# L-Scofano/SEEME

Hardware: AMD Instinct MI355X
Metric: sampled seqs/sec (T=196, 50 DDIM steps) (higher is better)
Workload: dtype f32 accumulate (fp16 denoiser weights, fp16 VAE MFMA operands); 1 GPU; config_mld_egobody interactee-only: VAE encode -> 50-step DDIM -> VAE decode, B=32/GPU, T=196, nfeats=132, random-init recipe weights; batch_per_gpu=32, seq_len=196, ddim_steps=50, parallelism=dp1 (independent shards, no collective on the data path)

## Files before the change

include/seeme_hip.h:

```cpp
#ifndef SEEME_HIP_H
#define SEEME_HIP_H

#include <stddef.h>
#include <stdint.h>

#ifdef __cplusplus
extern "C" {
#endif

#define SEEME_D 256
#define SEEME_NLAYERS 5

enum { SEEME_ACT_NONE = 0, SEEME_ACT_RELU = 1, SEEME_ACT_GELU = 2, SEEME_ACT_SILU = 3 };
enum { SEEME_SCHED_NONE = 0, SEEME_SCHED_DDIM = 1, SEEME_SCHED_DDPM = 2 };

int seeme_version(void);
const char* seeme_last_error(void);

#define SEEME_LINEAR_MAX_K 1008
typedef struct {
    const float* A;  int lda;
    const float* A2; int lda2;
    int K1;
    const float* W;  int ldw;
    const float* bias;
    const float* res; int ldr;
    const float* ln_w; const float* ln_b;
    const float* pre_ln_w; const float* pre_ln_b;
    float* Y; int ldy;
    int M, N, K;
    int pre_act;
    int act;
    float eps;
} SeemeLinearArgs;
int seeme_linear(const SeemeLinearArgs* args, void* stream);

typedef struct {
    const float *in_w, *in_b;
    const float *out_w, *out_b;
    const float *l1_w, *l1_b;
    const float *l2_w, *l2_b;
    const float *n1_w, *n1_b, *n2_w, *n2_b;
    const float *ca_in_w, *ca_in_b;
    const float *ca_out_w, *ca_out_b;
    const float *n3_w, *n3_b;
} SeemeXfLayer;

typedef struct {
    SeemeXfLayer layer[SEEME_NLAYERS];
    const float *skip_w[2], *skip_b[2];
    const float *norm_w, *norm_b;
} SeemeSkipStack;

typedef struct { const uint16_t *in_w, *out_w, *l1_w, *l2_w; } SeemeXfLayerH;
typedef struct {
    SeemeXfLayerH enc[SEEME_NLAYERS], dec[SEEME_NLAYERS];
    const uint16_t *enc_skip[2], *dec_skip[2];
    const uint16_t *emb_w, *fin_w, *ca_fold_w;
    const void* dec_pro; int dec_pro_T;
} SeemeVaeWeightsH;

typedef struct {
    int nfeats;
    int ff;
    const float* token;
    const float* pe_enc;
    const float* pe_dec;
    const float* emb_w; int emb_ldw;
    const float* emb_b;
    const float* fin_w;
    const float* fin_b;
    SeemeSkipStack enc, dec;
    const float* ca_fold_w;
    const float* ca_fold_b;
    const SeemeVaeWeightsH* h16;
} SeemeVaeWeights;

size_t seeme_vae_workspace_bytes(int B, int T);

int seeme_vae_encode(const SeemeVaeWeights* w, const float* features, const int32_t* lengths,
                     int B, int T, float* mu, float* logvar, void* workspace, size_t ws_bytes, void* stream);

int seeme_vae_decode(const SeemeVaeWeights* w, const float* z, const int32_t* lengths,
                     int B, int T, float* feats, void* workspace, size_t ws_bytes, void* stream);

size_t seeme_vae_dec_prologue_bytes(int T);
int seeme_vae_dec_prologue_h16(const SeemeVaeWeights* w, int T, void* buf, size_t bytes, void* stream);

typedef struct {
    const void*  wg;   int wdtype;
    const float* vp;
    const int64_t* layout;
    int nhead;
    int ff_sa;
    int ff;
    const float* kv_cat_w; const float* kv_cat_b;
    const float* style_cat_w; const float* style_cat_b;
    const float* time_w1; const float* time_b1; const float* time_w2; const float* time_b2;
    const float* ca_kv_w[SEEME_NLAYERS]; const float* ca_kv_b[SEEME_NLAYERS];
    const float* ca_tn_w[SEEME_NLAYERS]; const float* ca_tn_b[SEEME_NLAYERS];
    const float* ca_fold_w; const float* ca_fold_b;
    const float* ln_ones; const float* ln_zeros;
    int sa_fold;
    const float* ca_pn_w; const float* ca_pn_b;
    const float* ca_po_w; const float* ca_po_b;
} SeemeDenoiserWeights;

#define SEEME_TROW 7680
#define SEEME_CROW 5120

size_t seeme_denoiser_workspace_bytes(int n_rows, int B, int N);

int seeme_denoiser_time_tables(const SeemeDenoiserWeights* w, const float* tfeat, int n_rows,
                               float* ttab, void* workspace, size_t ws_bytes, void* stream);

int seeme_denoiser_cond_tables(const SeemeDenoiserWeights* w, const float* cond, int Bc, int N,
                               float* ctab, void* workspace, size_t ws_bytes, void* stream);

int seeme_denoiser_ca_tables(const SeemeDenoiserWeights* w, const float* ctab, const float* ttab, const int32_t* trow,
                             int trow_per_sample, int n_trow, int Bc, float* catab,
                             void* workspace, size_t ws_bytes, void* stream);

typedef struct {
    int B;
    int N;
    int steps;
    int sched;
    int cfg;
    float guidance_scale;
    const float* latents;
    const float* ctab;
    const float* ttab;
    const int32_t* trow;
    int trow_per_sample;
    const float* coef;
    const float* noise;
    float* out;
    const float* catab;
    float* save;
    int force_query;
    const unsigned char* drop;
    float drop_scale;
    int xcds;
} SeemeSampleArgs;
#define SEEME_DEN_DROP_BYTES 10960

int seeme_denoiser_sample(const SeemeDenoiserWeights* w, const SeemeSampleArgs* a, void* stream);

typedef struct {
    const void*  wgc;  int wdtype;
    const float* vpc;
    int C;
    int placement;
    int flags;
    void* xchg; size_t xchg_bytes;
    int query;
    int samples;
} SeemeDenCluster;
size_t seeme_den_cluster_xchg_bytes(int B, int C);
size_t seeme_den_cluster_ms_xchg_bytes(int B, int C, int samples);
int seeme_den_cluster_layout(int C, int wdtype, int query, int64_t* out, int cap);
int seeme_denoiser_sample_cluster(const SeemeDenoiserWeights* w, const SeemeDenCluster* cl, const SeemeSampleArgs* a, void* stream);

int seeme_den_train_layout(int64_t* out, int cap);
int seeme_den_train_pack(const float* const* mats, float* img_f, float* img_b, const float* const* vec_src,
                         const int* vec_n, const int64_t* vec_dst, int n_vec, float* vp, void* stream);
int seeme_denoiser_backward(const SeemeDenoiserWeights* w, const void* img_bwd, int B, int N, const float* save,
                            const float* ctab, const float* ttab, const int32_t* trow, const float* dout,
                            float* gout, float* dctab, float* dttab, void* stream);
int seeme_denoiser_backward_drop(const SeemeDenoiserWeights* w, const void* img_bwd, int B, int N, const float* save,
                                 const float* ctab, const float* ttab, const int32_t* trow, const float* dout,
                                 float* gout, float* dctab, float* dttab, const unsigned char* drop, float drop_scale, int xcds, void* stream);

int seeme_den_layout(int ff_sa, int ff, int64_t* out, int cap);

typedef struct {
    int V;
    const float* v_template;
    const float* blend_w;
    const float* lbs_weights;
    const float* J_template;
    const float* J_shapedirs;
    const int32_t* parents;
    const float* ex_template;
    const float* ex_shapedirs;
    const float* ex_posedirs;
    const float* ex_weights;
} SeemeSmplModel;

size_t seeme_smpl_workspace_bytes(int M);

int seeme_smpl_lbs(const SeemeSmplModel* m, const float* betas, const float* pose, int pose_is_rotmat,
                   const float* transl, int M, float* joints, float* vertices,
                   void* workspace, size_t ws_bytes, void* stream);

int seeme_smpl_joints_backward(const SeemeSmplModel* m, const float* betas, const float* pose, const float* djoints, int dj_stride,
                               float* dpose, float* dtransl, int M, void* stream);

int seeme_smpl_joints_rot6d(const SeemeSmplModel* m, const float* betas, const float* r6, int order, const float* transl, int M,
                            float* joints, void* stream);
int seeme_smpl_joints_rot6d_backward(const SeemeSmplModel* m, const float* betas, const float* r6, int order, const float* djoints,
                                     int dj_stride, float* dr6, float* dtransl, int M, void* stream);

enum { SEEME_GEO_AA_TO_QUAT = 0, SEEME_GEO_AA_TO_ROTMAT = 1, SEEME_GEO_QUAT_TO_ROTMAT = 2,
       SEEME_GEO_ROT6D_PROHMR = 3, SEEME_GEO_ROT6D_DIFFUSION = 4 };
int seeme_geometry(int op, const float* in, float* out, int M, void* stream);
int seeme_renorm(const float* x, const float* mean, const float* stdv, float* y, long rows, int F, void* stream);

typedef struct {
    int out_dim;
    const float* pos_w; const float* pos_b;
    const float* fc0_w[4]; const float* fc0_b[4];
    const float* fc1_w[4]; const float* fc1_b[4];
    const float* sc_w[4];
    const float* fcc_w; const float* fcc_b;
} SeemePointnetWeights;
size_t seeme_pointnet_workspace_bytes(int B, int P);
int seeme_pointnet_encode(const SeemePointnetWeights* w, const float* points, int B, int P, float* out,
                          void* workspace, size_t ws_bytes, void* stream);

typedef struct {
    const uint16_t* posf;
    const uint16_t* stream[4];
    const uint16_t* sc3f;
} SeemePointnetBf16;
size_t seeme_pointnet_bf16_workspace_bytes(int B, int P);
int seeme_pointnet_encode_bf16(const SeemePointnetWeights* w, const SeemePointnetBf16* wb, const float* points,
                               int B, int P, float* out, void* workspace, size_t ws_bytes, void* stream);

int seeme_den_wgrad(const float* gout, int ldg, int B, const void* tiles, int n_tiles, float* out, void* stream);
int seeme_den_vecgrad(const float* gout, int ldg, int B, const int64_t* idx, int n, float* out, int dx0_col, float* dpe_row0,
                      void* stream);

int seeme_adamw_step(const void* chunks, int n_chunks, void* const* params, const void* const* grads, void* const* exp_avg,
                     void* const* exp_avg_sq, double lr, double beta1, double beta2, double eps, double weight_decay,
                     double step, void* stream);

int seeme_adamw_step_dev(const void* chunks, int n_chunks, void* const* params, const void* const* grads, void* const* exp_avg,
                         void* const* exp_avg_sq, const float* step_lr, double beta1, double beta2, double eps,
                         double weight_decay, void* stream);

typedef struct {
    const void* chunks;
    int n_chunks;
    void* const* params;
    const void* const* grads;
    void* const* exp_avg;
    void* const* exp_avg_sq;
    void* const* ema;
    const float* step_lr;
    double lr, step;
    double beta1, beta2, eps, weight_decay;
    double ema_decay;
    int ema_warmup;
    const float* grad_scale;
} SeemeAdamWEx;
int seeme_adamw_step_ex(const SeemeAdamWEx* a, void* stream);
int seeme_adamw_ex_bytes(void);

size_t seeme_grad_norm_workspace_bytes(int n_chunks);
int seeme_grad_norm(const void* chunks, int n_chunks, const void* const* grads, double max_norm, float* out ,
                    void* ws, size_t ws_bytes, void* stream);

typedef struct {
    int B, N;
    const float* dist;
    int dist_rows;
    const float* eps_z;
    const float* eps_c;
    int slot_c;
    float* cond;
    const float* noise;
    const int64_t* timesteps;
    const float* acp;
// ... 184 lines not shown
```

seeme_amd/_lib.py:

```python
from __future__ import annotations

import ctypes as C
import os
from typing import Optional

_HERE = os.path.dirname(os.path.abspath(__file__))
LIB_PATH = os.environ.get("SEEME_HIP_LIB") or os.path.join(_HERE, "libseeme_hip.so")

NLAYERS = 5
TROW = 7680
CROW = 5120
ACT_NONE, ACT_RELU, ACT_GELU, ACT_SILU = 0, 1, 2, 3
SCHED_NONE, SCHED_DDIM, SCHED_DDPM = 0, 1, 2

fp = C.c_void_p


class SeemeError(RuntimeError):
    pass


class LinearArgs(C.Structure):
    _fields_ = [("A", fp), ("lda", C.c_int), ("A2", fp), ("lda2", C.c_int), ("K1", C.c_int),
                ("W", fp), ("ldw", C.c_int), ("bias", fp), ("res", fp), ("ldr", C.c_int),
# ... 15 lines not shown

class XfLayerH(C.Structure):
    _fields_ = [(n, fp) for n in ("in_w", "out_w", "l1_w", "l2_w")]


class VaeWeightsH(C.Structure):
    _fields_ = [("enc", XfLayerH * NLAYERS), ("dec", XfLayerH * NLAYERS), ("enc_skip", fp * 2), ("dec_skip", fp * 2),
                ("emb_w", fp), ("fin_w", fp), ("ca_fold_w", fp), ("dec_pro", fp), ("dec_pro_T", C.c_int)]


def pack_mfma16(W, dtype):
    import torch
    N, K = W.shape
    Np, Kp = (N + 15) // 16 * 16, (K + 31) // 32 * 32
    Wz = torch.zeros(Np, Kp, device=W.device, dtype=dtype)
    Wz[:N, :K] = W.detach().to(dtype)
    return Wz.view(Np // 16, 16, Kp // 32, 4, 8).permute(0, 2, 3, 1, 4).contiguous()


class VaeWeights(C.Structure):
    _fields_ = [("nfeats", C.c_int), ("ff", C.c_int), ("token", fp), ("pe_enc", fp), ("pe_dec", fp),
                ("emb_w", fp), ("emb_ldw", C.c_int), ("emb_b", fp), ("fin_w", fp), ("fin_b", fp),
                ("enc", SkipStack), ("dec", SkipStack), ("ca_fold_w", fp), ("ca_fold_b", fp), ("h16", fp)]


class DenoiserWeights(C.Structure):
    _fields_ = [("wg", fp), ("wdtype", C.c_int), ("vp", fp), ("layout", fp), ("nhead", C.c_int), ("ff_sa", C.c_int),
                ("ff", C.c_int), ("kv_cat_w", fp), ("kv_cat_b", fp), ("style_cat_w", fp), ("style_cat_b", fp),
                ("time_w1", fp), ("time_b1", fp), ("time_w2", fp), ("time_b2", fp),
                ("ca_kv_w", fp * NLAYERS), ("ca_kv_b", fp * NLAYERS),
                ("ca_tn_w", fp * NLAYERS), ("ca_tn_b", fp * NLAYERS),
                ("ca_fold_w", fp), ("ca_fold_b", fp), ("ln_ones", fp), ("ln_zeros", fp), ("sa_fold", C.c_int),
                ("ca_pn_w", fp), ("ca_pn_b", fp), ("ca_po_w", fp), ("ca_po_b", fp)]


class SampleArgs(C.Structure):
    _fields_ = [("B", C.c_int), ("N", C.c_int), ("steps", C.c_int), ("sched", C.c_int), ("cfg", C.c_int),
                ("guidance_scale", C.c_float), ("latents", fp), ("ctab", fp), ("ttab", fp), ("trow", fp),
                ("trow_per_sample", C.c_int), ("coef", fp), ("noise", fp), ("out", fp), ("catab", fp), ("save", fp), ("force_query", C.c_int), ("drop", fp), ("drop_scale", C.c_float), ("xcds", C.c_int)]


class DenCluster(C.Structure):
    _fields_ = [("wgc", fp), ("wdtype", C.c_int), ("vpc", fp), ("C", C.c_int), ("placement", C.c_int), ("flags", C.c_int),
                ("xchg", fp), ("xchg_bytes", C.c_size_t), ("query", C.c_int), ("samples", C.c_int)]


class SmplModel(C.Structure):
    _fields_ = [("V", C.c_int), ("v_template", fp), ("blend_w", fp), ("lbs_weights", fp), ("J_template", fp),
                ("J_shapedirs", fp), ("parents", fp), ("ex_template", fp), ("ex_shapedirs", fp),
                ("ex_posedirs", fp), ("ex_weights", fp)]


class PointnetWeights(C.Structure):
    _fields_ = [("out_dim", C.c_int), ("pos_w", fp), ("pos_b", fp), ("fc0_w", fp * 4), ("fc0_b", fp * 4),
                ("fc1_w", fp * 4), ("fc1_b", fp * 4), ("sc_w", fp * 4), ("fcc_w", fp), ("fcc_b", fp)]


class PointnetBf16(C.Structure):
    _fields_ = [("posf", fp), ("stream", fp * 4), ("sc3f", fp)]


class GlueRows(C.Structure):
    _fields_ = [("B", C.c_int), ("N", C.c_int), ("dist", fp), ("dist_rows", C.c_int), ("eps_z", fp), ("eps_c", fp),
                ("slot_c", C.c_int), ("cond", fp), ("noise", fp), ("timesteps", fp), ("acp", fp), ("freq", fp),
                ("flip_sin_to_cos", C.c_int), ("latents", fp), ("noisy", fp), ("tfeat", fp)]


class GemmProblem(C.Structure):
    _fields_ = [("a", fp * 10), ("b", fp * 10), ("seg_len", C.c_int * 10), ("a_ks", C.c_long * 10),
                ("b_ks", C.c_long * 10), ("nseg", C.c_int), ("a_rs", C.c_long), ("b_cs", C.c_long), ("c", fp), ("ldc", C.c_long),
                ("M", C.c_int), ("N", C.c_int), ("a_pro", C.c_int), ("a_p0", fp), ("a_p1", fp), ("b_pro", C.c_int),
                ("b_p0", fp), ("b_p1", fp), ("bias", fp), ("epi", C.c_int), ("e0", fp), ("e_ld", C.c_long),
                ("accumulate", C.c_int), ("colsum", fp), ("tile0", C.c_int), ("tiles_n", C.c_int), ("nbatch", C.c_int),
                ("a_bstride", C.c_long), ("b_bstride", C.c_long), ("c_bstride", C.c_long), ("alpha", C.c_float), ("addend", fp),
                ("add_ld", C.c_long)]


class VtLn(C.Structure):
    _fields_ = [("sub", fp), ("res", fp), ("gamma", fp), ("beta", fp), ("y", fp), ("xhat", fp), ("rstd", fp), ("M", C.c_long),
                ("sub_seq_rows", C.c_int), ("eps", C.c_float)]


class VtLnBwd(C.Structure):
    _fields_ = [("dy", fp), ("xhat", fp), ("rstd", fp), ("gamma", fp), ("dpre", fp), ("dgamma", fp), ("dbeta", fp), ("M", C.c_long),
                ("accumulate", C.c_int), ("dy2", fp)]


class GlueMid(C.Structure):
    _fields_ = [("M", C.c_int), ("B", C.c_int), ("dxl", fp), ("dcs", fp), ("xhat", fp), ("rstd", fp), ("tn_w", fp * 5),
                ("g_tn_w", fp * 5), ("g_tn_b", fp * 5), ("dcond", fp), ("dea", fp), ("deb", fp), ("emb", fp), ("demb", fp)]


class AdamWEx(C.Structure):
    _fields_ = [("chunks", fp), ("n_chunks", C.c_int), ("params", fp), ("grads", fp), ("exp_avg", fp), ("exp_avg_sq", fp),
                ("ema", fp), ("step_lr", fp), ("lr", C.c_double), ("step", C.c_double), ("beta1", C.c_double), ("beta2", C.c_double),
                ("eps", C.c_double), ("weight_decay", C.c_double), ("ema_decay", C.c_double), ("ema_warmup", C.c_int),
                ("grad_scale", fp)]


RESNET_FP32, RESNET_BF16 = 0, 1
IMG_F32_NCHW, IMG_U8_NHWC = 0, 1
RESNET50_NCONV = 53


class Conv(C.Structure):
    _fields_ = [("weight", fp), ("weight_bf16", fp), ("bias", fp), ("cin", C.c_int), ("cout", C.c_int), ("k", C.c_int),
                ("stride", C.c_int)]


class Resnet50(C.Structure):
    _fields_ = [("precision", C.c_int), ("conv", Conv * RESNET50_NCONV), ("tap", fp * 5)]


class RenderScene(C.Structure):
    _fields_ = [("verts", fp), ("faces", fp), ("points", fp), ("cams", fp)] + \
               [(n, C.c_int) for n in ("F", "NV", "NF", "P", "FC", "H", "W", "point_size")] + \
               [(n, C.c_float) for n in ("fx", "fy", "cx", "cy", "znear")]


GEO_AA_TO_QUAT, GEO_AA_TO_ROTMAT, GEO_QUAT_TO_ROTMAT, GEO_ROT6D_PROHMR, GEO_ROT6D_DIFFUSION = range(5)

_SIGNATURES = {
    "seeme_smpl_joints_backward": (C.c_int, [C.POINTER(SmplModel), fp, fp, fp, C.c_int, fp, fp, C.c_int, fp]),
    "seeme_smpl_joints_rot6d": (C.c_int, [C.POINTER(SmplModel), fp, fp, C.c_int, fp, C.c_int, fp, fp]),
    "seeme_smpl_joints_rot6d_backward": (C.c_int, [C.POINTER(SmplModel), fp, fp, C.c_int, fp, C.c_int, fp, fp, C.c_int, fp]),
    "seeme_vt_add_ln": (C.c_int, [C.POINTER(VtLn), fp]),
    "seeme_vt_ln_bwd": (C.c_int, [C.POINTER(VtLnBwd), fp]),
    "seeme_vt_softmax_fwd": (C.c_int, [fp, fp, C.c_int, C.c_int, C.c_int, C.c_float, fp]),
    "seeme_vt_softmax_bwd": (C.c_int, [fp, fp, C.c_long, C.c_int, C.c_float, fp]),
    "seeme_vt_gelu": (C.c_int, [fp, fp, fp, C.c_long, fp]),
    "seeme_vt_seq_sum": (C.c_int, [fp, fp, C.c_int, C.c_int, C.c_int, fp, C.c_float, fp]),
    "seeme_vt_dropout": (C.c_int, [fp, fp, C.c_float, fp, C.c_long, fp]),
    "seeme_vt_cross_rows": (C.c_int, [fp, fp, fp, fp, C.c_float, C.c_int, C.c_int, fp, fp]),
    "seeme_den_vecgrad": (C.c_int, [fp, C.c_int, C.c_int, fp, C.c_int, fp, C.c_int, fp, fp]),
    "seeme_glue_rows": (C.c_int, [C.POINTER(GlueRows), fp]),
    "seeme_glue_ln": (C.c_int, [fp, fp, fp, C.c_int, fp]),
    "seeme_glue_mid": (C.c_int, [C.POINTER(GlueMid), fp]),
    "seeme_grouped_gemm": (C.c_int, [fp, C.c_int, C.c_int, fp]),
    "seeme_gemm_problem_bytes": (C.c_int, []),
    "seeme_wgrad128": (C.c_int, [fp, C.c_long, fp, C.c_long, C.c_int, C.c_int, C.c_int, fp, C.c_long, fp, fp]),
    "seeme_gemm128": (C.c_int, [fp, C.c_long, fp, C.c_long, C.c_int, fp, C.c_long, C.c_int, C.c_int, C.c_int, fp, fp, C.c_long, fp]),
    "seeme_version": (C.c_int, []),
    "seeme_last_error": (C.c_char_p, []),
    "seeme_linear": (C.c_int, [C.POINTER(LinearArgs), fp]),
    "seeme_vae_workspace_bytes": (C.c_size_t, [C.c_int, C.c_int]),
    "seeme_vae_encode": (C.c_int, [C.POINTER(VaeWeights), fp, fp, C.c_int, C.c_int, fp, fp, fp, C.c_size_t, fp]),
    "seeme_vae_decode": (C.c_int, [C.POINTER(VaeWeights), fp, fp, C.c_int, C.c_int, fp, fp, C.c_size_t, fp]),
    "seeme_vae_dec_prologue_bytes": (C.c_size_t, [C.c_int]),
    "seeme_vae_dec_prologue_h16": (C.c_int, [C.POINTER(VaeWeights), C.c_int, fp, C.c_size_t, fp]),
    "seeme_denoiser_workspace_bytes": (C.c_size_t, [C.c_int, C.c_int, C.c_int]),
    "seeme_denoiser_time_tables": (C.c_int, [C.POINTER(DenoiserWeights), fp, C.c_int, fp, fp, C.c_size_t, fp]),
    "seeme_denoiser_cond_tables": (C.c_int, [C.POINTER(DenoiserWeights), fp, C.c_int, C.c_int, fp, fp, C.c_size_t, fp]),
    "seeme_denoiser_ca_tables": (C.c_int, [C.POINTER(DenoiserWeights), fp, fp, fp, C.c_int, C.c_int, C.c_int, fp, fp, C.c_size_t, fp]),
    "seeme_denoiser_sample": (C.c_int, [C.POINTER(DenoiserWeights), C.POINTER(SampleArgs), fp]),
    "seeme_denoiser_sample_cluster": (C.c_int, [C.POINTER(DenoiserWeights), C.POINTER(DenCluster), C.POINTER(SampleArgs), fp]),
    "seeme_den_cluster_xchg_bytes": (C.c_size_t, [C.c_int, C.c_int]),
    "seeme_den_cluster_ms_xchg_bytes": (C.c_size_t, [C.c_int, C.c_int, C.c_int]),
    "seeme_den_cluster_layout": (C.c_int, [C.c_int, C.c_int, C.c_int, C.POINTER(C.c_int64), C.c_int]),
    "seeme_den_train_layout": (C.c_int, [C.POINTER(C.c_int64), C.c_int]),
    "seeme_den_train_pack": (C.c_int, [fp, fp, fp, fp, C.POINTER(C.c_int), C.POINTER(C.c_int64), C.c_int, fp, fp]),
    "seeme_denoiser_backward": (C.c_int, [C.POINTER(DenoiserWeights), fp, C.c_int, C.c_int, fp, fp, fp, fp, fp, fp, fp, fp, fp]),
    "seeme_denoiser_backward_drop": (C.c_int, [C.POINTER(DenoiserWeights), fp, C.c_int, C.c_int, fp, fp, fp, fp, fp, fp, fp, fp, fp, C.c_float, C.c_int, fp]),
    "seeme_den_layout": (C.c_int, [C.c_int, C.c_int, C.POINTER(C.c_int64), C.c_int]),
    "seeme_den_wgrad": (C.c_int, [fp, C.c_int, C.c_int, fp, C.c_int, fp, fp]),
    "seeme_adamw_step": (C.c_int, [fp, C.c_int, fp, fp, fp, fp, C.c_double, C.c_double, C.c_double, C.c_double, C.c_double,
                                   C.c_double, fp]),
    "seeme_adamw_step_dev": (C.c_int, [fp, C.c_int, fp, fp, fp, fp, fp, C.c_double, C.c_double, C.c_double, C.c_double, fp]),
    "seeme_adamw_step_ex": (C.c_int, [C.POINTER(AdamWEx), fp]),
    "seeme_adamw_ex_bytes": (C.c_int, []),
    "seeme_grad_norm_workspace_bytes": (C.c_size_t, [C.c_int]),
    "seeme_grad_norm": (C.c_int, [fp, C.c_int, fp, C.c_double, fp, fp, C.c_size_t, fp]),
    "seeme_geometry": (C.c_int, [C.c_int, fp, fp, C.c_int, fp]),
    "seeme_renorm": (C.c_int, [fp, fp, fp, fp, C.c_long, C.c_int, fp]),
    "seeme_pointnet_workspace_bytes": (C.c_size_t, [C.c_int, C.c_int]),
    "seeme_pointnet_encode": (C.c_int, [C.POINTER(PointnetWeights), fp, C.c_int, C.c_int, fp, fp, C.c_size_t, fp]),
    "seeme_pointnet_bf16_workspace_bytes": (C.c_size_t, [C.c_int, C.c_int]),
    "seeme_pointnet_encode_bf16": (C.c_int, [C.POINTER(PointnetWeights), C.POINTER(PointnetBf16), fp, C.c_int, C.c_int, fp, fp,
                                             C.c_size_t, fp]),
    "seeme_smpl_workspace_bytes": (C.c_size_t, [C.c_int]),
    "seeme_smpl_lbs": (C.c_int, [C.POINTER(SmplModel), fp, fp, C.c_int, fp, C.c_int, fp, fp, fp, C.c_size_t, fp]),
    "seeme_hyp_metrics_workspace_bytes": (C.c_size_t, [C.c_int, C.c_int, C.c_int]),
    "seeme_hyp_metrics": (C.c_int, [fp, fp, fp, C.c_int, C.c_int, C.c_int, fp, fp, fp, C.c_size_t, fp]),
    "seeme_hyp_pairdist_workspace_bytes": (C.c_size_t, [C.c_int, C.c_int, C.c_int]),
    "seeme_hyp_pairdist": (C.c_int, [fp, fp, C.c_int, C.c_int, C.c_int, fp, fp, fp, C.c_size_t, fp]),
    "seeme_social_metrics_workspace_bytes": (C.c_size_t, [C.c_int, C.c_int, C.c_int]),
    "seeme_social_metrics": (C.c_int, [fp, fp, fp, fp, fp, fp, fp, C.c_int, C.c_int, C.c_int, fp, fp, fp, C.c_size_t, fp]),
    "seeme_overlap_cost_workspace_bytes": (C.c_size_t, [C.c_int, C.c_int, C.c_int, C.c_int]),
    "seeme_overlap_cost": (C.c_int, [fp, C.c_int, C.c_int, C.c_int, C.c_int, fp, fp, C.c_size_t, fp]),
    "seeme_path_select_workspace_bytes": (C.c_size_t, [C.c_int, C.c_int]),
    "seeme_path_select": (C.c_int, [fp, fp, C.c_int, C.c_int, fp, fp, fp, fp, C.c_size_t, fp]),
    "seeme_stitch_windows": (C.c_int, [fp, C.c_int, C.c_int, C.c_int, C.c_int, C.c_int, C.c_int, fp, fp]),
    "seeme_scene_views_workspace_bytes": (C.c_size_t, [C.c_int, C.c_int, C.c_int]),
    "seeme_scene_views": (C.c_int, [fp, fp, C.c_int, C.c_int, C.c_int, fp, fp, fp, fp, C.c_size_t, fp]),
    "seeme_crop_patches": (C.c_int, [fp, C.c_int, C.c_int, C.c_int, fp, fp, C.c_int, C.c_int, fp, fp]),
    "seeme_render_workspace_bytes": (C.c_size_t, [C.c_int, C.c_int, C.c_int, C.c_int]),
    "seeme_render": (C.c_int, [C.POINTER(RenderScene), fp, fp, fp, fp, C.c_size_t, fp]),
    "seeme_render_shade": (C.c_int, [C.POINTER(RenderScene), fp, fp, fp, C.c_int, fp, C.c_uint32, fp, fp]),
    "seeme_pa_mpjpe_frames": (C.c_int, [fp, fp, fp, C.c_int, fp, fp]),
    "seeme_mesh_v2v_frames": (C.c_int, [fp, fp, fp, fp, fp, C.c_int, C.c_int, fp, fp]),
    "seeme_scene_min_dist2_workspace_bytes": (C.c_size_t, [C.c_int, C.c_int, C.c_int, C.c_int]),
    "seeme_scene_min_dist2": (C.c_int, [fp, fp, fp, C.c_int, C.c_int, C.c_int, C.c_int, fp, fp, C.c_size_t, fp]),
    "seeme_scene_inside_count_workspace_bytes": (C.c_size_t, [C.c_int, C.c_int, C.c_int, C.c_int]),
    "seeme_scene_inside_count": (C.c_int, [fp, fp, C.c_int, fp, fp, C.c_int, C.c_int, C.c_int, C.c_int, fp, fp, C.c_size_t, fp]),
    "seeme_mesh_winding": (C.c_int, [fp, fp, C.c_int, fp, fp, C.c_int, C.c_int, C.c_int, C.c_int, fp, fp]),
    "seeme_resnet50_workspace_bytes": (C.c_size_t, [C.c_int, C.c_int]),
    "seeme_resnet50_encode": (C.c_int, [C.POINTER(Resnet50), fp, C.c_int, C.c_int, fp, fp, C.c_size_t, fp]),
    "seeme_resnet_conv": (C.c_int, [C.POINTER(Conv), C.c_int, fp, C.c_int, C.c_int, C.c_int, fp, C.c_int, fp, fp]),
    "seeme_resnet_stem_pack": (C.c_int, [fp, C.c_int, C.c_int, C.c_int, C.c_int, C.c_int, fp, fp]),
    "seeme_resnet_maxpool": (C.c_int, [C.c_int, fp, C.c_int, C.c_int, C.c_int, C.c_int, fp, fp]),
}

_lib: Optional[C.CDLL] = None


def lib() -> C.CDLL:
    global _lib
    if _lib is None:
        if not os.path.exists(LIB_PATH):
            raise SeemeError(
                f"{LIB_PATH} is missing: build it with `python -c 'import __graft_entry__ as g; g.build()'` "
                "or seeme_amd/csrc/build.sh.  There is no CPU / PyTorch fallback for this path.")
        try:
            l = C.CDLL(LIB_PATH)
        except OSError as e:
            raise SeemeError(f"cannot load {LIB_PATH}: {e}") from e
        for name, (res, args) in _SIGNATURES.items():
            f = getattr(l, name)
            f.restype = res
            f.argtypes = args
        _lib = l
    return _lib


def exported_symbols():
    return sorted(_SIGNATURES)


def check(rc: int, what: str = ""):
    if rc != 0:
        msg = lib().seeme_last_error().decode("utf-8", "replace")
        raise SeemeError(f"{what or 'seeme_hip'} failed (rc={rc}): {msg}")


def call(name: str, *args):
    check(getattr(lib(), name)(*args), name)


class Workspace:

    def __init__(self, per_stream: bool):
        self.per_stream = per_stream
        self._held = {}

    def get(self, need: int, device):
        import torch
        device = torch.device(device)
        if device.type == "cuda" and device.index is None:
            device = torch.device("cuda", torch.cuda.current_device())
        key = device
        if self.per_stream and device.type == "cuda":
            key = (device, torch.cuda.current_stream(device).cuda_stream)
        ws = self._held.get(key)
        if ws is None or ws.numel() < max(need, 16):
            ws = None
            self._held.pop(key, None)
            ws = self._held[key] = torch.empty(max(int(need), 16), dtype=torch.uint8, device=device)
        return ws

    def cached(self) -> list:
        return list(self._held.values())

    def fill_(self, byte: int):
        for ws in self._held.values():
            ws.fill_(byte)


def default_xcds(chains: int, want="auto") -> int:
    e = os.environ.get("SEEME_DEN_XCDS")
    if e is not None:
        want = int(e)
    if want == "auto":
        want = (chains + 15) // 16
    return min(8, max(1, int(want)))


def ptr(t) -> int:
    return 0 if t is None else t.data_ptr()


def current_stream() -> int:
    import torch
    return torch.cuda.current_stream().cuda_stream


def require_cuda(t, name: str):
    import torch
    if not isinstance(t, torch.Tensor) or not t.is_cuda:
        raise SeemeError(f"{name} must be a tensor on the ROCm device (cuda:N); this path has no CPU fallback")
    if t.dtype != torch.float32:
        raise SeemeError(f"{name} must be float32, got {t.dtype}")
```

seeme_amd/csrc/den_kernels.hip:

```cpp
#include <atomic>
#include "common.hpp"
#include "api_util.hpp"
#include "den_layout.h"
#include "lds_ring.hpp"
#include "den_train.h"
#include <utility>

#define DEN_THREADS 512
#define SEEME_DEN_PAIR_ABOVE 256
#define DEN_MAXTOK 6
#define DEN_R 4
#define DEN_CH 8

struct WF32 { typedef float T; static constexpr int KV = 4; static constexpr bool HALF = false, MFMA = false; static constexpr int PARTS = 1; };
struct WBF16 { typedef uint16_t T; static constexpr int KV = 8; static constexpr bool HALF = false, MFMA = true; static constexpr int PARTS = 3; };
struct WF16 { typedef uint16_t T; static constexpr int KV = 8; static constexpr bool HALF = true, MFMA = true; static constexpr int PARTS = 2; };
#define DEN_F16_LO_SCALE 2048.f

typedef float f2 __attribute__((ext_vector_type(2)));
typedef unsigned int u32x4 __attribute__((ext_vector_type(4)));
typedef float f32x4 __attribute__((ext_vector_type(4)));
typedef _Float16 h16x8 __attribute__((ext_vector_type(8)));
typedef __bf16 bf16x8 __attribute__((ext_vector_type(8)));

struct Ring { u32x4 r[DEN_R][DEN_CH]; };

#define FF_SA 1024
#define FF_D 128
#define XB_LD 1024

enum { G_SKIP = 0, G_INP, G_OUTP, G_L1, G_L2, G_CAQ, G_CAO, G_F1, G_F2, G_FO, G_NUM,
       GB_FO = G_NUM, GB_F2, GB_F1, GB_CAO, GB_CAQ, GB_L2, GB_L1, GB_OUTP, GB_INP, GB_SKIP, G_ALL };
constexpr int den_gK(int g) {
    constexpr int k[G_ALL] = {512, 256, 256, 256, FF_SA, 256, 256, 256, FF_D, 256,
                              256, 256, FF_D, 256, 256, 256, FF_SA, 256, 768, 256};
    return k[g];
}
constexpr int den_gN(int g) {
    constexpr int n[G_ALL] = {256, 768, 256, FF_SA, 256, 256, 256, FF_D, 256, 256,
                              256, FF_D, 256, 256, 256, FF_SA, 256, 256, 256, 512};
    return n[g];
}

constexpr int den_gcd(int a, int b) { return b == 0 ? a : den_gcd(b, a % b); }
template <typename WT, int G>
struct GS {
    static constexpr int K = den_gK(G), N = den_gN(G);
    static constexpr int G0 = N / 2;
    static constexpr int KS = DEN_THREADS / den_gcd(G0, DEN_THREADS);
    static constexpr int IT = G0 / den_gcd(G0, DEN_THREADS);
    static constexpr int NQ = K / WT::KV / KS;
    static constexpr int CPI = NQ / 4;
    static constexpr int TOT = IT * CPI;
    static_assert(G0 * KS == DEN_THREADS * IT && NQ * KS * WT::KV == K && NQ % 4 == 0 && TOT >= 1, "unsupported GEMV shape");
    static constexpr int TW = N / 16 / (DEN_THREADS / 64), KB = K / 32;
    static constexpr int TG = (TW % 4 == 0) ? 4 : ((TW % 3 == 0) ? 3 : ((TW % 2 == 0) ? 2 : 1));
    static constexpr int GL = TG * KB;
    static_assert(!WT::MFMA || (TW * 16 * (DEN_THREADS / 64) == N && KB * 32 == K && TW * KB == TOT * DEN_CH && GL % DEN_CH == 0),
                  "unsupported MFMA GEMV shape");
    __device__ static __forceinline__ void item(int tid, int it, int& ks, int& n0) {
        const int idx = tid + it * DEN_THREADS;
        ks = idx / G0; n0 = idx - ks * G0;
    }
};

#define V_CAQ 1
#define V_FOLD 2
template <typename WT, int V>
struct Prog {
    static constexpr bool CAQ = (V & V_CAQ) != 0, FOLD = (V & V_FOLD) != 0;
    static constexpr int NG = 6 + (CAQ ? 2 : 0) + (FOLD ? 0 : 1);
    static constexpr int gid(int i) {
        constexpr int all[9] = {G_INP, G_OUTP, G_L1, G_L2, G_CAQ, G_CAO, G_F1, G_F2, G_FO};
        int k = 0;
        for (int j = 0; j < 9; ++j) {
            const int g = all[j];
            if ((g == G_OUTP && FOLD) || ((g == G_CAQ || g == G_CAO) && !CAQ)) continue;
            if (k == i) return g;
            ++k;
        }
        return G_FO;
    }
    static constexpr int tot(int g) {
        switch (g) {
            case G_SKIP: return GS<WT, G_SKIP>::TOT; case G_INP: return GS<WT, G_INP>::TOT; case G_OUTP: return GS<WT, G_OUTP>::TOT;
            case G_L1: return GS<WT, G_L1>::TOT; case G_L2: return GS<WT, G_L2>::TOT; case G_CAQ: return GS<WT, G_CAQ>::TOT;
            case G_CAO: return GS<WT, G_CAO>::TOT; case G_F1: return GS<WT, G_F1>::TOT; case G_F2: return GS<WT, G_F2>::TOT;
            default: return GS<WT, G_FO>::TOT;
        }
    }
    static constexpr int sum_real() { int s = 0; for (int j = 0; j < NG; ++j) s += tot(gid(j)); return s; }
    static constexpr int T = (sum_real() + DEN_R - 1) / DEN_R * DEN_R;
    static constexpr int PAD = T - sum_real();
    static constexpr int PAD0 = tot(G_INP);
    static constexpr bool is_pad(int t) { return t >= PAD0 && t < PAD0 + PAD; }
    static constexpr int start(int i) { int s = (i >= 1 ? PAD : 0); for (int j = 0; j < i; ++j) s += tot(gid(j)); return s; }
    static constexpr int TS = tot(G_SKIP);
    static constexpr int find(int t) { int i = 0; while (i + 1 < NG && start(i + 1) <= t) ++i; return i; }
    static constexpr int pos(int g) { int i = 0; while (gid(i) != g) ++i; return i; }
    static_assert(gid(0) == G_INP, "in_proj opens the layer program");
    static_assert(TS % DEN_R == 0 && TS >= DEN_R, "skip linear must fill whole ring turns");
    static_assert(tot(G_INP) >= DEN_R, "the first GEMV of a layer must cover the cross-layer prefetch");
};

#ifdef DEN_DBG_TIMES
__device__ unsigned long long den_dbg_times[512];
__device__ __forceinline__ void den_dbg(int mode) {
    __shared__ unsigned long long buf[512];
    __shared__ int cnt, armed;
    if (blockIdx.x != 0 || threadIdx.x != 0) return;
    if (mode == 1) { cnt = 0; armed = 1; }
    else if (mode == 2) { armed = 0; }
    else if (mode == 0) { if (armed && cnt < 511) { buf[cnt] = __builtin_readcyclecounter(); cnt = cnt + 1; } }
    else {
        const int n = (armed == 0 && cnt >= 0 && cnt <= 511) ? cnt : 0;
        for (int i = 0; i < n; ++i) den_dbg_times[i + 1] = buf[i];
        den_dbg_times[0] = (unsigned long long)n;
    }
}
#define DEN_DBG(m) den_dbg(m)
#else
#define DEN_DBG(m) do {} while (0)
#endif

template <typename WT, int G, int C>
__device__ __forceinline__ void issue_mat(u32x4 (&slot)[DEN_CH], int tid, __amdgpu_buffer_rsrc_t rsrc, unsigned mat_bytes) {
    typedef GS<WT, G> S;
    if constexpr (WT::MFMA) {
        const unsigned voff = (unsigned)(tid >> 6) * (unsigned)(S::TW * S::KB * 1024) + (unsigned)(tid & 63) * 16u;
        const unsigned soff = mat_bytes + (unsigned)(C * DEN_CH) * 1024u;
#pragma unroll
        for (int i = 0; i < DEN_CH; ++i) slot[i] = __builtin_amdgcn_raw_buffer_load_b128(rsrc, voff, soff + (unsigned)(i * 1024), 0);
        return;
    }
    constexpr int it = C / S::CPI, cc = C % S::CPI;
    int ks, n0;
    S::item(tid, it, ks, n0);
    const unsigned voff = (unsigned)(ks * S::NQ * S::N + n0) * 16u;
    const unsigned soff = mat_bytes + (unsigned)(cc * 4) * S::N * 16u;
#pragma unroll
    for (int i = 0; i < DEN_CH; ++i)
        slot[i] = __builtin_amdgcn_raw_buffer_load_b128(rsrc, voff, soff + (unsigned)(((i >> 1) * S::N + (i & 1) * S::G0) * 16), 0);
}
struct MatOffs { unsigned m[G_NUM]; unsigned next; };
template <typename WT>
__device__ __forceinline__ MatOffs load_mat_offs(const DenLayerOff* __restrict__ L, const DenLayerOff* __restrict__ Ln, bool nskip) {
    MatOffs o;
#pragma unroll
    for (int g = 0; g < G_NUM; ++g) o.m[g] = (unsigned)(reinterpret_cast<const int64_t*>(L)[g] * (long long)sizeof(typename WT::T));
    o.next = (unsigned)((nskip ? Ln->skip : Ln->inp) * (long long)sizeof(typename WT::T));
    return o;
}

template <typename WT, int V, int T>
__device__ __forceinline__ void issue_p0(Ring& ring, int tid, __amdgpu_buffer_rsrc_t rsrc, const MatOffs& mo) {
// ... 659 lines not shown
                    xr = f4_add(nl, ld4(CONSTV + 4 * lane));
                    put_x<WT, MS>(XB, es, 0, lane, xr);
                }
                __syncthreads(); DEN_DBG(0);
            }
            cur ^= 1;
        }
        row = row_next;
    }
    DEN_DBG(3);
    if (epi && (es == 0 || (!A.cfg && MS * b + es < A.B))) st4(A.out + (size_t)bl * 256 + 4 * lane, ld4(keep));
#pragma unroll
    for (int s = 0; s < DEN_R; ++s) asm volatile("" ::"v"(ring.r[s][0].x));
}

static size_t den_lds_bytes(int MS, int N, bool mfma) {
    return (size_t)(768 + MS * 768 + 2 * (VP_LAYER + STG_TT + MS * N * 1024 + (N > 1 ? 0 : MS * 256)) + XB_FLOATS(mfma, MS) + (mfma ? MS * 1024 : 4 * MS * 768)) * sizeof(float);
}

static int den_xcd_grid(int chains, int want, int* xcds) {
    int k = (want >= 1 && want <= 7) ? want : 8;
    if (chains > 32 * k) k = 8;
    *xcds = k;
    return k < 8 ? (chains + k - 1) / k * 8 : chains;
}
template <typename WT, int MS, int V>
static int launch_den(const DenKArgs& ka, hipStream_t st) {
    const int chains = (MS == 2 && !ka.s.cfg) ? (ka.s.B + 1) / 2 : ka.s.B;
    const size_t lds = den_lds_bytes(MS, ka.s.N, WT::MFMA);
    if (lds > 160 * 1024) return seeme_fail("denoiser_sample: LDS budget exceeded");
    SEEME_HIP(hipFuncSetAttribute((const void*)k_den_sample<WT, MS, V>, hipFuncAttributeMaxDynamicSharedMemorySize, (int)lds));
    DenKArgs k2 = ka;
    k2.chains = chains;
    const int grid = den_xcd_grid(chains, ka.s.xcds, &k2.xcds);
    hipLaunchKernelGGL((k_den_sample<WT, MS, V>), dim3(grid), dim3(DEN_THREADS), lds, st, k2);
    return seeme_check_launch("k_den_sample");
}
template <typename WT, int MS>
static int launch_den_ms(const DenKArgs& ka, bool fold, hipStream_t st) {
    const bool caq = ka.s.N > 1 || ka.s.force_query;
    if (caq) return fold ? launch_den<WT, MS, V_CAQ | V_FOLD>(ka, st) : launch_den<WT, MS, V_CAQ>(ka, st);
    return fold ? launch_den<WT, MS, V_FOLD>(ka, st) : launch_den<WT, MS, 0>(ka, st);
}
template <typename WT>
static int launch_den_wt(const DenKArgs& ka, bool fold, hipStream_t st) {
    const bool pair = ka.s.cfg || (ka.s.B > SEEME_DEN_PAIR_ABOVE && !ka.s.trow_per_sample);
    return pair ? launch_den_ms<WT, 2>(ka, fold, st) : launch_den_ms<WT, 1>(ka, fold, st);
}

extern "C" int seeme_denoiser_sample(const SeemeDenoiserWeights* w, const SeemeSampleArgs* a, void* stream) {
    if (a->B <= 0) return seeme_fail("denoiser_sample: B must be > 0");
    if (a->N < 1 || a->N > DEN_MAXTOK - 2) return seeme_fail("denoiser_sample: 1 <= N <= 4 condition tokens");
    if (w->nhead != 1 && w->nhead != 2 && w->nhead != 4) return seeme_fail("denoiser_sample: nhead must be 1, 2 or 4");
    if (w->ff_sa != FF_SA || w->ff != FF_D) return seeme_fail("denoiser_sample: built for sa ff 1024 / ffn_dim 128 (all reference configs)");
    if (w->layout == nullptr) return seeme_fail("denoiser_sample: layout table missing");
    if (a->sched == SEEME_SCHED_NONE && a->steps != 1) return seeme_fail("denoiser_sample: SCHED_NONE needs steps == 1");
    if (a->steps < 1) return seeme_fail("denoiser_sample: steps must be >= 1");
    if (a->save != nullptr && (a->steps != 1 || a->cfg || w->sa_fold || w->wdtype != 0 || !(a->N > 1 || a->force_query) || !a->trow_per_sample))
        return seeme_fail("denoiser_sample: save needs one step, no CFG, the unfolded fp32 image, the query GEMV and per-sample rows");
    DenKArgs ka;
    ka.wg = w->wg; ka.vp = w->vp; ka.lay = seeme_make_den_layout(FF_SA, FF_D);
    ka.wg_bytes = (int)(ka.lay.wg_total * (w->wdtype == 0 ? 4 : 2));
    ka.nhead = w->nhead; ka.s = *a;
    hipStream_t st = (hipStream_t)stream;
    const bool fold = w->sa_fold != 0;
    if (fold && w->nhead != 1) return seeme_fail("denoiser_sample: sa_fold needs nhead == 1");
    if (a->N == 1 && a->catab == nullptr && !a->force_query) return seeme_fail("denoiser_sample: N == 1 needs the ca table (seeme_denoiser_ca_tables)");
    if (w->wdtype == 0) return launch_den_wt<WF32>(ka, fold, st);
    if (w->wdtype == 1) return launch_den_wt<WBF16>(ka, fold, st);
    if (w->wdtype == 2) return launch_den_wt<WF16>(ka, fold, st);
    return seeme_fail("denoiser_sample: wdtype must be 0 (fp32), 1 (bf16) or 2 (fp16)");
}

extern "C" int seeme_den_layout(int ff_sa, int ff, int64_t* out, int cap) {
    if (cap < SEEME_DEN_LAYOUT_FIELDS) return seeme_fail("seeme_den_layout: output too small");
    const DenLayout lay = seeme_make_den_layout(ff_sa, ff);
    int k = 0;
    for (int l = 0; l < SEEME_DEN_NL; ++l) {
        const int64_t* f = reinterpret_cast<const int64_t*>(&lay.L[l]);
        for (int i = 0; i < SEEME_DEN_LAYER_FIELDS; ++i) out[k++] = f[i];
    }
    out[k++] = lay.pe0; out[k++] = lay.fnw; out[k++] = lay.fnb; out[k++] = lay.wg_total; out[k++] = lay.vp_total;
    return 0;
}

extern "C" size_t seeme_denoiser_workspace_bytes(int n_rows, int B, int N) {
    (void)B; (void)N;
    return (size_t)n_rows * 256 * 2 * sizeof(float) + 256;
}

extern "C" int seeme_denoiser_time_tables(const SeemeDenoiserWeights* w, const float* tfeat, int n_rows,
                                          float* ttab, void* workspace, size_t ws_bytes, void* stream) {
    hipStream_t st = (hipStream_t)stream;
    if (ws_bytes < seeme_denoiser_workspace_bytes(n_rows, 0, 0)) return seeme_fail("time_tables: workspace too small");
    float* t1 = (float*)workspace;
    float* temb = t1 + (size_t)n_rows * 256;
    int rc;
    if ((rc = seeme_linear_simple(st, tfeat, 256, w->time_w1, 256, w->time_b1, t1, 256, n_rows, 256, 256, SEEME_ACT_SILU, 0, nullptr, nullptr))) return rc;
    if ((rc = seeme_linear_simple(st, t1, 256, w->time_w2, 256, w->time_b2, temb, 256, n_rows, 256, 256, 0, 0, nullptr, nullptr))) return rc;
    if ((rc = seeme_linear_simple(st, temb, 256, w->kv_cat_w, 256, w->kv_cat_b, ttab, SEEME_TROW, n_rows, 2560, 256, 0, 0, nullptr, nullptr))) return rc;
    return seeme_linear_simple(st, temb, 256, w->style_cat_w, 256, w->style_cat_b, ttab + 2560, SEEME_TROW, n_rows, 5120, 256, 0, SEEME_ACT_SILU, nullptr, nullptr);
}

extern "C" int seeme_denoiser_cond_tables(const SeemeDenoiserWeights* w, const float* cond, int Bc, int N,
                                          float* ctab, void* workspace, size_t ws_bytes, void* stream) {
    (void)workspace; (void)ws_bytes;
    hipStream_t st = (hipStream_t)stream;
    const int M = Bc * N;
    if (w->ca_fold_w == nullptr) return seeme_fail("cond_tables: folded key/value weights missing");
    LinearKArgs ka{};
    ka.a.A = cond; ka.a.lda = 256; ka.a.K1 = 256; ka.a.K = 256; ka.a.W = w->kv_cat_w; ka.a.ldw = 256; ka.a.bias = w->kv_cat_b;
    ka.a.Y = ctab; ka.a.ldy = SEEME_CROW; ka.a.M = M; ka.a.N = 2560; ka.a.eps = 1e-5f;
    ka.a.pre_ln_w = w->ln_ones; ka.a.pre_ln_b = w->ln_zeros;
    ka.nz = 2; ka.zs_a = 0; ka.zs_w = (long)(w->ca_fold_w - w->kv_cat_w); ka.zs_b = (long)(w->ca_fold_b - w->kv_cat_b); ka.zs_y = 2560;
    ka.zs_ln = 0; ka.pre_ln_zmin = 1;
    return seeme_launch_linear(ka, st);
}

__global__ __launch_bounds__(256) void k_ca_rows(const float* __restrict__ ctab, const float* __restrict__ ttab,
                                                 const int32_t* __restrict__ trow, int per_sample, int n_trow, int R, int rows,
                                                 const float* __restrict__ nw, const float* __restrict__ nb, float* __restrict__ H) {
    const int lane = threadIdx.x & 63, l = blockIdx.y;
    const int r0 = blockIdx.x * 4 + (threadIdx.x >> 6);
    if (r0 >= rows) return;
    const int bc = r0 / R, r = r0 - bc * R;
    const int row = per_sample ? trow[bc % n_trow] : trow[r];
    const float4 v = ld4(ctab + (size_t)bc * SEEME_CROW + 2560 + l * 512 + 256 + 4 * lane);
    const float4 hn = wave_ln(v, nw + l * 256, nb + l * 256, lane);
    const float* tt = ttab + (size_t)row * SEEME_TROW + 2560 + l * 1024;
    st4(H + ((size_t)l * rows + r0) * 256 + 4 * lane, f4_silu(f4_adaln(hn, ld4(tt + 4 * lane), ld4(tt + 256 + 4 * lane))));
}

extern "C" int seeme_denoiser_ca_tables(const SeemeDenoiserWeights* w, const float* ctab, const float* ttab, const int32_t* trow,
                                        int trow_per_sample, int n_trow, int Bc, float* catab,
                                        void* workspace, size_t ws_bytes, void* stream) {
    hipStream_t st = (hipStream_t)stream;
    if (Bc <= 0 || n_trow <= 0) return seeme_fail("ca_tables: empty batch / row list");
    const int R = trow_per_sample ? 1 : n_trow;
    const int rows = Bc * R;
    if (ws_bytes < (size_t)SEEME_DEN_NL * rows * 256 * sizeof(float)) return seeme_fail("ca_tables: workspace too small");
    if (w->ca_pn_w == nullptr || w->ca_po_w == nullptr) return seeme_fail("ca_tables: proj_out weights missing");
    float* H = (float*)workspace;
    hipLaunchKernelGGL(k_ca_rows, dim3((rows + 3) / 4, SEEME_DEN_NL), dim3(256), 0, st, ctab, ttab, trow, trow_per_sample, n_trow, R, rows,
                       w->ca_pn_w, w->ca_pn_b, H);
    int rc = seeme_check_launch("k_ca_rows");
    if (rc) return rc;
    LinearKArgs ka{};
    ka.a.A = H; ka.a.lda = 256; ka.a.K1 = 256; ka.a.W = w->ca_po_w; ka.a.ldw = 256; ka.a.bias = w->ca_po_b;
    ka.a.Y = catab; ka.a.ldy = SEEME_DEN_NL * 256; ka.a.M = rows; ka.a.N = 256; ka.a.K = 256; ka.a.eps = 1e-5f;
    ka.nz = SEEME_DEN_NL; ka.zs_a = (long)rows * 256; ka.zs_w = 256 * 256; ka.zs_b = 256; ka.zs_y = 256;
    return seeme_launch_linear(ka, st);
}

#ifdef DEN_DBG_TIMES
extern "C" int seeme_debug_den_times(unsigned long long* host, int n) {
    SEEME_HIP(hipMemcpyFromSymbol(host, HIP_SYMBOL(den_dbg_times), sizeof(unsigned long long) * (size_t)(n < 512 ? n : 512)));
    return 0;
}
#endif

#include "den_train.inc.hip"
#include "den_cluster.inc.hip"
#include "den_cluster_ms.inc.hip"
```

seeme_amd/csrc/vae_h16.hip:

```cpp
#include "common.hpp"
#include "api_util.hpp"

typedef _Float16 h16x8 __attribute__((ext_vector_type(8)));
#define HPAD 16

__device__ __forceinline__ unsigned short f2h(float x) { return __builtin_bit_cast(unsigned short, (_Float16)x); }
__device__ __forceinline__ float h_exp(float x) { return __builtin_amdgcn_exp2f(x * 1.44269504088896340736f); }
__device__ __forceinline__ float h_gelu(float x) {
    const float z = fabsf(x) * 0.70710678118654752440f;
    const float t = __builtin_amdgcn_rcpf(fmaf(0.3275911f, z, 1.f));
    const float poly = t * fmaf(t, fmaf(t, fmaf(t, fmaf(t, 1.061405429f, -1.453152027f), 1.421413741f), -0.284496736f), 0.254829592f);
    return 0.5f * x * (1.f + copysignf(1.f - poly * h_exp(-z * z), x));
}
__device__ __forceinline__ float h_act(float v, int act) { return act == SEEME_ACT_GELU ? h_gelu(v) : act_apply(v, act); }

#ifdef H16_DBG_TIMES
__device__ unsigned long long h16_dbg_times[32];
#ifndef H16_DBG_KERNEL
#define H16_DBG_KERNEL 1
#endif
#define H16_DBG(k, i) do { if (H16_DBG_KERNEL == (k) && blockIdx.x == 3 && blockIdx.y == ((k) == 1 ? 5 : 0) && threadIdx.x == 0) h16_dbg_times[i] = __builtin_readcyclecounter(); } while (0)
extern "C" int seeme_debug_h16_times(unsigned long long* host, int n) {
    SEEME_HIP(hipMemcpyFromSymbol(host, HIP_SYMBOL(h16_dbg_times), sizeof(unsigned long long) * (size_t)(n < 32 ? n : 32)));
    return 0;
}
#else
#define H16_DBG(k, i) do {} while (0)
#endif
#ifndef H16_PF
#define H16_PF 4
#endif
#ifndef H16_ALA
#define H16_ALA 1
#endif
#ifndef FFN_PF
#define FFN_PF H16_PF
#endif
template <int NTL, int PF>
struct BRing { uint4 br[PF][NTL]; };
template <int NTL, int PF, typename LoadB>
__device__ __forceinline__ void ring_prime(BRing<NTL, PF>& ring, int K32, LoadB loadb) {
#pragma unroll
    for (int u = 0; u < PF; ++u)
#pragma unroll
        for (int nt = 0; nt < NTL; ++nt) ring.br[u][nt] = loadb(nt, u < K32 ? u : K32 - 1);
}

template <int MTL, int NTL, int PF, typename LoadB>
__device__ __forceinline__ void tile_gemm_h16(const unsigned short* __restrict__ As, int lda, int K32, LoadB loadb,
                                              f32x4 (&acc)[MTL][NTL], BRing<NTL, PF>& ring) {
    const int lane = threadIdx.x & 63, r = lane & 15, kq = lane >> 4;
    const unsigned short* ap = As + r * lda + 8 * kq;
    uint4 (&br)[PF][NTL] = ring.br;
    constexpr int AS = H16_ALA == 1 ? 2 : 4;
    static_assert(PF % AS == 0, "A-fragment slots follow the ring slot");
    uint4 ab[AS][MTL];
#pragma unroll
    for (int d = 0; d < H16_ALA; ++d)
#pragma unroll
        for (int mt = 0; mt < MTL; ++mt) ab[d][mt] = *reinterpret_cast<const uint4*>(ap + mt * 16 * lda + (d < K32 ? d : K32 - 1) * 32);
    const int K32r = (K32 + PF - 1) / PF * PF;
    int kb0 = 0;
    for (; kb0 + PF < K32r; kb0 += PF) {
#pragma unroll
        for (int u = 0; u < PF; ++u) {
            const int kb = kb0 + u;
            const int ka = kb + H16_ALA < K32 ? kb + H16_ALA : K32 - 1;
#pragma unroll
            for (int mt = 0; mt < MTL; ++mt) ab[(u + H16_ALA) % AS][mt] = *reinterpret_cast<const uint4*>(ap + mt * 16 * lda + ka * 32);
            __builtin_amdgcn_sched_barrier(0);
#pragma unroll
            for (int mt = 0; mt < MTL; ++mt)
#pragma unroll
                for (int nt = 0; nt < NTL; ++nt)
                    acc[mt][nt] = __builtin_amdgcn_mfma_f32_16x16x32_f16(__builtin_bit_cast(h16x8, ab[u % AS][mt]), __builtin_bit_cast(h16x8, br[u][nt]), acc[mt][nt], 0, 0, 0);
            __builtin_amdgcn_sched_barrier(0);
            const int kn = kb + PF < K32 ? kb + PF : K32 - 1;
#pragma unroll
            for (int nt = 0; nt < NTL; ++nt) br[u][nt] = loadb(nt, kn);
        }
    }
#pragma unroll
    for (int u = 0; u < PF; ++u) {
        const int kb = kb0 + u;
        const int ka = (kb + H16_ALA < K32) ? kb + H16_ALA : K32 - 1;
#pragma unroll
        for (int mt = 0; mt < MTL; ++mt) ab[(u + H16_ALA) % AS][mt] = *reinterpret_cast<const uint4*>(ap + mt * 16 * lda + ka * 32);
        __builtin_amdgcn_sched_barrier(0);
        if (kb < K32) {
#pragma unroll
            for (int mt = 0; mt < MTL; ++mt)
#pragma unroll
                for (int nt = 0; nt < NTL; ++nt)
                    acc[mt][nt] = __builtin_amdgcn_mfma_f32_16x16x32_f16(__builtin_bit_cast(h16x8, ab[u % AS][mt]), __builtin_bit_cast(h16x8, br[u][nt]), acc[mt][nt], 0, 0, 0);
        }
        __builtin_amdgcn_sched_barrier(0);
    }
}
struct PackedSrc {
    __amdgpu_buffer_rsrc_t rs; int kstride, ntile0, ntiles; unsigned voff;
    __device__ __forceinline__ PackedSrc(const uint4* __restrict__ Wp, int kstride_, int ntile0_, int ntiles_)
        : rs(__builtin_amdgcn_make_buffer_rsrc(const_cast<uint4*>(Wp), 0, 0x7FFFFFF0, 0x00020000)), kstride(kstride_),
          ntile0(__builtin_amdgcn_readfirstlane(ntile0_)), ntiles(ntiles_), voff((threadIdx.x & 63) * 16u) {}
    __device__ __forceinline__ uint4 operator()(int nt, int kb) const {
        int t = ntile0 + nt; t = t < ntiles ? t : ntiles - 1;
        return __builtin_bit_cast(uint4, __builtin_amdgcn_raw_buffer_load_b128(rs, voff, (unsigned)(t * kstride + kb) * 1024u, 0));
    }
};
template <int MTL, int NTL, int PF = H16_PF>
__device__ __forceinline__ void gemm_packed(const unsigned short* As, int lda, const uint4* __restrict__ Wp, int kstride,
                                            int ntile0, int ntiles, int K32, f32x4 (&acc)[MTL][NTL], BRing<NTL, PF>& ring) {
    tile_gemm_h16<MTL, NTL, PF>(As, lda, K32, PackedSrc(Wp, kstride, ntile0, ntiles), acc, ring);
}
template <int NTL, int PF = H16_PF>
__device__ __forceinline__ void prime_packed(BRing<NTL, PF>& ring, const uint4* __restrict__ Wp, int kstride, int ntile0, int ntiles, int K32) {
    ring_prime(ring, K32, PackedSrc(Wp, kstride, ntile0, ntiles));
}
template <int MTL, int NTL, int PF = H16_PF>
__device__ __forceinline__ void gemm_packed(const unsigned short* As, int lda, const uint4* __restrict__ Wp, int kstride,
                                            int ntile0, int ntiles, int K32, f32x4 (&acc)[MTL][NTL]) {
    BRing<NTL, PF> ring;
    prime_packed(ring, Wp, kstride, ntile0, ntiles, K32);
    gemm_packed<MTL, NTL, PF>(As, lda, Wp, kstride, ntile0, ntiles, K32, acc, ring);
}
template <int MTL, int NTL, int PF = H16_PF>
__device__ __forceinline__ void gemm_rows(const unsigned short* As, int lda, const unsigned short* __restrict__ Bm, int ldb,
                                          int n0, int n_valid, int K32, f32x4 (&acc)[MTL][NTL]) {
    const int lane = threadIdx.x & 63, r = lane & 15, kq = lane >> 4;
    auto loadb = [&](int nt, int kb) {
        int n = n0 + nt * 16 + r; n = n < n_valid ? n : n_valid - 1;
        return *reinterpret_cast<const uint4*>(Bm + (size_t)n * ldb + kb * 32 + 8 * kq);
    };
    BRing<NTL, PF> ring;
    ring_prime(ring, K32, loadb);
    tile_gemm_h16<MTL, NTL, PF>(As, lda, K32, loadb, acc, ring);
}
template <int MTL, int NTL>
__device__ __forceinline__ void acc_store_h16(const f32x4 (&acc)[MTL][NTL], unsigned short* __restrict__ Hs, int ldh, int c0,
                                              const float* __restrict__ bias, int act) {
    const int lane = threadIdx.x & 63, r = lane & 15, kq = lane >> 4;
#pragma unroll
    for (int nt = 0; nt < NTL; ++nt) {
        const int c = c0 + nt * 16 + r;
        const float bv = bias ? bias[c] : 0.f;
#pragma unroll
        for (int mt = 0; mt < MTL; ++mt)
#pragma unroll
            for (int i = 0; i < 4; ++i) Hs[(mt * 16 + 4 * kq + i) * ldh + c] = f2h(h_act(acc[mt][nt][i] + bv, act));
    }
}

template <int MTL, int NTL>
__device__ __forceinline__ void acc_store_h16(const f32x4 (&acc)[MTL][NTL], unsigned short* __restrict__ Hs, int ldh, int c0,
                                              const BiasRegs<NTL>& bias, int act) {
    const int lane = threadIdx.x & 63, r = lane & 15, kq = lane >> 4;
#pragma unroll
    for (int nt = 0; nt < NTL; ++nt) {
        const int c = c0 + nt * 16 + r;
#pragma unroll
        for (int mt = 0; mt < MTL; ++mt)
#pragma unroll
            for (int i = 0; i < 4; ++i) Hs[(mt * 16 + 4 * kq + i) * ldh + c] = f2h(h_act(acc[mt][nt][i] + bias.v[nt], act));
    }
}

struct LinearHArgs {
    LinearKArgs k;
    const uint4* wp; int kstride; int ntiles;
    int qkv_mode;
    unsigned short* qk; unsigned short* vt; int S, spv;
    int fast;
};
__host__ __device__ static inline bool linear_h_fast(const SeemeLinearArgs& a) {
    return (a.pre_ln_w == nullptr) && ((a.K & 3) == 0) && ((a.K1 & 3) == 0) && ((a.lda & 3) == 0) &&
           ((reinterpret_cast<size_t>(a.A) & 15) == 0) &&
           (a.A2 == nullptr || (((a.lda2 & 3) == 0) && ((reinterpret_cast<size_t>(a.A2) & 15) == 0)));
}

__global__ __launch_bounds__(256) void k_linear_h(const LinearHArgs ha) {
    extern __shared__ __attribute__((aligned(16))) float smem[];
    const LinearKArgs& ka = ha.k;
    const SeemeLinearArgs& a = ka.a;
    const int tid = threadIdx.x, wave = tid >> 6, lane = tid & 63;
    const int Kp = (a.K + 31) & ~31;
    const int lda_f = Kp + LDS_PAD, lda_h = Kp + HPAD;
    const bool fast = ha.fast != 0;
    float* Af = smem;
    float* Cs = fast ? smem : Af + TILE_M * lda_f;
    unsigned short* Ah = reinterpret_cast<unsigned short*>(Cs + TILE_M * (CH_N + LDS_PAD));
    const int ldc = CH_N + LDS_PAD;
    const int m0 = blockIdx.x * TILE_M, cn0 = blockIdx.y * CH_N;
    H16_DBG(2, 0);
    const int n0 = cn0 + wave * 64;
    const BiasRegs<4> bias = bias_load<4>(a.bias, n0, a.N);
    BRing<4, H16_PF> ring;
    if (n0 < a.N) prime_packed(ring, ha.wp, ha.kstride, n0 >> 4, ha.ntiles, Kp >> 5);

    if (ha.fast == 1) {
        const int Kp4 = Kp >> 2, K4 = a.K >> 2, total = TILE_M * Kp4;
        for (int base = 0; base < total; base += 256 * 8) {
            float4 v[8];
#pragma unroll
            for (int j = 0; j < 8; ++j) {
                const int idx = base + tid + j * 256, row = idx / Kp4, c4 = idx - row * Kp4, m = m0 + row;
                const bool valid = idx < total && m < a.M && c4 < K4;
                int prow = valid ? m : 0;
                if (ka.seq_in > 0) prow = (prow / ka.seq_in) * ka.in_stride + (prow % ka.seq_in) + ka.in_off;
                const bool first = 4 * c4 < a.K1 || a.A2 == nullptr;
                const float* p = first ? a.A + (size_t)prow * a.lda + 4 * c4 : a.A2 + (size_t)prow * a.lda2 + (4 * c4 - a.K1);
                v[j] = *reinterpret_cast<const float4*>(valid ? p : a.A);
                if (!valid) v[j] = make_float4(0.f, 0.f, 0.f, 0.f);
            }
            __builtin_amdgcn_sched_barrier(0);
#pragma unroll
            for (int j = 0; j < 8; ++j) {
                const int idx = base + tid + j * 256, row = idx / Kp4, c4 = idx - row * Kp4;
                if (idx < total) {
                    float4 w = v[j];
                    if (a.pre_act != SEEME_ACT_NONE)
                        w = make_float4(act_apply(w.x, a.pre_act), act_apply(w.y, a.pre_act), act_apply(w.z, a.pre_act), act_apply(w.w, a.pre_act));
                    if (!(m0 + row < a.M && c4 < K4)) w = make_float4(0.f, 0.f, 0.f, 0.f);
                    const unsigned lo = (unsigned)f2h(w.x) | ((unsigned)f2h(w.y) << 16), hi = (unsigned)f2h(w.z) | ((unsigned)f2h(w.w) << 16);
                    *reinterpret_cast<uint2*>(Ah + row * lda_h + 4 * c4) = make_uint2(lo, hi);
                }
            }
        }
        __syncthreads();
    } else if (ha.fast == 2) {
        const LnParams lp = ln_params256(a.pre_ln_w, a.pre_ln_b);
        float4 xv[8];
#pragma unroll
        for (int rr = 0; rr < 8; ++rr) {
            const int m = m0 + wave * 8 + rr;
            int prow = m < a.M ? m : 0;
            if (ka.seq_in > 0) prow = (prow / ka.seq_in) * ka.in_stride + (prow % ka.seq_in) + ka.in_off;
            xv[rr] = *reinterpret_cast<const float4*>(a.A + (size_t)prow * a.lda + lane * 4);
        }
        __builtin_amdgcn_sched_barrier(0);
#pragma unroll
        for (int rr = 0; rr < 8; ++rr) {
            const int row = wave * 8 + rr;
            float4 v = wave_layernorm256(xv[rr], lp, a.eps);
            if (a.pre_act != SEEME_ACT_NONE)
                v = make_float4(act_apply(v.x, a.pre_act), act_apply(v.y, a.pre_act), act_apply(v.z, a.pre_act), act_apply(v.w, a.pre_act));
            if (m0 + row >= a.M) v = make_float4(0.f, 0.f, 0.f, 0.f);
            const unsigned lo = (unsigned)f2h(v.x) | ((unsigned)f2h(v.y) << 16), hi = (unsigned)f2h(v.z) | ((unsigned)f2h(v.w) << 16);
            *reinterpret_cast<uint2*>(Ah + row * lda_h + lane * 4) = make_uint2(lo, hi);
        }
        __syncthreads();
// ... 386 lines not shown
    const BiasRegs<2> bias1 = bias_load<2>(a.b1, wave * 32, a.FF);
    const BiasRegs<4> bias2 = bias_load<4>(a.b2, wave * 64, 256);
    BRing<2, FFN_PF> ring1;
    BRing<4, H16_PF> ring2;
    prime_packed(ring1, a.w1, 8, wave * 2, a.FF >> 4, 8);
    prime_packed(ring2, a.w2, a.FF >> 5, wave * 4, 16, a.FF >> 5);
    H16_DBG(3, 0);
    {
        float4 xv[8], cv[8];
        const LnParams lc = ln_params256(a.lnc_w, a.lnc_b);
#pragma unroll
        for (int rr = 0; rr < 8; ++rr) {
            const int m = m0 + wave * 8 + rr, mc = m < a.M ? m : 0;
            const int seq = mc / a.seq_rows;
            const size_t prow = (size_t)seq * a.seq_stride + (mc % a.seq_rows);
            xv[rr] = *reinterpret_cast<const float4*>(a.x + prow * 256 + lane * 4);
            cv[rr] = make_float4(0.f, 0.f, 0.f, 0.f);
            if (a.cvec != nullptr) cv[rr] = *reinterpret_cast<const float4*>(a.cvec + (size_t)seq * a.cvec_ld + lane * 4);
        }
        __builtin_amdgcn_sched_barrier(0);
#pragma unroll
        for (int rr = 0; rr < 8; ++rr) {
            const int row = wave * 8 + rr, m = m0 + row;
            float4 v = xv[rr];
            if (a.cvec != nullptr) {
                v = make_float4(v.x + cv[rr].x, v.y + cv[rr].y, v.z + cv[rr].z, v.w + cv[rr].w);
                v = wave_layernorm256(v, lc, a.eps);
            }
            if (m >= a.M) v = make_float4(0.f, 0.f, 0.f, 0.f);
            *reinterpret_cast<float4*>(Xs + row * ld + lane * 4) = v;
            const unsigned lo = (unsigned)f2h(v.x) | ((unsigned)f2h(v.y) << 16), hi = (unsigned)f2h(v.z) | ((unsigned)f2h(v.w) << 16);
            *reinterpret_cast<uint2*>(Xh + row * ldh + lane * 4) = make_uint2(lo, hi);
        }
    }
    __syncthreads();
    H16_DBG(3, 1);
    const int ldhh = a.FF + HPAD;
    {
        f32x4 acc1[2][2];
        acc_zero(acc1);
        gemm_packed<2, 2, FFN_PF>(Xh, ldh, a.w1, 8, wave * 2, a.FF >> 4, 8, acc1, ring1);
        acc_store_h16<2, 2>(acc1, Hh, ldhh, wave * 32, bias1, a.act);
    }
    __syncthreads();
    H16_DBG(3, 2);
    {
        f32x4 acc2[2][4];
        acc_zero(acc2);
        gemm_packed<2, 4>(Hh, ldhh, a.w2, a.FF >> 5, wave * 4, 16, a.FF >> 5, acc2, ring2);
        acc_store_lds<2, 4>(acc2, Cs, ld, wave * 64, bias2, SEEME_ACT_NONE);
    }
    __syncthreads();
    H16_DBG(3, 3);
    const LnParams lp = ln_params256(a.ln_w, a.ln_b), lf = ln_params256(a.fin_w, a.fin_b);
#pragma unroll 2
    for (int rr = 0; rr < 8; ++rr) {
        const int row = wave * 8 + rr, m = m0 + row;
        if (m >= a.M) continue;
        float4 v = *reinterpret_cast<const float4*>(Cs + row * ld + lane * 4);
        const float4 x = *reinterpret_cast<const float4*>(Xs + row * ld + lane * 4);
        v = make_float4(v.x + x.x, v.y + x.y, v.z + x.z, v.w + x.w);
        v = wave_layernorm256(v, lp, a.eps);
        if (a.fin_w != nullptr) v = wave_layernorm256(v, lf, a.eps);
        const int seq = m / a.seq_rows, sr = m % a.seq_rows;
        size_t orow = (size_t)seq * a.seq_stride + sr;
        if (a.out_mode == 1) orow = (size_t)sr * (a.M / a.seq_rows) + seq;
        *reinterpret_cast<float4*>(a.out + orow * 256 + lane * 4) = v;
    }
    H16_DBG(3, 4);
}

static int launch_ffn_h(const FfnHArgs& a, hipStream_t st) {
    if (a.FF != 128) return seeme_fail("ffn_h: FF must be 128 (hard-coded in the reference VAE, mld_vae.py:53)");
    const size_t lds = (size_t)2 * TILE_M * (256 + LDS_PAD) * 4 + (size_t)TILE_M * (a.FF + HPAD) * 2;
    dim3 grid((a.M + TILE_M - 1) / TILE_M);
    SEEME_HIP(hipFuncSetAttribute((const void*)k_ffn_block_h, hipFuncAttributeMaxDynamicSharedMemorySize, (int)lds));
    hipLaunchKernelGGL(k_ffn_block_h, grid, dim3(256), lds, st, a);
    return seeme_check_launch("k_ffn_block_h");
}

#ifndef LAYER_KV_PF
#define LAYER_KV_PF 4
#endif
#ifndef LAYER_W8_PF
#define LAYER_W8_PF 4
#endif
#ifndef LAYER_WPE
#define LAYER_WPE 2
#endif
struct LayerHArgs {
    const unsigned short* q; const uint4* kp; const uint4* vp; const float* res;
    const uint4* wo; const float* bo; const float* n1_w; const float* n1_b;
    const int32_t* lengths;
    int S, n_prefix, q_rows, Sp, spv; float scale, eps;
    const float* cvec; int cvec_ld; const float* lnc_w; const float* lnc_b;
    const uint4* w1; const float* b1; const uint4* w2; const float* b2; const float* n2_w; const float* n2_b;
    const float* fin_w; const float* fin_b;
    float* out; int out_mode, B;
    int in_shared;
    const uint4* skip_w; const float* skip_b; const float* skip_src; float* xnext;
    const uint4* qkv_w; const float* qkv_b; unsigned short* q_out; uint4* kp_out; uint4* vp_out;
    const uint4* proj_w; const float* proj_b; float* feats; int F;
    const float* z; const uint4* cf_w; const float* cf_b; int layer;
};
template <int WAVES, int RW>
__host__ __device__ constexpr bool layer_cvec_in() { return WAVES == 8 && RW == 4; }

__device__ __forceinline__ void rows_to_h16(unsigned short* Xh, int ldh, int row, int lane, float4 v) {
    const unsigned lo = (unsigned)f2h(v.x) | ((unsigned)f2h(v.y) << 16), hi = (unsigned)f2h(v.z) | ((unsigned)f2h(v.w) << 16);
    *reinterpret_cast<uint2*>(Xh + row * ldh + lane * 4) = make_uint2(lo, hi);
}

template <int WAVES, int RW>
__device__ __forceinline__ void tail_store_q(const unsigned short* Oh, int ld, unsigned short* __restrict__ q_out, size_t base, int q0, int S) {
    constexpr int NT = 64 * WAVES;
    const int tid = threadIdx.x;
#pragma unroll
    for (int it = 0; it < RW / 2; ++it) {
        const int idx = tid + it * NT, row = idx >> 5, c8 = (idx & 31) * 8, s = q0 + row;
        if (s < S) *reinterpret_cast<uint4*>(q_out + (base + s) * 256 + c8) = *reinterpret_cast<const uint4*>(Oh + row * ld + c8);
    }
}
template <int WAVES, int RW>
__device__ __forceinline__ void tail_store_k(const unsigned short* Oh, int ld, uint4* __restrict__ kp_out, int b, int q0, int S, int NT16) {
    constexpr int NT = 64 * WAVES;
    const int tid = threadIdx.x;
    uint4* kb_out = kp_out + ((size_t)b * NT16 + (q0 >> 4)) * 512;
#pragma unroll
    for (int it = 0; it < RW / 2; ++it) {
        const int idx = tid + it * NT, r = idx & 15, kq = (idx >> 4) & 3, kb = (idx >> 6) & 7, half = idx >> 9, row = half * 16 + r;
        if (q0 + row < S) kb_out[(half * 8 + kb) * 64 + kq * 16 + r] = *reinterpret_cast<const uint4*>(Oh + row * ld + kb * 32 + kq * 8);
    }
}
template <int WAVES, int RW>
__device__ __forceinline__ void tail_store_v(const unsigned short* Oh, int ld, uint4* __restrict__ vp_out, int b, int q0, int S, int KB) {
    constexpr int NT = 64 * WAVES;
    const int tid = threadIdx.x;
    uint4* vb_out = vp_out + (size_t)b * 16 * KB * 64;
#pragma unroll
    for (int it = 0; it < RW / 2; ++it) {
        const int idx = tid + it * NT, r = idx & 15, g = (idx >> 4) & 3, nt = (idx >> 6) & 15, kh = idx >> 10;
        const int row0 = 32 * kh + 8 * g, kb = (q0 >> 5) + kh;
        const unsigned short* src = Oh + row0 * ld + nt * 16 + r;
        unsigned w[4];
#pragma unroll
        for (int j = 0; j < 4; ++j) {
            const int s0 = q0 + row0 + 2 * j;
            const unsigned lo = s0 < S ? src[(2 * j) * ld] : 0u, hi = s0 + 1 < S ? src[(2 * j + 1) * ld] : 0u;
            w[j] = lo | (hi << 16);
        }
        if (kb < KB) vb_out[((size_t)nt * KB + kb) * 64 + g * 16 + r] = make_uint4(w[0], w[1], w[2], w[3]);
    }
}
template <int WAVES, int RW, int PF>
__device__ __forceinline__ void tail_qkv_rows(const unsigned short* Xh, unsigned short* Oh, const uint4* __restrict__ qkv_w,
                                              const float* __restrict__ qkv_b, unsigned short* __restrict__ q_out,
                                              uint4* __restrict__ kp_out, uint4* __restrict__ vp_out, int b, int q0, int S, int spv,
                                              BRing<16 / WAVES, PF>& ring_t) {
    constexpr int ROWS = RW * WAVES, MTL = ROWS / 16, NTL = 16 / WAVES, CW = 256 / WAVES;
    const int tid = threadIdx.x, wave = tid >> 6;
    const int ldq = 256 + HPAD;
    const size_t base = (size_t)b * S;
    const int NT16 = (S + 15) >> 4, KB = spv >> 5;
    constexpr int ldk = 256;
    unsigned short* const OhK = Oh + ROWS * ldq;
    {
        f32x4 acc[MTL][NTL];
        acc_zero(acc);
        const BiasRegs<NTL> bias = bias_load<NTL>(qkv_b, 0 * 256 + wave * CW, 768);
        gemm_packed<MTL, NTL, PF>(Xh, ldq, qkv_w, 8, 0 * 16 + wave * NTL, 48, 8, acc, ring_t);
        prime_packed(ring_t, qkv_w, 8, 1 * 16 + wave * NTL, 48, 8);
        __syncthreads();
        acc_store_h16<MTL, NTL>(acc, Oh, ldq, wave * CW, bias, SEEME_ACT_NONE);
    }
    {
        f32x4 acc[MTL][NTL];
        acc_zero(acc);
        const BiasRegs<NTL> bias = bias_load<NTL>(qkv_b, 1 * 256 + wave * CW, 768);
        gemm_packed<MTL, NTL, PF>(Xh, ldq, qkv_w, 8, 1 * 16 + wave * NTL, 48, 8, acc, ring_t);
        prime_packed(ring_t, qkv_w, 8, 2 * 16 + wave * NTL, 48, 8);
        acc_store_h16<MTL, NTL>(acc, OhK, ldk, wave * CW, bias, SEEME_ACT_NONE);
    }
    {
        f32x4 acc[MTL][NTL];
        acc_zero(acc);
        const BiasRegs<NTL> bias = bias_load<NTL>(qkv_b, 2 * 256 + wave * CW, 768);
        gemm_packed<MTL, NTL, PF>(Xh, ldq, qkv_w, 8, 2 * 16 + wave * NTL, 48, 8, acc, ring_t);
        __syncthreads();
        tail_store_q<WAVES, RW>(Oh, ldq, q_out, base, q0, S);
        tail_store_k<WAVES, RW>(OhK, ldk, kp_out, b, q0, S, NT16);
        __syncthreads();
        acc_store_h16<MTL, NTL>(acc, Oh, ldq, wave * CW, bias, SEEME_ACT_NONE);
        __syncthreads();
        tail_store_v<WAVES, RW>(Oh, ldq, vp_out, b, q0, S, KB);
    }
}

#define LAYER_DBG(i) do { if (a.qkv_w != nullptr) H16_DBG(5, i); } while (0)
template <int WAVES, int RW>
__global__ __launch_bounds__(64 * WAVES, WAVES == 4 ? LAYER_WPE : 1) void k_layer_h(const LayerHArgs a) {
    constexpr int ROWS = RW * WAVES, MTL = ROWS / 16, NTL = 16 / WAVES, CW = 256 / WAVES, N1 = 8 / WAVES, NT = 64 * WAVES;
    constexpr int PFW = (WAVES == 8 && RW == 4) ? LAYER_W8_PF : H16_PF, PFA = (WAVES == 8 && RW == 4) ? LAYER_W8_PF : ATT_PF,
                  PFK = (WAVES == 8 && RW == 4) ? LAYER_W8_PF : LAYER_KV_PF, PFF = (WAVES == 8 && RW == 4) ? LAYER_W8_PF : FFN_PF;
    extern __shared__ __attribute__((aligned(16))) float smem[];
    const int tid = threadIdx.x, wave = tid >> 6, lane = tid & 63, r = lane & 15, kq = lane >> 4;
    const int ldp = a.Sp + LDS_PAD, ldq = 256 + HPAD, ldph = 2 * ldp, ldc = 256 + LDS_PAD;
    float* R0 = smem;
    unsigned short* R1 = reinterpret_cast<unsigned short*>(R0 + ROWS * ldp);
    float* Ps = R0;
    unsigned short* Ph = reinterpret_cast<unsigned short*>(R0);
    unsigned short* Qh = R1;
    int b = blockIdx.y, qt = blockIdx.x;
    if ((gridDim.y & 7) == 0) {
        const int L = blockIdx.x + gridDim.x * blockIdx.y, rr = L & 7, q = L >> 3;
        b = rr + 8 * (q / (int)gridDim.x);
        qt = q % (int)gridDim.x;
    }
    const int q0 = qt * ROWS;
    const size_t base = (size_t)b * a.S;
    const size_t bin = a.in_shared ? 0 : (size_t)b, base_in = bin * a.S;
    const int n_valid_keys = min(a.S, a.n_prefix + a.lengths[b]);
    const BiasRegs<NTL> bias_o = bias_load<NTL>(a.bo, wave * CW, 256);
    BRing<NTL, PFA> ring_o;
    prime_packed(ring_o, a.wo, 8, wave * NTL, 16, 8);
    const bool cv_in = layer_cvec_in<WAVES, RW>() && a.z != nullptr;
    unsigned short* Zh = R1 + ROWS * ldq;
    float* CVs = reinterpret_cast<float*>(Zh + 16 * ldq);
    const int cv_t0 = 16 * a.layer + wave * NTL;
    BRing<NTL, 8> ring_c;
    BiasRegs<NTL> bias_c;
    if (cv_in) {
        bias_c = bias_load<NTL>(a.cf_b + 256 * a.layer, wave * CW, 256);
        for (int i = tid; i < 15 * ldq / 8; i += NT) reinterpret_cast<uint4*>(Zh + ldq)[i] = make_uint4(0u, 0u, 0u, 0u);
        if (wave == 0) rows_to_h16(Zh, ldq, 0, lane, *reinterpret_cast<const float4*>(a.z + (size_t)b * 256 + lane * 4));
    }
    LAYER_DBG(0);
    {
        uint4 qv[4];
#pragma unroll
        for (int it = 0; it < RW / 2; ++it) {
            const int idx = tid + it * NT, row = idx >> 5, c8 = (idx & 31) * 8, s = q0 + row;
            qv[it] = *reinterpret_cast<const uint4*>(a.q + (base_in + (s < a.q_rows ? s : 0)) * 256 + c8);
            if (s >= a.q_rows) qv[it] = make_uint4(0u, 0u, 0u, 0u);
        }
#pragma unroll
        for (int it = 0; it < RW / 2; ++it) {
            const int idx = tid + it * NT, row = idx >> 5, c8 = (idx & 31) * 8;
            *reinterpret_cast<uint4*>(Qh + row * ldq + c8) = qv[it];
        }
    }
    __syncthreads();
    LAYER_DBG(1);
    const int NT16 = (a.S + 15) >> 4;
    const uint4* Kp = a.kp + bin * NT16 * 512;
    for (int c0 = 0; c0 < a.Sp; c0 += CH_N) {
        const int n0 = c0 + wave * CW;
        f32x4 acc[MTL][NTL];
        acc_zero(acc);
        if (n0 < a.S) gemm_packed<MTL, NTL, PFK>(Qh, ldq, Kp, 8, n0 >> 4, NT16, 8, acc);
#pragma unroll
        for (int nt = 0; nt < NTL; ++nt) {
            const int c = n0 + nt * 16 + r;
            const bool ok = c < n_valid_keys;
#pragma unroll
            for (int mt = 0; mt < MTL; ++mt)
#pragma unroll
                for (int i = 0; i < 4; ++i) Ps[(mt * 16 + 4 * kq + i) * ldp + c] = ok ? acc[mt][nt][i] * a.scale : -INFINITY;
        }
    }
    __syncthreads();
    LAYER_DBG(2);
    if (cv_in) prime_packed(ring_c, a.cf_w, 8, cv_t0, 16 * SEEME_NLAYERS, 8);
    LAYER_DBG(21);
    if (a.Sp == 256) attn_softmax_rows<4, RW>(Ps, ldp, Ph, ldph, wave, lane);
    else attn_softmax_rows<8, RW>(Ps, ldp, Ph, ldph, wave, lane);
    __syncthreads();
    LAYER_DBG(3);
    if (cv_in) {
        f32x4 acc_c[1][NTL];
        acc_zero(acc_c);
        gemm_packed<1, NTL, 8>(Zh, ldq, a.cf_w, 8, cv_t0, 16 * SEEME_NLAYERS, 8, acc_c, ring_c);
        if (kq == 0) {
#pragma unroll
            for (int nt = 0; nt < NTL; ++nt) CVs[wave * CW + nt * 16 + r] = acc_c[0][nt][0] + bias_c.v[nt];
        }
    }
    LAYER_DBG(22);
    {
        f32x4 acc[MTL][NTL];
        acc_zero(acc);
        const int K32 = (n_valid_keys + 31) >> 5;
        gemm_packed<MTL, NTL, PFK>(Ph, ldph, a.vp + bin * 16 * (a.spv >> 5) * 64, a.spv >> 5, wave * NTL, 16, K32, acc);
        acc_store_h16<MTL, NTL>(acc, Qh, ldq, wave * CW, nullptr, SEEME_ACT_NONE);
    }
    __syncthreads();
    LAYER_DBG(4);
    float* Cs = R0;
    {
        f32x4 acc[MTL][NTL];
        acc_zero(acc);
        gemm_packed<MTL, NTL, PFA>(Qh, ldq, a.wo, 8, wave * NTL, 16, 8, acc, ring_o);
#ifdef H16_DBG_TIMES
        asm volatile("" : "+v"(acc[0][0][0]), "+v"(acc[MTL - 1][NTL - 1][3]));
        LAYER_DBG(23);
#endif
        acc_store_lds<MTL, NTL>(acc, Cs, ldc, wave * CW, bias_o, SEEME_ACT_NONE);
    }
    LAYER_DBG(24);
    const BiasRegs<N1> bias1 = bias_load<N1>(a.b1, wave * (128 / WAVES), 128);
    const BiasRegs<NTL> bias2 = bias_load<NTL>(a.b2, wave * CW, 256);
    BRing<N1, PFF> ring1;
    BRing<NTL, PFW> ring2;
    prime_packed(ring1, a.w1, 8, wave * N1, 8, 8);
    prime_packed(ring2, a.w2, 4, wave * NTL, 16, 4);
    LAYER_DBG(25);
    __syncthreads();
    LAYER_DBG(5);
    unsigned short* Xh = R1;
    float4 x1[RW];
    {
        const LnParams lp = ln_params256_opt(a.n1_w, a.n1_b, a.n1_w), lc = ln_params256_opt(a.lnc_w, a.lnc_b, a.n1_w);
        float4 xr[RW];
        const bool has_cv = cv_in || a.cvec != nullptr;
        const float4 cv = cv_in ? *reinterpret_cast<const float4*>(CVs + lane * 4)
                                : *reinterpret_cast<const float4*>((a.cvec != nullptr ? a.cvec + (size_t)b * a.cvec_ld : a.n1_w) + lane * 4);
#pragma unroll
        for (int rr = 0; rr < RW; ++rr) {
            const int s = q0 + wave * RW + rr;
            xr[rr] = *reinterpret_cast<const float4*>(a.res + (base_in + (s < a.q_rows ? s : 0)) * 256 + lane * 4);
        }
        __builtin_amdgcn_sched_barrier(0);
        LAYER_DBG(16);
#pragma unroll
        for (int rr = 0; rr < RW; ++rr) {
            const float4 v = *reinterpret_cast<const float4*>(Cs + (wave * RW + rr) * ldc + lane * 4);
            x1[rr] = make_float4(v.x + xr[rr].x, v.y + xr[rr].y, v.z + xr[rr].z, v.w + xr[rr].w);
        }
        LAYER_DBG(17);
        wave_layernorm256_rows<RW>(x1, lp, a.eps);
        LAYER_DBG(18);
        if (has_cv) {
#pragma unroll
            for (int rr = 0; rr < RW; ++rr) x1[rr] = make_float4(x1[rr].x + cv.x, x1[rr].y + cv.y, x1[rr].z + cv.z, x1[rr].w + cv.w);
            wave_layernorm256_rows<RW>(x1, lc, a.eps);
        }
        LAYER_DBG(19);
#pragma unroll
        for (int rr = 0; rr < RW; ++rr) {
            const int row = wave * RW + rr;
            if (q0 + row >= a.q_rows) x1[rr] = make_float4(0.f, 0.f, 0.f, 0.f);
            rows_to_h16(Xh, ldq, row, lane, x1[rr]);
        }
        LAYER_DBG(20);
    }
    __syncthreads();
    LAYER_DBG(6);
    unsigned short* Hh = R1;
    const int ldhh = 128 + HPAD;
    {
        f32x4 acc1[MTL][N1];
        acc_zero(acc1);
        gemm_packed<MTL, N1, PFF>(Xh, ldq, a.w1, 8, wave * N1, 8, 8, acc1, ring1);
        __syncthreads();
        acc_store_h16<MTL, N1>(acc1, Hh, ldhh, wave * (128 / WAVES), bias1, SEEME_ACT_GELU);
    }
    __syncthreads();
    LAYER_DBG(7);
    {
        f32x4 acc2[MTL][NTL];
        acc_zero(acc2);
        gemm_packed<MTL, NTL, PFW>(Hh, ldhh, a.w2, 4, wave * NTL, 16, 4, acc2, ring2);
        acc_store_lds<MTL, NTL>(acc2, Cs, ldc, wave * CW, bias2, SEEME_ACT_NONE);
    }
    const bool has_tail = a.skip_w != nullptr || a.qkv_w != nullptr || a.proj_w != nullptr;
    BRing<NTL, PFW> ring_t;
    if (a.skip_w != nullptr) prime_packed(ring_t, a.skip_w, 16, wave * NTL, 16, 8);
    else if (a.qkv_w != nullptr) prime_packed(ring_t, a.qkv_w, 8, wave * NTL, 48, 8);
    else if (a.proj_w != nullptr) prime_packed(ring_t, a.proj_w, 8, wave * NTL, (a.F + 15) >> 4, 8);
    __syncthreads();
    LAYER_DBG(8);
    {
        const LnParams lp = ln_params256_opt(a.n2_w, a.n2_b, a.n2_w), lf = ln_params256_opt(a.fin_w, a.fin_b, a.n2_w);
        float4 v[RW];
#pragma unroll
        for (int rr = 0; rr < RW; ++rr) {
            const float4 c = *reinterpret_cast<const float4*>(Cs + (wave * RW + rr) * ldc + lane * 4);
            v[rr] = make_float4(c.x + x1[rr].x, c.y + x1[rr].y, c.z + x1[rr].z, c.w + x1[rr].w);
        }
        wave_layernorm256_rows<RW>(v, lp, a.eps);
        if (a.fin_w != nullptr) wave_layernorm256_rows<RW>(v, lf, a.eps);
#pragma unroll
        for (int rr = 0; rr < RW; ++rr) {
            const int row = wave * RW + rr, s = q0 + row;
            if (s >= a.q_rows) v[rr] = make_float4(0.f, 0.f, 0.f, 0.f);
            if (a.out != nullptr && s < a.q_rows) {
                const size_t orow = a.out_mode == 1 ? (size_t)s * a.B + b : base + s;
                *reinterpret_cast<float4*>(a.out + orow * 256 + lane * 4) = v[rr];
            }
            if (has_tail) rows_to_h16(Xh, ldq, row, lane, v[rr]);
        }
    }
    LAYER_DBG(9);
    if (!has_tail) return;
    __syncthreads();
    if (a.skip_w != nullptr) {
        unsigned short* Sh = reinterpret_cast<unsigned short*>(R0);
        {
            float4 sv[RW];
#pragma unroll
            for (int rr = 0; rr < RW; ++rr) {
                const int s = q0 + wave * RW + rr;
                sv[rr] = *reinterpret_cast<const float4*>(a.skip_src + (base + (s < a.S ? s : 0)) * 256 + lane * 4);
                if (s >= a.S) sv[rr] = make_float4(0.f, 0.f, 0.f, 0.f);
            }
#pragma unroll
            for (int rr = 0; rr < RW; ++rr) rows_to_h16(Sh, ldq, wave * RW + rr, lane, sv[rr]);
        }
        const BiasRegs<NTL> bias_s = bias_load<NTL>(a.skip_b, wave * CW, 256);
        __syncthreads();
        f32x4 acc[MTL][NTL];
        acc_zero(acc);
        gemm_packed<MTL, NTL, PFW>(Xh, ldq, a.skip_w, 16, wave * NTL, 16, 8, acc, ring_t);
        gemm_packed<MTL, NTL, PFW>(Sh, ldq, a.skip_w + 8 * 64, 16, wave * NTL, 16, 8, acc);
        if (a.qkv_w != nullptr) prime_packed(ring_t, a.qkv_w, 8, wave * NTL, 48, 8);
        __syncthreads();
        acc_store_lds<MTL, NTL>(acc, Cs, ldc, wave * CW, bias_s, SEEME_ACT_NONE);
        __syncthreads();
#pragma unroll
        for (int rr = 0; rr < RW; ++rr) {
            const int row = wave * RW + rr, s = q0 + row;
            float4 v = *reinterpret_cast<const float4*>(Cs + row * ldc + lane * 4);
            if (s >= a.S) v = make_float4(0.f, 0.f, 0.f, 0.f);
            if (s < a.S) *reinterpret_cast<float4*>(a.xnext + (base + s) * 256 + lane * 4) = v;
            rows_to_h16(Xh, ldq, row, lane, v);
        }
        __syncthreads();
    }
    LAYER_DBG(10);
    if (a.qkv_w != nullptr) {
        tail_qkv_rows<WAVES, RW, PFW>(Xh, reinterpret_cast<unsigned short*>(R0), a.qkv_w, a.qkv_b, a.q_out, a.kp_out, a.vp_out, b, q0, a.S, a.spv, ring_t);
        LAYER_DBG(11);
        return;
    }
    if (a.proj_w != nullptr) {
        const int ntiles = (a.F + 15) >> 4;
        const BiasRegs<NTL> bias = bias_load<NTL>(a.proj_b, wave * CW, a.F);
        f32x4 acc[MTL][NTL];
        acc_zero(acc);
        if (wave * NTL < ntiles) gemm_packed<MTL, NTL, PFW>(Xh, ldq, a.proj_w, 8, wave * NTL, ntiles, 8, acc, ring_t);
        acc_store_lds<MTL, NTL>(acc, Cs, ldc, wave * CW, bias, SEEME_ACT_NONE);
        __syncthreads();
        for (int idx = tid; idx < ROWS * 256; idx += NT) {
            const int row = idx >> 8, c = idx & 255, s = q0 + row;
            if (s < a.S && c < a.F) a.feats[(base + s) * a.F + c] = Cs[row * ldc + c];
        }
    }
}

template <int WAVES, int RW>
static int launch_layer_w(const LayerHArgs& a, hipStream_t st) {
    constexpr int ROWS = RW * WAVES;
    if (a.z != nullptr && !layer_cvec_in<WAVES, RW>()) return seeme_fail("layer_h: this instantiation does not form the cross-attention vector");
    const size_t lds = (size_t)ROWS * (a.Sp + LDS_PAD) * 4 + (size_t)ROWS * (256 + HPAD) * 2 +
                       (layer_cvec_in<WAVES, RW>() ? (size_t)16 * (256 + HPAD) * 2 + 256 * 4 : 0);
    dim3 grid((a.q_rows + ROWS - 1) / ROWS, a.B);
    SEEME_HIP(hipFuncSetAttribute((const void*)k_layer_h<WAVES, RW>, hipFuncAttributeMaxDynamicSharedMemorySize, (int)lds));
    hipLaunchKernelGGL((k_layer_h<WAVES, RW>), grid, dim3(64 * WAVES), lds, st, a);
    return seeme_check_launch("k_layer_h");
}
static int layer_form(int B, int q_rows, int S) {
    static int rows = -1, w8_max = -1;
    if (rows < 0) { const char* e = getenv("SEEME_LAYER_ROWS"); rows = e ? atoi(e) : 32; }
    if (w8_max < 0) { const char* e = getenv("SEEME_LAYER_W8_MAX"); w8_max = e ? atoi(e) : 256; }
    const int Sp = (S + CH_N - 1) / CH_N * CH_N;
    if (rows == 64 && Sp <= 256 && q_rows > 32) return 2;
    const long wgs = (long)B * ((q_rows + 31) / 32);
    return wgs <= w8_max ? 1 : 0;
}
static bool layer_forms_cvec(int B, int q_rows, int S) { return layer_form(B, q_rows, S) == 1; }
static int launch_layer_h(const LayerHArgs& a_in, hipStream_t st) {
    LayerHArgs a = a_in;
    if (a.S <= 0 || a.S > 512) return seeme_fail("layer_h: S must be in 1..512");
    a.Sp = (a.S + CH_N - 1) / CH_N * CH_N;
    const int form = layer_form(a.B, a.q_rows, a.S);
    if (form == 2) return launch_layer_w<8, 8>(a, st);
    return form == 1 ? launch_layer_w<8, 4>(a, st) : launch_layer_w<4, 8>(a, st);
}


struct ProHArgs {
    int mode, B, S, T, F, spv;
    const float* features; const uint4* emb_w; const float* emb_b; const float* token; const float* pe;
    float* x;
    const uint4* qkv_w; const float* qkv_b; unsigned short* q_out; uint4* kp_out; uint4* vp_out;
};
__global__ __launch_bounds__(256) void k_vae_pro_h(const ProHArgs a) {
    extern __shared__ __attribute__((aligned(16))) float smem[];
    const int tid = threadIdx.x, wave = tid >> 6, lane = tid & 63;
    const int ldq = 256 + HPAD, ldc = 256 + LDS_PAD;
    float* Cs = smem;
    unsigned short* R1 = reinterpret_cast<unsigned short*>(Cs + TILE_M * ldc);
    const int b = blockIdx.y, q0 = blockIdx.x * TILE_M;
    const size_t base = (size_t)b * a.S;
    BRing<4, H16_PF> ring_t;
    if (a.mode == 1) {
        const int Kp = (a.F + 31) & ~31, lda_h = Kp + HPAD;
        const BiasRegs<4> bias = bias_load<4>(a.emb_b, wave * 64, 256);
        for (int idx = tid; idx < TILE_M * Kp; idx += 256) {
            const int row = idx / Kp, c = idx - row * Kp, s = q0 + row;
            const bool ok = s >= 2 && s < a.S && c < a.F;
            float v = a.features[ok ? ((size_t)b * a.T + (s - 2)) * a.F + c : 0];
            R1[row * lda_h + c] = f2h(ok ? v : 0.f);
        }
        __syncthreads();
        f32x4 acc[2][4];
        acc_zero(acc);
        gemm_packed<2, 4>(R1, lda_h, a.emb_w, Kp >> 5, wave * 4, 16, Kp >> 5, acc);
        acc_store_lds<2, 4>(acc, Cs, ldc, wave * 64, bias, SEEME_ACT_NONE);
    }
    prime_packed(ring_t, a.qkv_w, 8, wave * 4, 48, 8);
    __syncthreads();
    unsigned short* Xh = R1;
#pragma unroll
    for (int rr = 0; rr < 8; ++rr) {
        const int row = wave * 8 + rr, s = q0 + row, sc = s < a.S ? s : 0;
        float4 v = *reinterpret_cast<const float4*>(a.pe + (size_t)sc * 256 + lane * 4);
        if (a.mode == 1) {
            const float4 e = s < 2 ? *reinterpret_cast<const float4*>(a.token + (size_t)sc * 256 + lane * 4)
                                   : *reinterpret_cast<const float4*>(Cs + row * ldc + lane * 4);
            v = make_float4(v.x + e.x, v.y + e.y, v.z + e.z, v.w + e.w);
        }
        if (s >= a.S) v = make_float4(0.f, 0.f, 0.f, 0.f);
        else *reinterpret_cast<float4*>(a.x + (base + s) * 256 + lane * 4) = v;
        rows_to_h16(Xh, ldq, row, lane, v);
    }
    __syncthreads();
    tail_qkv_rows<4, 8, H16_PF>(Xh, reinterpret_cast<unsigned short*>(Cs), a.qkv_w, a.qkv_b, a.q_out, a.kp_out, a.vp_out, b, q0, a.S, a.spv, ring_t);
}
static int launch_pro_h(const ProHArgs& a, hipStream_t st) {
    if (a.mode == 1 && a.F > 256) return seeme_fail("vae_pro_h: nfeats > 256");
    const size_t lds = (size_t)TILE_M * (256 + LDS_PAD) * 4 + (size_t)TILE_M * (256 + HPAD) * 2;
    dim3 grid((a.S + TILE_M - 1) / TILE_M, a.B);
    SEEME_HIP(hipFuncSetAttribute((const void*)k_vae_pro_h, hipFuncAttributeMaxDynamicSharedMemorySize, (int)lds));
    hipLaunchKernelGGL(k_vae_pro_h, grid, dim3(256), lds, st, a);
    return seeme_check_launch("k_vae_pro_h");
}

__global__ void k_enc_tokens_h(const float* __restrict__ token, const float* __restrict__ pe, float* __restrict__ x, int B, int S) {
    const int idx = blockIdx.x * blockDim.x + threadIdx.x;
    if (idx >= B * 2 * 256) return;
    const int d = idx & 255, i = (idx >> 8) & 1, b = idx >> 9;
    x[((size_t)b * S + i) * 256 + d] = token[i * 256 + d] + pe[i * 256 + d];
}
__global__ void k_bcast_rows_h(const float* __restrict__ src, float* __restrict__ dst, int B, int rows) {
    const size_t idx = (size_t)blockIdx.x * blockDim.x + threadIdx.x;
    const size_t per = (size_t)rows * 64;
    if (idx >= per * B) return;
    reinterpret_cast<float4*>(dst)[idx] = reinterpret_cast<const float4*>(src)[idx % per];
}

struct WsH { float *x, *y, *sk0, *sk1, *cvec; unsigned short *qk, *vt; int spv; uint4* kp[2]; };
static WsH carve_h(void* ws, int B, int S) {
    const size_t R = (size_t)B * S;
    float* p = (float*)ws;
    WsH w;
    w.x = p; p += R * 256; w.y = p; p += R * 256; w.sk0 = p; p += R * 256; w.sk1 = p; p += R * 256;
    unsigned short* h = (unsigned short*)p;
    w.qk = h; h += R * 512;
    w.spv = (S + 31) & ~31;
    w.vt = h;
    p += R * 768;
    w.cvec = p;
    p += (size_t)B * 256 * (SEEME_NLAYERS + 1) + 64;
    w.kp[0] = reinterpret_cast<uint4*>(p);
    w.kp[1] = reinterpret_cast<uint4*>(reinterpret_cast<unsigned short*>(p) + (size_t)B * ((S + 15) & ~15) * 256);
    return w;
}

static int lin_h(hipStream_t st, const float* A, int lda, const uint16_t* wp, int K, int N, const float* bias, float* Y, int ldy,
                 int M, const float* pre_ln_w = nullptr, const float* pre_ln_b = nullptr) {
    LinearHArgs ha{};
    ha.k.a.A = A; ha.k.a.lda = lda; ha.k.a.K1 = K; ha.k.a.K = K; ha.k.a.bias = bias; ha.k.a.Y = Y; ha.k.a.ldy = ldy;
    ha.k.a.M = M; ha.k.a.N = N; ha.k.a.eps = 1e-5f; ha.k.a.pre_ln_w = pre_ln_w; ha.k.a.pre_ln_b = pre_ln_b;
    ha.wp = (const uint4*)wp; ha.kstride = ((K + 31) & ~31) >> 5; ha.ntiles = (N + 15) >> 4;
    return launch_linear_h(ha, st);
}

static int run_layer_h(hipStream_t st, const SeemeXfLayer& L, const SeemeXfLayerH& H, float* cur, float* mid, float* out, WsH& ws,
                       const int32_t* lengths, int B, int S, int n_prefix, int q_rows, const float* cvec, int cvec_ld,
                       const float* fin_w, const float* fin_b, int out_mode) {
    LinearHArgs q{};
    q.k.a.A = cur; q.k.a.lda = 256; q.k.a.K1 = 256; q.k.a.K = 256; q.k.a.bias = L.in_b; q.k.a.M = B * S; q.k.a.N = 768; q.k.a.eps = 1e-5f;
    q.wp = (const uint4*)H.in_w; q.kstride = 8; q.ntiles = 48; q.qkv_mode = 1; q.qk = ws.qk; q.vt = ws.vt; q.S = S; q.spv = ws.spv;
    int rc = ((reinterpret_cast<size_t>(cur) & 15) == 0) ? launch_qkv_h(q, st) : launch_linear_h(q, st);
    if (rc) return rc;
    AttnHArgs at{};
    at.qk = ws.qk; at.vt = ws.vt; at.res = cur; at.wo = (const uint4*)H.out_w; at.bo = L.out_b; at.ln_w = L.n1_w; at.ln_b = L.n1_b;
    at.out = mid; at.lengths = lengths; at.S = S; at.n_prefix = n_prefix; at.q_rows = q_rows; at.spv = ws.spv;
    at.scale = 1.0f / 16.0f; at.eps = 1e-5f;
    if ((rc = launch_attn_h(at, B, st))) return rc;
    FfnHArgs f{};
    f.x = mid; f.out = out; f.w1 = (const uint4*)H.l1_w; f.b1 = L.l1_b; f.w2 = (const uint4*)H.l2_w; f.b2 = L.l2_b;
    f.M = B * q_rows; f.FF = 128; f.act = SEEME_ACT_GELU; f.seq_rows = q_rows; f.seq_stride = S; f.out_mode = out_mode; f.eps = 1e-5f;
    f.fin_w = fin_w; f.fin_b = fin_b;
    if (cvec != nullptr) { f.cvec = cvec; f.cvec_ld = cvec_ld; f.lnc_w = L.n2_w; f.lnc_b = L.n2_b; f.ln_w = L.n3_w; f.ln_b = L.n3_b; }
    else { f.ln_w = L.n2_w; f.ln_b = L.n2_b; }
    return launch_ffn_h(f, st);
}

static int skip_lin_h(hipStream_t st, const float* a1, const float* a2, const uint16_t* wp, const float* b, float* y, int M) {
    LinearHArgs ha{};
    ha.k.a.A = a1; ha.k.a.lda = 256; ha.k.a.A2 = a2; ha.k.a.lda2 = 256; ha.k.a.K1 = 256; ha.k.a.K = 512; ha.k.a.bias = b;
    ha.k.a.Y = y; ha.k.a.ldy = 256; ha.k.a.M = M; ha.k.a.N = 256; ha.k.a.eps = 1e-5f;
    ha.wp = (const uint4*)wp; ha.kstride = 16; ha.ntiles = 16;
    return launch_linear_h(ha, st);
}

static void place_vt_unfused(WsH& ws, int S_carved) {
    if (ws.spv > 4 * S_carved) ws.vt = reinterpret_cast<unsigned short*>(ws.kp[0]);
}

static int vae_encode_h16_unfused(const SeemeVaeWeights* w, const float* features, const int32_t* lengths, int B, int T, float* mu,
                         void* workspace, hipStream_t st) {
    const SeemeVaeWeightsH* H = w->h16;
    const int S = T + 2, F = w->nfeats;
    WsH ws = carve_h(workspace, B, S);
    place_vt_unfused(ws, S);
    const SeemeSkipStack& E = w->enc;
    SEEME_HIP(hipMemsetAsync(ws.vt, 0, (size_t)B * 256 * ws.spv * 2, st));
    hipLaunchKernelGGL(k_enc_tokens_h, dim3((B * 512 + 255) / 256), dim3(256), 0, st, w->token, w->pe_enc, ws.x, B, S);
    int rc = seeme_check_launch("k_enc_tokens_h");
    if (rc) return rc;
    {
        LinearHArgs ha{};
        ha.k.a.A = features; ha.k.a.lda = F; ha.k.a.K1 = F; ha.k.a.K = F; ha.k.a.bias = w->emb_b; ha.k.a.res = w->pe_enc; ha.k.a.ldr = 256;
        ha.k.a.Y = ws.x; ha.k.a.ldy = 256; ha.k.a.M = B * T; ha.k.a.N = 256; ha.k.a.eps = 1e-5f;
        ha.k.seq_in = T; ha.k.in_stride = T; ha.k.out_stride = S; ha.k.out_off = 2; ha.k.res_mode = 1; ha.k.res_off = 2;
        ha.wp = (const uint4*)H->emb_w; ha.kstride = ((F + 31) & ~31) >> 5; ha.ntiles = 16;
        if ((rc = launch_linear_h(ha, st))) return rc;
    }
    if ((rc = run_layer_h(st, E.layer[0], H->enc[0], ws.x, ws.y, ws.sk0, ws, lengths, B, S, 2, S, nullptr, 0, nullptr, nullptr, 0))) return rc;
    if ((rc = run_layer_h(st, E.layer[1], H->enc[1], ws.sk0, ws.y, ws.sk1, ws, lengths, B, S, 2, S, nullptr, 0, nullptr, nullptr, 0))) return rc;
    if ((rc = run_layer_h(st, E.layer[2], H->enc[2], ws.sk1, ws.y, ws.x, ws, lengths, B, S, 2, S, nullptr, 0, nullptr, nullptr, 0))) return rc;
    if ((rc = skip_lin_h(st, ws.x, ws.sk1, H->enc_skip[0], E.skip_b[0], ws.x, B * S))) return rc;
    if ((rc = run_layer_h(st, E.layer[3], H->enc[3], ws.x, ws.y, ws.x, ws, lengths, B, S, 2, S, nullptr, 0, nullptr, nullptr, 0))) return rc;
    if ((rc = skip_lin_h(st, ws.x, ws.sk0, H->enc_skip[1], E.skip_b[1], ws.x, B * S))) return rc;
    return run_layer_h(st, E.layer[4], H->enc[4], ws.x, ws.y, mu, ws, lengths, B, S, 2, 2, nullptr, 0, E.norm_w, E.norm_b, 1);
}

static int vae_decode_h16_unfused(const SeemeVaeWeights* w, const float* z, const int32_t* lengths, int B, int T, float* feats,
                         void* workspace, hipStream_t st) {
    const SeemeVaeWeightsH* H = w->h16;
    const int S = T, F = w->nfeats;
    WsH ws = carve_h(workspace, B, S + 2);
    ws.spv = (S + 31) & ~31;
    place_vt_unfused(ws, S + 2);
    const SeemeSkipStack& Dk = w->dec;
    int rc;
    SEEME_HIP(hipMemsetAsync(ws.vt, 0, (size_t)B * 256 * ws.spv * 2, st));
    const int CL = SEEME_NLAYERS * 256;
    if ((rc = lin_h(st, z, 256, H->ca_fold_w, 256, CL, w->ca_fold_b, ws.cvec, CL, B))) return rc;
    {
        const size_t n4 = (size_t)B * S * 64;
        hipLaunchKernelGGL(k_bcast_rows_h, dim3((unsigned)((n4 + 255) / 256)), dim3(256), 0, st, w->pe_dec, ws.x, B, S);
        if ((rc = seeme_check_launch("k_bcast_rows_h"))) return rc;
    }
    if ((rc = run_layer_h(st, Dk.layer[0], H->dec[0], ws.x, ws.y, ws.sk0, ws, lengths, B, S, 0, S, ws.cvec + 0 * 256, CL, nullptr, nullptr, 0))) return rc;
    if ((rc = run_layer_h(st, Dk.layer[1], H->dec[1], ws.sk0, ws.y, ws.sk1, ws, lengths, B, S, 0, S, ws.cvec + 1 * 256, CL, nullptr, nullptr, 0))) return rc;
    if ((rc = run_layer_h(st, Dk.layer[2], H->dec[2], ws.sk1, ws.y, ws.x, ws, lengths, B, S, 0, S, ws.cvec + 2 * 256, CL, nullptr, nullptr, 0))) return rc;
    if ((rc = skip_lin_h(st, ws.x, ws.sk1, H->dec_skip[0], Dk.skip_b[0], ws.x, B * S))) return rc;
    if ((rc = run_layer_h(st, Dk.layer[3], H->dec[3], ws.x, ws.y, ws.x, ws, lengths, B, S, 0, S, ws.cvec + 3 * 256, CL, nullptr, nullptr, 0))) return rc;
    if ((rc = skip_lin_h(st, ws.x, ws.sk0, H->dec_skip[1], Dk.skip_b[1], ws.x, B * S))) return rc;
    if ((rc = run_layer_h(st, Dk.layer[4], H->dec[4], ws.x, ws.y, ws.x, ws, lengths, B, S, 0, S, ws.cvec + 4 * 256, CL, nullptr, nullptr, 0))) return rc;
    return lin_h(st, ws.x, 256, H->fin_w, 256, F, w->fin_b, feats, F, B * S, Dk.norm_w, Dk.norm_b);
}

static bool vae_fused_enabled() {
    static int v = -1;
    if (v < 0) { const char* e = getenv("SEEME_VAE_FUSED"); v = (e && e[0] == '0') ? 0 : 1; }
    return v != 0;
}
struct KvSet { unsigned short* q; uint4* kp; uint4* vp; };
static void kv_sets(const WsH& ws, int B, KvSet (&kv)[2]) {
    kv[0] = KvSet{ws.qk, ws.kp[0], reinterpret_cast<uint4*>(ws.vt)};
    kv[1] = KvSet{reinterpret_cast<unsigned short*>(ws.y), ws.kp[1], reinterpret_cast<uint4*>(ws.vt + (size_t)B * 256 * ws.spv)};
}

static LayerHArgs layer_args(const SeemeXfLayer& L, const SeemeXfLayerH& H, const KvSet& in, const float* res, const int32_t* lengths,
                             int B, int S, int spv, int n_prefix, int q_rows, const float* cvec, int cvec_ld) {
    LayerHArgs a{};
    a.q = in.q; a.kp = in.kp; a.vp = in.vp; a.res = res; a.wo = (const uint4*)H.out_w; a.bo = L.out_b; a.n1_w = L.n1_w; a.n1_b = L.n1_b;
    a.lengths = lengths; a.S = S; a.n_prefix = n_prefix; a.q_rows = q_rows; a.spv = spv; a.scale = 1.0f / 16.0f; a.eps = 1e-5f;
    a.w1 = (const uint4*)H.l1_w; a.b1 = L.l1_b; a.w2 = (const uint4*)H.l2_w; a.b2 = L.l2_b; a.B = B;
    if (cvec != nullptr) { a.cvec = cvec; a.cvec_ld = cvec_ld; a.lnc_w = L.n2_w; a.lnc_b = L.n2_b; a.n2_w = L.n3_w; a.n2_b = L.n3_b; }
    else { a.n2_w = L.n2_w; a.n2_b = L.n2_b; }
    return a;
}
static void tail_qkv(LayerHArgs& a, const SeemeXfLayer& Ln, const SeemeXfLayerH& Hn, const KvSet& out) {
// ... 112 lines not shown
```

seeme_amd/csrc/vae_kernels.hip:

```cpp
#include "common.hpp"
#include "api_util.hpp"



__global__ __launch_bounds__(256) void k_linear(const LinearKArgs ka) {
    extern __shared__ __attribute__((aligned(16))) float smem[];
    SeemeLinearArgs a = ka.a;
    if (ka.nz > 1) {
        const long z = blockIdx.z;
        a.A += z * ka.zs_a; a.W += z * ka.zs_w; a.Y += z * ka.zs_y;
        if (a.bias) a.bias += z * ka.zs_b;
        if (a.pre_ln_w) { a.pre_ln_w += z * ka.zs_ln; a.pre_ln_b += z * ka.zs_ln; }
        if (z < ka.pre_ln_zmin) { a.pre_ln_w = nullptr; a.pre_ln_b = nullptr; }
    }
    const int tid = threadIdx.x, wave = tid >> 6, lane = tid & 63;
    const int Kp = (a.K + 15) & ~15;
    const int lda_s = Kp + LDS_PAD;
    float* As = smem;
    float* Cs = smem + TILE_M * lda_s;
    const int ldc = CH_N + LDS_PAD;
    const int m0 = blockIdx.x * TILE_M;
    const int cn0 = blockIdx.y * (ka.narrow ? 64 : CH_N);

    const bool a_vec = (a.A2 == nullptr) && ((a.K & 3) == 0) && ((a.lda & 3) == 0) && ((reinterpret_cast<size_t>(a.A) & 15) == 0);
    if (a_vec) {
        const int K4 = a.K >> 2, Kp4 = Kp >> 2, total = TILE_M * Kp4;
        for (int base = 0; base < total; base += 256 * 8) {
            float4 v[8];
#pragma unroll
            for (int j = 0; j < 8; ++j) {
                const int idx = base + tid + j * 256, row = idx / Kp4, c4 = idx - row * Kp4, m = m0 + row;
                const bool valid = idx < total && m < a.M && c4 < K4;
                int prow = valid ? m : 0;
                if (ka.seq_in > 0) prow = (prow / ka.seq_in) * ka.in_stride + (prow % ka.seq_in) + ka.in_off;
                v[j] = *reinterpret_cast<const float4*>(valid ? a.A + (size_t)prow * a.lda + 4 * c4 : a.A);
                if (!valid) v[j] = make_float4(0.f, 0.f, 0.f, 0.f);
            }
#pragma unroll
            for (int j = 0; j < 8; ++j) {
                const int idx = base + tid + j * 256, row = idx / Kp4, c4 = idx - row * Kp4;
                if (idx < total) *reinterpret_cast<float4*>(As + row * lda_s + 4 * c4) = v[j];
            }
        }
    } else {
        for (int idx = tid; idx < TILE_M * Kp; idx += 256) {
            const int row = idx / Kp, c = idx - row * Kp;
            const int m = m0 + row;
            float v = 0.f;
            if (m < a.M && c < a.K) {
                int prow = m;
                if (ka.seq_in > 0) prow = (m / ka.seq_in) * ka.in_stride + (m % ka.seq_in) + ka.in_off;
                v = (c < a.K1) ? a.A[(size_t)prow * a.lda + c] : a.A2[(size_t)prow * a.lda2 + (c - a.K1)];
            }
            As[row * lda_s + c] = v;
        }
    }
    __syncthreads();
    if (a.pre_ln_w != nullptr) {
        for (int rr = 0; rr < 8; ++rr) {
            const int row = wave * 8 + rr;
            float s = 0.f;
            for (int c = lane; c < a.K; c += 64) s += As[row * lda_s + c];
            const float mean = wave_sum(s) / (float)a.K;
            float q = 0.f;
            for (int c = lane; c < a.K; c += 64) { float d = As[row * lda_s + c] - mean; q += d * d; }
            const float rs = 1.f / sqrtf(wave_sum(q) / (float)a.K + a.eps);
            for (int c = lane; c < a.K; c += 64)
                As[row * lda_s + c] = (As[row * lda_s + c] - mean) * rs * a.pre_ln_w[c] + a.pre_ln_b[c];
        }
        __syncthreads();
    }
    if (a.pre_act != SEEME_ACT_NONE) {
        for (int idx = tid; idx < TILE_M * Kp; idx += 256) {
            const int row = idx / Kp, c = idx - row * Kp;
            if (c < a.K) As[row * lda_s + c] = act_apply(As[row * lda_s + c], a.pre_act);
        }
        __syncthreads();
    }

    if (ka.narrow) {
        f32x4 acc[2][1];
        acc_zero(acc);
        const int n0 = cn0 + wave * 16;
        if (n0 < a.N) tile_gemm_f32<2, 1>(As, lda_s, a.W, a.ldw, n0, a.N, Kp >> 4, acc);
        acc_store_lds<2, 1>(acc, Cs, ldc, wave * 16, a.bias, cn0, a.N, a.act);
    } else {
        f32x4 acc[2][4];
        acc_zero(acc);
        const int n0 = cn0 + wave * 64;
        if (n0 < a.N) tile_gemm_f32<2, 4>(As, lda_s, a.W, a.ldw, n0, a.N, Kp >> 4, acc);
        acc_store_lds<2, 4>(acc, Cs, ldc, wave * 64, a.bias, cn0, a.N, a.act);
    }
    __syncthreads();

    const bool vec_ok = ((a.ldy & 3) == 0) && ((a.N & 3) == 0) && ((reinterpret_cast<size_t>(a.Y) & 15) == 0);
    const bool res_vec = a.res != nullptr && ((a.ldr & 3) == 0) && ((a.N & 3) == 0) && ((reinterpret_cast<size_t>(a.res) & 15) == 0);
    const LnParams lp = ln_params256(a.ln_w, a.ln_b);
    float4 rv[8];
#pragma unroll
    for (int rr = 0; rr < 8; ++rr) {
        rv[rr] = make_float4(0.f, 0.f, 0.f, 0.f);
        if (res_vec) {
            const int m = m0 + wave * 8 + rr, mc = m < a.M ? m : 0, g = (ka.narrow && lane >= 16) ? a.N : cn0 + lane * 4;
            int orow = mc;
            if (ka.seq_in > 0) orow = (mc / ka.seq_in) * ka.out_stride + (mc % ka.seq_in) + ka.out_off;
            const size_t rrow = ka.res_mode == 1 ? (size_t)((mc % ka.seq_in) + ka.res_off)
                              : ka.res_mode == 2 ? (size_t)(mc / ka.seq_in) : (size_t)orow;
            rv[rr] = *reinterpret_cast<const float4*>(a.res + rrow * a.ldr + (g + 3 < a.N ? g : 0));
            if (g + 3 >= a.N) rv[rr] = make_float4(0.f, 0.f, 0.f, 0.f);
        }
    }
#pragma unroll
    for (int rr = 0; rr < 8; ++rr) {
        const int row = wave * 8 + rr;
        const int m = m0 + row;
        if (m >= a.M) continue;
        int orow = m;
        if (ka.seq_in > 0) orow = (m / ka.seq_in) * ka.out_stride + (m % ka.seq_in) + ka.out_off;
        const int c = (ka.narrow && lane >= 16) ? 0 : lane * 4, g = (ka.narrow && lane >= 16) ? a.N : cn0 + c;
        float4 v = *reinterpret_cast<const float4*>(Cs + row * ldc + c);
        if (res_vec) {
            v = make_float4(v.x + rv[rr].x, v.y + rv[rr].y, v.z + rv[rr].z, v.w + rv[rr].w);
        } else if (a.res != nullptr) {
            const size_t rrow = ka.res_mode == 1 ? (size_t)((m % ka.seq_in) + ka.res_off)
                              : ka.res_mode == 2 ? (size_t)(m / ka.seq_in) : (size_t)orow;
            const float* rp = a.res + rrow * a.ldr + g;
            if (g + 0 < a.N) v.x += rp[0];
            if (g + 1 < a.N) v.y += rp[1];
            if (g + 2 < a.N) v.z += rp[2];
            if (g + 3 < a.N) v.w += rp[3];
        }
        if (a.ln_w != nullptr) v = wave_layernorm256(v, lp, a.eps);
        float* yp = a.Y + (size_t)orow * a.ldy + g;
        if (vec_ok && g + 3 < a.N) {
            *reinterpret_cast<float4*>(yp) = v;
        } else {
            if (g + 0 < a.N) yp[0] = v.x;
            if (g + 1 < a.N) yp[1] = v.y;
            if (g + 2 < a.N) yp[2] = v.z;
            if (g + 3 < a.N) yp[3] = v.w;
        }
    }
}

#define SEEME_LDS_PER_WORKGROUP 163840
#ifndef SEEME_NARROW_MIN_N
#define SEEME_NARROW_MIN_N 512
#endif
#ifndef SEEME_NARROW_MAX
#define SEEME_NARROW_MAX 64
#endif
int seeme_launch_linear(const LinearKArgs& ka, hipStream_t st) {
    const SeemeLinearArgs& a = ka.a;
    if (a.M <= 0 || a.N <= 0 || a.K <= 0) return seeme_fail("seeme_linear: empty problem");
    if (a.ln_w && a.N != 256) return seeme_fail("seeme_linear: fused LayerNorm needs N == 256");
    if (a.A2 == nullptr && a.K1 != a.K) return seeme_fail("seeme_linear: K1 must equal K without A2");
    const int Kp = (a.K + 15) & ~15;
    if (a.ldw < Kp) return seeme_fail("seeme_linear: ldw < roundup16(K) (weights must be zero padded)");
    if ((a.ldw & 3) != 0) return seeme_fail("seeme_linear: ldw must be a multiple of 4");
    const size_t lds = (size_t)(TILE_M * ((size_t)Kp + LDS_PAD) + TILE_M * (CH_N + LDS_PAD)) * sizeof(float);
    static_assert(SEEME_LINEAR_MAX_K == (SEEME_LDS_PER_WORKGROUP / (TILE_M * sizeof(float)) - (CH_N + 2 * LDS_PAD)) / 16 * 16, "header's K limit");
    if (lds > SEEME_LDS_PER_WORKGROUP) return seeme_fail("seeme_linear: K > 1008 not supported (A tile + output tile exceed the 163840 B of LDS a workgroup may have)");
    LinearKArgs k2 = ka;
    const long wide = (long)((a.M + TILE_M - 1) / TILE_M) * ((a.N + CH_N - 1) / CH_N) * (ka.nz > 1 ? ka.nz : 1);
    k2.narrow = (a.ln_w == nullptr && a.N >= SEEME_NARROW_MIN_N && wide <= SEEME_NARROW_MAX) ? 1 : 0;
    const int cw = k2.narrow ? 64 : CH_N;
    dim3 grid((a.M + TILE_M - 1) / TILE_M, (a.N + cw - 1) / cw, ka.nz > 1 ? ka.nz : 1);
    SEEME_HIP(hipFuncSetAttribute((const void*)k_linear, hipFuncAttributeMaxDynamicSharedMemorySize, (int)lds));
    hipLaunchKernelGGL(k_linear, grid, dim3(256), lds, st, k2);
    return seeme_check_launch("k_linear");
}

extern "C" int seeme_linear(const SeemeLinearArgs* args, void* stream) {
    LinearKArgs ka{};
    ka.a = *args;
    if (ka.a.A2 == nullptr) ka.a.K1 = ka.a.K;
    return seeme_launch_linear(ka, (hipStream_t)stream);
}

static int linear_simple(hipStream_t st, const float* A, int lda, const float* W, int ldw, const float* bias,
                         float* Y, int ldy, int M, int N, int K, int act = SEEME_ACT_NONE,
                         int pre_act = SEEME_ACT_NONE, const float* pre_ln_w = nullptr,
                         const float* pre_ln_b = nullptr) {
    LinearKArgs ka{};
    ka.a.A = A; ka.a.lda = lda; ka.a.K1 = K; ka.a.W = W; ka.a.ldw = ldw; ka.a.bias = bias;
    ka.a.Y = Y; ka.a.ldy = ldy; ka.a.M = M; ka.a.N = N; ka.a.K = K; ka.a.act = act; ka.a.pre_act = pre_act;
    ka.a.pre_ln_w = pre_ln_w; ka.a.pre_ln_b = pre_ln_b; ka.a.eps = 1e-5f;
    return seeme_launch_linear(ka, st);
}
int seeme_linear_simple(hipStream_t st, const float* A, int lda, const float* W, int ldw, const float* bias,
                        float* Y, int ldy, int M, int N, int K, int act, int pre_act,
                        const float* pre_ln_w, const float* pre_ln_b) {
    return linear_simple(st, A, lda, W, ldw, bias, Y, ldy, M, N, K, act, pre_act, pre_ln_w, pre_ln_b);
}

struct AttnKArgs {
    const float* qkv;
    const float* res;
    const float* wo; const float* bo; const float* ln_w; const float* ln_b;
    float* out;
    const int32_t* lengths;
    int S;
    int n_prefix;
    int q_rows;
    int Sp;
    float scale;
    float eps;
};

template <int NC>
__device__ __forceinline__ void attn_softmax_rows_f32(float* Ps, int ldp, int wave, int lane) {
    float v[8][NC], mx[8], sum[8];
#pragma unroll
    for (int rr = 0; rr < 8; ++rr) {
        const float* prow = Ps + (wave * 8 + rr) * ldp + lane;
        mx[rr] = -INFINITY;
#pragma unroll
        for (int j = 0; j < NC; ++j) { v[rr][j] = prow[64 * j]; mx[rr] = fmaxf(mx[rr], v[rr][j]); }
    }
#pragma unroll
    for (int rr = 0; rr < 8; ++rr) mx[rr] = wave_max(mx[rr]);
#pragma unroll
    for (int rr = 0; rr < 8; ++rr) {
        sum[rr] = 0.f;
#pragma unroll
        for (int j = 0; j < NC; ++j) { v[rr][j] = expf(v[rr][j] - mx[rr]); sum[rr] += v[rr][j]; }
    }
#pragma unroll
    for (int rr = 0; rr < 8; ++rr) sum[rr] = wave_sum(sum[rr]);
#pragma unroll
    for (int rr = 0; rr < 8; ++rr) {
        const float inv = 1.f / sum[rr];
        float* prow = Ps + (wave * 8 + rr) * ldp + lane;
#pragma unroll
        for (int j = 0; j < NC; ++j) prow[64 * j] = v[rr][j] * inv;
    }
}

__global__ __launch_bounds__(256) void k_attn_block(const AttnKArgs a) {
    extern __shared__ __attribute__((aligned(16))) float smem[];
    const int tid = threadIdx.x, wave = tid >> 6, lane = tid & 63, r = lane & 15, kq = lane >> 4;
    const int ldq = 256 + LDS_PAD, ldp = a.Sp + LDS_PAD;
    float* Qs = smem;
    float* Ps = smem + TILE_M * ldq;
    int b = blockIdx.y, qt = blockIdx.x;
    if ((gridDim.y & 7) == 0) {
        const int L = blockIdx.x + gridDim.x * blockIdx.y, r = L & 7, q = L >> 3;
        b = r + 8 * (q / (int)gridDim.x);
        qt = q % (int)gridDim.x;
    }
    const int q0 = qt * TILE_M;
    const size_t base = (size_t)b * a.S;
    const int n_valid_keys = min(a.S, a.n_prefix + a.lengths[b]);

    {
        float4 qv[8];
#pragma unroll
        for (int it = 0; it < 8; ++it) {
            const int idx = tid + it * 256, row = idx >> 6, c4 = (idx & 63) * 4, s = q0 + row;
            qv[it] = *reinterpret_cast<const float4*>(a.qkv + (base + (s < a.q_rows ? s : 0)) * 768 + c4);
            if (s >= a.q_rows) qv[it] = make_float4(0.f, 0.f, 0.f, 0.f);
        }
#pragma unroll
        for (int it = 0; it < 8; ++it) {
            const int idx = tid + it * 256, row = idx >> 6, c4 = (idx & 63) * 4;
            *reinterpret_cast<float4*>(Qs + row * ldq + c4) = qv[it];
        }
    }
    __syncthreads();

    const float* Kmat = a.qkv + base * 768 + 256;
    for (int c0 = 0; c0 < a.Sp; c0 += CH_N) {
        const int n0 = c0 + wave * 64;
        f32x4 acc[2][4];
        acc_zero(acc);
        if (n0 < a.S) tile_gemm_f32<2, 4>(Qs, ldq, Kmat, 768, n0, a.S, 16, acc);
#pragma unroll
        for (int nt = 0; nt < 4; ++nt) {
            const int c = n0 + nt * 16 + r;
            const bool ok = c < n_valid_keys;
#pragma unroll
            for (int mt = 0; mt < 2; ++mt)
#pragma unroll
                for (int i = 0; i < 4; ++i)
                    Ps[(mt * 16 + 4 * kq + i) * ldp + c] = ok ? acc[mt][nt][i] * a.scale : -INFINITY;
        }
    }
    __syncthreads();

    if (a.Sp == 256) attn_softmax_rows_f32<4>(Ps, ldp, wave, lane);
    else attn_softmax_rows_f32<8>(Ps, ldp, wave, lane);
    __syncthreads();

    {
        f32x4 acc[2][4];
// ... 279 lines not shown
```

seeme_amd/mld_denoiser.py:

```python
from __future__ import annotations

import ctypes as C
import math
import os
from typing import Optional

import torch
import torch.nn as nn

from . import _lib as L
from .mld_vae import _PositionEmbeddingLearned1D, _EncoderLayerParams, _SkipStackParams, _param_fingerprint

_LAYER_FIELDS = ["skip", "inp", "outp", "l1", "l2", "caq", "cao", "f1", "f2", "fo",
                 "skip_b", "in_b", "out_b", "n1w", "n1b", "l1b", "l2b", "n2w", "n2b", "cnw", "cnb", "caq_b",
                 "csnw", "csnb", "cao_b", "f1b", "f2b", "fsnw", "fsnb", "fo_b"]


_CUS = {}


def _device_cus(device) -> int:
    idx = torch.device(device).index
    idx = torch.cuda.current_device() if idx is None else idx
    if idx not in _CUS:
        _CUS[idx] = int(torch.cuda.get_device_properties(idx).multi_processor_count)
    return _CUS[idx]


def timestep_features(timesteps: torch.Tensor, dim: int = 256, flip_sin_to_cos: bool = True,
                      freq_shift: float = 0.0, max_period: int = 10000) -> torch.Tensor:
    assert timesteps.dim() == 1
    half = dim // 2
    exponent = -math.log(max_period) * torch.arange(0, half, dtype=torch.float32, device=timesteps.device)
    exponent = exponent / (half - freq_shift)
    emb = timesteps[:, None].float() * torch.exp(exponent)[None, :]
    emb = torch.cat([torch.sin(emb), torch.cos(emb)], dim=-1)
    if flip_sin_to_cos:
        emb = torch.cat([emb[:, half:], emb[:, :half]], dim=-1)
    if dim % 2 == 1:
        emb = torch.nn.functional.pad(emb, (0, 1, 0, 0))
    return emb


def cluster_pack_stage(Wsub: torch.Tensor, TPW: int, KL: int, UL: int) -> torch.Tensor:
    EPL = KL // 4
    NT, K = Wsub.shape[0] // 16, Wsub.shape[1]
    assert NT == 8 * TPW and K % KL == 0 and (K // KL * TPW) % UL == 0
    KB = K // KL
    t = Wsub.reshape(NT, 16, KB, 4, EPL).permute(0, 2, 3, 1, 4).reshape(8, TPW, KB, 64, EPL)
    t = t.permute(0, 2, 1, 3, 4).reshape(8, (KB * TPW) // UL, UL, 64, EPL)
    return t.permute(1, 0, 2, 3, 4)


class _TimestepEmbeddingParams(nn.Module):
    def __init__(self, channel, time_embed_dim):
        super().__init__()
        self.linear_1 = nn.Linear(channel, time_embed_dim)
        self.linear_2 = nn.Linear(time_embed_dim, time_embed_dim)


class _StylizationParams(nn.Module):

    def __init__(self, d, t):
        super().__init__()
        self.emb_layers = nn.Sequential(nn.SiLU(), nn.Linear(t, 2 * d))
        self.norm = nn.LayerNorm(d)
        self.out_layers = nn.Sequential(nn.SiLU(), nn.Dropout(p=0.0), nn.Linear(d, d))


class _CrossAttnParams(nn.Module):
    def __init__(self, d, t):
        super().__init__()
        self.norm = nn.LayerNorm(d)
        self.text_norm = nn.LayerNorm(d)
        self.query = nn.Linear(d, d)
        self.key = nn.Linear(d, d)
        self.value = nn.Linear(d, d)
        self.proj_out = _StylizationParams(d, t)


class _FFNParams(nn.Module):
    def __init__(self, d, ff, t):
        super().__init__()
        self.linear1 = nn.Linear(d, ff)
        self.linear2 = nn.Linear(ff, d)
        self.proj_out = _StylizationParams(d, t)


class _MDLayerParams(nn.Module):

    def __init__(self, d, ff, nhead, dropout):
        super().__init__()
        self.d_model = d
        self.ca_block = _CrossAttnParams(d, d)
        self.ffn = _FFNParams(d, ff, d)
        self.sa_block = _EncoderLayerParams(d, nhead, 1024, dropout)


class MldDenoiser(nn.Module):

    def __init__(self,
                 ablation,
                 nfeats: int = 72,
                 condition: str = "text",
                 latent_dim: list = [1, 256],
                 ff_size: int = 128,
                 num_layers: int = 6,
                 num_heads: int = 4,
                 dropout: float = 0.1,
                 normalize_before: bool = False,
                 activation: str = "gelu",
                 flip_sin_to_cos: bool = True,
                 return_intermediate_dec: bool = False,
                 position_embedding: str = "learned",
                 arch: str = "trans_enc",
                 freq_shift: int = 0,
                 guidance_scale: float = 7.5,
                 guidance_uncondp: float = 0.1,
                 text_encoded_dim: int = 256,
                 nclasses: int = 10,
                 weight_dtype: str = "fp32",
                 cluster="auto",
                 **kwargs) -> None:
        super().__init__()
        self.latent_dim = latent_dim[-1]
        self.text_encoded_dim = text_encoded_dim
        self.condition = condition
        self.arch = arch
        self.pe_type = ablation.DIFF_PE_TYPE
        self.MD_trans = ablation.MD_TRANS
        self.flip_sin_to_cos, self.freq_shift = flip_sin_to_cos, freq_shift
        self.num_heads, self.ff_size, self.num_layers = num_heads, ff_size, num_layers
        if "text" not in self.condition:
            raise TypeError(f"condition type {self.condition} not supported")
        if self.pe_type != "mld":
            if self.pe_type == "actor":
                raise NotImplementedError("DIFF_PE_TYPE 'actor' is outside the accelerated path")
            raise ValueError("Not Support PE type")
        if arch != "trans_enc":
            if arch == "trans_dec":
                raise NotImplementedError("arch 'trans_dec' is outside the accelerated path")
            raise ValueError(f"Not supported architechure{self.arch}!")
        if ablation.VAE_TYPE == "no" or not ablation.SKIP_CONNECT or not self.MD_trans:
            raise NotImplementedError("accelerated path: VAE latent + SKIP_CONNECT + MD_TRANS (all SEE-ME configs)")
        if text_encoded_dim != self.latent_dim or self.latent_dim != 256 or latent_dim[0] != 1 or num_layers != 5:
            raise NotImplementedError("accelerated path: latent_dim [1,256], text_encoded_dim 256, 5 layers")
        if num_heads not in (1, 2, 4):
            raise NotImplementedError("accelerated path: num_heads in {1,2,4}")
        if weight_dtype not in ("fp32", "bf16", "fp16"):
            raise ValueError("weight_dtype must be 'fp32', 'bf16' or 'fp16'")
        self.weight_dtype = weight_dtype
        if cluster not in ("auto", 0, 2, 4, 8):
            raise ValueError("cluster must be 'auto', 0, 2, 4 or 8")
        self.cluster = cluster
        self.cluster_placement = 1
        self.cluster_flags = 0
        self.cluster_ms = True
        self.pack_xcds = "auto"

        d = self.latent_dim
        self.time_embedding = _TimestepEmbeddingParams(text_encoded_dim, d)
        self.query_pos = _PositionEmbeddingLearned1D(d)
        self.mem_pos = _PositionEmbeddingLearned1D(d)
        self.encoder = _SkipStackParams(lambda: _MDLayerParams(d, ff_size, num_heads, dropout), num_layers, d)

        self._wcache = None
        self._ws = L.Workspace(per_stream=False)
        self._table_cache = {}
        self._ccache = {}
        self._xchg = None

    def _layout(self):
        n = 5 * len(_LAYER_FIELDS) + 5
        buf = (C.c_int64 * n)()
        L.call("seeme_den_layout", 1024, self.ff_size, buf, n)
        vals = list(buf)
        layers = [dict(zip(_LAYER_FIELDS, vals[i * 30:(i + 1) * 30])) for i in range(5)]
        pe0, fnw, fnb, wg_total, vp_total = vals[150:155]
        self._layout_vals = vals
        return layers, pe0, fnw, fnb, wg_total, vp_total

    def _weights(self):
        fpnt = (_param_fingerprint(self), self.weight_dtype)
        if self._wcache is not None and self._wcache[0] == fpnt:
            return self._wcache[1]
        for p in self.parameters():
            L.require_cuda(p, "MldDenoiser parameter")
        dev = self.query_pos.pe.device
        layers, pe0, fnw, fnb, wg_total, vp_total = self._layout()
        bf16 = self.weight_dtype != "fp32"
        KV = 8 if bf16 else 4
        wdt = {"fp32": torch.float32, "bf16": torch.bfloat16, "fp16": torch.float16}[self.weight_dtype]
        wg = torch.zeros(wg_total, dtype=wdt, device=dev)
        vp = torch.zeros(vp_total, dtype=torch.float32, device=dev)

        def put_w(off, W):
            N, K = W.shape
            if bf16:
                TW, KB = N // 128, K // 32
                TG = 4 if TW % 4 == 0 else (3 if TW % 3 == 0 else (2 if TW % 2 == 0 else 1))
                g = W.detach().reshape(8, TW // TG, TG, 16, KB, 4, 8).permute(0, 1, 4, 2, 5, 3, 6).reshape(-1)
            else:
                g = W.detach().reshape(N, K // KV, KV).permute(1, 0, 2).reshape(-1)
            wg[off:off + g.numel()] = g.to(wg.dtype)

        def put_v(off, v):
            vp[off:off + v.numel()] = v.detach().reshape(-1)

        blocks = self.encoder.blocks()
        fold = self.num_heads == 1

        def sa_in_proj(sa):
            Wi, bi = sa.self_attn.in_proj_weight.detach(), sa.self_attn.in_proj_bias.detach()
            if not fold:
                return Wi, bi
            Wo, bo = sa.self_attn.out_proj.weight.detach().double(), sa.self_attn.out_proj.bias.detach().double()
            Wu = (Wo @ Wi[512:].double()).float()
            bu = (Wo @ bi[512:].double() + bo).float()
            return torch.cat([Wi[:512], Wu]), torch.cat([bi[:512], bu])

        with torch.no_grad():
            in_proj = [sa_in_proj(b.sa_block) for b in blocks]
            put_v(pe0, self.query_pos.pe[0, 0])
            put_v(fnw, self.encoder.norm.weight)
            put_v(fnb, self.encoder.norm.bias)
            for l, (blk, o) in enumerate(zip(blocks, layers)):
                sa, ca, ffn = blk.sa_block, blk.ca_block, blk.ffn
                if l >= 3:
                    put_w(o["skip"], self.encoder.linear_blocks[l - 3].weight)
                    put_v(o["skip_b"], self.encoder.linear_blocks[l - 3].bias)
                put_w(o["inp"], in_proj[l][0]); put_v(o["in_b"], in_proj[l][1])
                if not fold:
                    put_w(o["outp"], sa.self_attn.out_proj.weight); put_v(o["out_b"], sa.self_attn.out_proj.bias)
                put_w(o["l1"], sa.linear1.weight); put_v(o["l1b"], sa.linear1.bias)
                put_w(o["l2"], sa.linear2.weight); put_v(o["l2b"], sa.linear2.bias)
                put_v(o["n1w"], sa.norm1.weight); put_v(o["n1b"], sa.norm1.bias)
                put_v(o["n2w"], sa.norm2.weight); put_v(o["n2b"], sa.norm2.bias)
                put_v(o["cnw"], ca.norm.weight); put_v(o["cnb"], ca.norm.bias)
                put_w(o["caq"], ca.query.weight); put_v(o["caq_b"], ca.query.bias)
                put_v(o["csnw"], ca.proj_out.norm.weight); put_v(o["csnb"], ca.proj_out.norm.bias)
                put_w(o["cao"], ca.proj_out.out_layers[2].weight); put_v(o["cao_b"], ca.proj_out.out_layers[2].bias)
                put_w(o["f1"], ffn.linear1.weight); put_v(o["f1b"], ffn.linear1.bias)
                put_w(o["f2"], ffn.linear2.weight); put_v(o["f2b"], ffn.linear2.bias)
                put_v(o["fsnw"], ffn.proj_out.norm.weight); put_v(o["fsnb"], ffn.proj_out.norm.bias)
                put_w(o["fo"], ffn.proj_out.out_layers[2].weight); put_v(o["fo_b"], ffn.proj_out.out_layers[2].bias)
            kv_w = torch.cat([in_proj[l][0][256:] for l in range(len(blocks))]).contiguous()
            kv_b = torch.cat([in_proj[l][1][256:] for l in range(len(blocks))]).contiguous()
            st_w = torch.cat([torch.cat([b.ca_block.proj_out.emb_layers[1].weight, b.ffn.proj_out.emb_layers[1].weight])
                              for b in blocks]).contiguous()
            st_b = torch.cat([torch.cat([b.ca_block.proj_out.emb_layers[1].bias, b.ffn.proj_out.emb_layers[1].bias])
                              for b in blocks]).contiguous()
            ca_w = [torch.cat([b.ca_block.key.weight, b.ca_block.value.weight]).contiguous() for b in blocks]
            ca_b = [torch.cat([b.ca_block.key.bias, b.ca_block.value.bias]).contiguous() for b in blocks]
            cf_w = torch.cat([ca_w[l] * blk.ca_block.text_norm.weight[None, :] for l, blk in enumerate(blocks)]).contiguous()
            cf_b = torch.cat([ca_w[l] @ blk.ca_block.text_norm.bias + ca_b[l] for l, blk in enumerate(blocks)]).contiguous()
            ones, zeros = torch.ones(256, device=dev), torch.zeros(256, device=dev)
        lay_dev = torch.tensor(self._layout_vals, dtype=torch.int64, device=dev)
        w = L.DenoiserWeights()
        w.wg, w.wdtype, w.vp, w.layout = wg.data_ptr(), {"fp32": 0, "bf16": 1, "fp16": 2}[self.weight_dtype], vp.data_ptr(), lay_dev.data_ptr()
        w.nhead, w.ff_sa, w.ff = self.num_heads, 1024, self.ff_size
        w.kv_cat_w, w.kv_cat_b, w.style_cat_w, w.style_cat_b = kv_w.data_ptr(), kv_b.data_ptr(), st_w.data_ptr(), st_b.data_ptr()
        te = self.time_embedding
        w.time_w1, w.time_b1 = L.ptr(te.linear_1.weight), L.ptr(te.linear_1.bias)
        w.time_w2, w.time_b2 = L.ptr(te.linear_2.weight), L.ptr(te.linear_2.bias)
        for l, b in enumerate(blocks):
            w.ca_kv_w[l], w.ca_kv_b[l] = ca_w[l].data_ptr(), ca_b[l].data_ptr()
            w.ca_tn_w[l], w.ca_tn_b[l] = L.ptr(b.ca_block.text_norm.weight), L.ptr(b.ca_block.text_norm.bias)
        with torch.no_grad():
            pn_w = torch.stack([b.ca_block.proj_out.norm.weight for b in blocks]).contiguous()
            pn_b = torch.stack([b.ca_block.proj_out.norm.bias for b in blocks]).contiguous()
            po_w = torch.stack([b.ca_block.proj_out.out_layers[2].weight for b in blocks]).contiguous()
            po_b = torch.stack([b.ca_block.proj_out.out_layers[2].bias for b in blocks]).contiguous()
        w.ca_pn_w, w.ca_pn_b, w.ca_po_w, w.ca_po_b = pn_w.data_ptr(), pn_b.data_ptr(), po_w.data_ptr(), po_b.data_ptr()
        w.sa_fold = int(fold)
        w.ca_fold_w, w.ca_fold_b, w.ln_ones, w.ln_zeros = cf_w.data_ptr(), cf_b.data_ptr(), ones.data_ptr(), zeros.data_ptr()
        self._ccache = {}
        self._fold_parts = (in_proj, vp, layers)
        self._wcache = (fpnt, w, (wg, vp, kv_w, kv_b, st_w, st_b, ca_w, ca_b, lay_dev, cf_w, cf_b, ones, zeros, pn_w, pn_b, po_w, po_b))
        self._table_cache = {}
        return w

    def _cluster_weights(self, Cc: int, query: bool = False):
        self._weights()
        if (Cc, query) in self._ccache:
            return self._ccache[(Cc, query)]
        in_proj, vp, layers = self._fold_parts
        dev = vp.device
        code = {"fp32": 0, "bf16": 1, "fp16": 2}[self.weight_dtype]
        wdt = {"fp32": torch.float32, "bf16": torch.bfloat16, "fp16": torch.float16}[self.weight_dtype]
        lo = (C.c_int64 * 14)()
        L.call("seeme_den_cluster_layout", Cc, code, int(query), lo, 14)
        NU, UB, total, UL, KL = (int(v) for v in lo[:5])
        U_D, U_G, U_H = int(lo[9]), int(lo[12]), int(lo[13])
        EPL = KL // 4
        S, NB, TA, TB = 256 // Cc, 1024 // Cc, 256 // Cc // 32, 8 // Cc

        def pack_stage(Wsub, TPW):
            return cluster_pack_stage(Wsub, TPW, KL, UL)

        blocks = self.encoder.blocks()
        img = torch.zeros(5, Cc, NU, 8, UL, 64, EPL, dtype=wdt, device=dev)
        vpc = vp.clone()
        with torch.no_grad():
            for l, (blk, o) in enumerate(zip(blocks, layers)):
                Wq, bq = in_proj[l][0].double(), in_proj[l][1].double()
                if l >= 3:
                    Ws = self.encoder.linear_blocks[l - 3].weight.detach().double()
                    bs = self.encoder.linear_blocks[l - 3].bias.detach().double()
                    Wa = torch.cat([Wq @ Ws, Ws])
                    vpc[o["in_b"]:o["in_b"] + 768] = (Wq @ bs + bq).float()
                else:
                    Wa = torch.cat([Wq, torch.zeros(256, 256, dtype=torch.float64, device=dev)])
                W1, W2 = blk.sa_block.linear1.weight.detach(), blk.sa_block.linear2.weight.detach()
                Wf1, Wf2 = blk.ffn.linear1.weight.detach(), blk.ffn.linear2.weight.detach()
                Wfo = blk.ffn.proj_out.out_layers[2].weight.detach()
                for c in range(Cc):
                    rows = torch.cat([torch.arange(p * 256 + c * S, p * 256 + (c + 1) * S, device=dev) for p in range(4)])
                    ua = pack_stage(Wa[rows].to(wdt), TA)
                    img[l, c, 0:ua.shape[0]] = ua
                    img[l, c, 2 * TA:2 * TA + TB] = pack_stage(W1[c * NB:(c + 1) * NB].to(wdt), TB)
                    img[l, c, 2 * TA + TB:2 * TA + 2 * TB] = pack_stage(W2[:, c * NB:(c + 1) * NB].to(wdt), 2)
                    if query:
                        Wq_ca = blk.ca_block.query.weight.detach()[c * S:(c + 1) * S]
                        Wq_pad = torch.zeros(128, 256, dtype=Wq_ca.dtype, device=dev)
                        Wq_pad[:S] = Wq_ca
                        img[l, c, U_G:U_G + 1] = pack_stage(Wq_pad.to(wdt), 1)
                        img[l, c, U_H:U_H + 2] = pack_stage(blk.ca_block.proj_out.out_layers[2].weight.detach().to(wdt), 2)
                    u0 = U_D
                    img[l, c, u0:u0 + 1] = pack_stage(Wf1.to(wdt), 1)
                    img[l, c, u0 + 1:u0 + 2] = pack_stage(Wf2.to(wdt), 2)
                    img[l, c, u0 + 2:u0 + 4] = pack_stage(Wfo.to(wdt), 2)
        assert img.numel() * img.element_size() == total
        self._ccache[(Cc, query)] = (img, vpc, code)
        return self._ccache[(Cc, query)]

    def _cluster_size(self, B: int, N: int, cfg: bool, cus: int = 256) -> int:
        want = os.environ.get("SEEME_DEN_CLUSTER")
        want = self.cluster if want is None else (want if want == "auto" else int(want))
        if want == 0 or N > 2 or cfg or self.num_heads != 1:
            return 0
        Bp = (B + 7) // 8 * 8
        cus = min(int(cus), 256)
        if want == "auto":
            for Cc in (8, 4, 2):
                if Bp * Cc <= cus:
                    return Cc
            return 0
        return want if Bp * want <= cus else 0

    def _cluster_plan(self, B: int, N: int, cfg: bool, per_sample: bool, cus: int = 256):
        Cc = self._cluster_size(B, N, cfg, cus)
        want = os.environ.get("SEEME_DEN_CLUSTER")
        want = self.cluster if want is None else (want if want == "auto" else int(want))
        ms = os.environ.get("SEEME_DEN_CLUSTER_MS", "1") != "0" and self.cluster_ms
        forced = os.environ.get("SEEME_DEN_CLUSTER_MS_PLAN")
        if (want != "auto" or not ms or (B <= 32 and not forced) or N not in (1, 2) or cfg or per_sample or self.num_heads != 1
                or self.weight_dtype not in ("fp16", "bf16")):
            return Cc, 1
        if forced:
            C4, spc = (int(x) for x in forced.split(","))
            return C4, spc
        cus = min(int(cus), 256)
        if B <= 64 and Cc == 4:
            return Cc, 1
        ncl = (cus // 4) // 8 * 8
        most = 4 if self.weight_dtype == "bf16" else (8 if N == 1 else 6)
        if ncl >= 8 and -(-B // ncl) <= most:
            return 4, max(2, -(-B // ncl))
        return Cc, 1

    def cluster_status(self):
        if self._xchg is None:
            return (0, 0)
        hdr = self._xchg[:8].cpu().view(torch.int32)
        return int(hdr[0]), int(hdr[1])

    def _workspace(self, rows: int, device):
        return self._ws.get(L.lib().seeme_denoiser_workspace_bytes(rows, 0, 0), device)

    def time_tables(self, tfeat: torch.Tensor) -> torch.Tensor:
        L.require_cuda(tfeat, "tfeat")
        tfeat = tfeat.contiguous()
        rows = tfeat.shape[0]
        ttab = torch.empty(rows, L.TROW, device=tfeat.device, dtype=torch.float32)
        ws = self._workspace(rows, tfeat.device)
        w = self._weights()
        L.call("seeme_denoiser_time_tables", C.byref(w), tfeat.data_ptr(), rows, ttab.data_ptr(), ws.data_ptr(), ws.numel(),
               L.current_stream())
        return ttab

    def cond_tables(self, cond_bf: torch.Tensor) -> torch.Tensor:
        L.require_cuda(cond_bf, "condition")
        cond_bf = cond_bf.contiguous()
        Bc, N, _ = cond_bf.shape
        ctab = torch.empty(Bc, N, L.CROW, device=cond_bf.device, dtype=torch.float32)
        w = self._weights()
        L.call("seeme_denoiser_cond_tables", C.byref(w), cond_bf.data_ptr(), Bc, N, ctab.data_ptr(), 0, 0, L.current_stream())
        return ctab

    def ca_tables(self, ctab: torch.Tensor, ttab: torch.Tensor, trow: torch.Tensor, per_sample: bool) -> torch.Tensor:
        Bc = ctab.shape[0]
        R = 1 if per_sample else trow.numel()
        catab = torch.empty(Bc, R, 5, self.latent_dim, device=ctab.device, dtype=torch.float32)
        ws = torch.empty(5 * Bc * R * 256, device=ctab.device, dtype=torch.float32)
        w = self._weights()
        L.call("seeme_denoiser_ca_tables", C.byref(w), ctab.data_ptr(), ttab.data_ptr(), trow.data_ptr(), int(per_sample),
               trow.numel(), Bc, catab.data_ptr(), ws.data_ptr(), ws.numel() * 4, L.current_stream())
        return catab

    def _launch(self, latents2d, ctab, ttab, trow, per_sample, steps, sched, coef, noise, cfg, guidance):
        B, N = latents2d.shape[0], ctab.shape[1]
        out = torch.empty(B, self.latent_dim, device=latents2d.device, dtype=torch.float32)
        a = L.SampleArgs()
        a.B, a.N, a.steps, a.sched, a.cfg, a.guidance_scale = B, N, steps, sched, int(cfg), float(guidance)
        a.latents, a.ctab, a.ttab, a.trow, a.trow_per_sample = latents2d.data_ptr(), ctab.data_ptr(), ttab.data_ptr(), trow.data_ptr(), int(per_sample)
        a.coef, a.noise, a.out = L.ptr(coef), L.ptr(noise), out.data_ptr()
        catab = self.ca_tables(ctab, ttab, trow, per_sample) if N == 1 else None
        a.catab = L.ptr(catab)
        a.xcds = L.default_xcds((B + 1) // 2 if (B > 256 and not per_sample and not cfg) else B, self.pack_xcds)
        w = self._weights()
        Cc, spc = self._cluster_plan(B, N, bool(cfg), bool(per_sample), _device_cus(latents2d.device))
        if Cc:
            img, vpc, code = self._cluster_weights(Cc, N > 1)
            need = (L.lib().seeme_den_cluster_ms_xchg_bytes(B, Cc, spc) if spc > 1 else L.lib().seeme_den_cluster_xchg_bytes(B, Cc))
            if self._xchg is None or self._xchg.numel() < need or self._xchg.device != latents2d.device:
                self._xchg = torch.zeros(need, dtype=torch.uint8, device=latents2d.device)
            cl = L.DenCluster()
            cl.wgc, cl.wdtype, cl.vpc, cl.C = img.data_ptr(), code, vpc.data_ptr(), Cc
            cl.placement = int(os.environ.get("SEEME_DEN_CLUSTER_PLACE", self.cluster_placement))
            cl.flags = int(os.environ.get("SEEME_DEN_CLUSTER_FLAGS", self.cluster_flags))
            cl.xchg, cl.xchg_bytes = self._xchg.data_ptr(), self._xchg.numel()
            cl.query = int(N > 1)
            cl.samples = spc
            L.call("seeme_denoiser_sample_cluster", C.byref(w), C.byref(cl), C.byref(a), L.current_stream())
            return out
        L.call("seeme_denoiser_sample", C.byref(w), C.byref(a), L.current_stream())
        return out

    def forward(self, sample, timestep, encoder_hidden_states, lengths=None, **kwargs):
        L.require_cuda(sample, "sample")
        L.require_cuda(encoder_hidden_states, "encoder_hidden_states")
        B = sample.shape[0]
        if sample.shape[1] != 1:
            raise NotImplementedError("accelerated path: one latent token (latent_dim [1,256])")
        t = torch.as_tensor(timestep)
        per_sample = t.dim() > 0 and t.numel() > 1
        t1 = t.reshape(-1) if per_sample else t.reshape(1)
        tfeat = timestep_features(t1.to(sample.device), self.text_encoded_dim, self.flip_sin_to_cos, self.freq_shift)
        ttab = self.time_tables(tfeat.to(torch.float32))
        trow = (torch.arange(B, dtype=torch.int32, device=sample.device) if per_sample
                else torch.zeros(max(B, 1), dtype=torch.int32, device=sample.device))
        ctab = self.cond_tables(encoder_hidden_states.permute(1, 0, 2))
        out = self._launch(sample.reshape(B, -1).contiguous(), ctab, ttab, trow, True, 1, L.SCHED_NONE,
                           None, None, False, 1.0)
        return (out.reshape(B, 1, self.latent_dim),)

    def sample_loop(self, latents: torch.Tensor, cond_bf: torch.Tensor, scheduler, eta: float = 0.0,
                    guidance_scale: float = 1.0, step_noise: Optional[torch.Tensor] = None,
                    events=None) -> torch.Tensor:
        L.require_cuda(latents, "latents")
        B = latents.shape[0]
        cfg = guidance_scale > 1.0
        if cond_bf.shape[0] != (2 * B if cfg else B):
            raise ValueError("condition batch must be B (or 2B with classifier-free guidance)")
        dev = latents.device
        key = (tuple(scheduler.timesteps.tolist()), float(eta), type(scheduler).__name__)
        self._weights()
        cached = self._table_cache.get(key)
        if cached is None:
            tfeat = timestep_features(scheduler.timesteps.cpu(), self.text_encoded_dim, self.flip_sin_to_cos,
                                      self.freq_shift).to(dev)
            coef = scheduler.coef_table(eta).to(dev)
            trow = torch.arange(len(scheduler.timesteps), dtype=torch.int32, device=dev)
            cached = (tfeat, coef, trow, self.time_tables(tfeat))
            self._table_cache = {key: cached}
        tfeat, coef, trow, ttab = cached
        ctab = self.cond_tables(cond_bf)
        steps = len(trow)
        noise = None
        if scheduler.needs_noise(eta):
            if step_noise is None:
                step_noise = torch.randn(steps, B, self.latent_dim, device=dev, dtype=torch.float32)
            noise = step_noise.reshape(steps, B, self.latent_dim).contiguous()
        sched = L.SCHED_DDIM if type(scheduler).__name__.startswith("DDIM") else L.SCHED_DDPM
        lat2 = latents.reshape(B, -1).contiguous()
        if events is not None:
            events[0].record()
        out = self._launch(lat2, ctab, ttab, trow, False, steps, sched, coef, noise, cfg, guidance_scale)
        if events is not None:
            events[1].record()
        return out.reshape(1, B, self.latent_dim)
```

Before: 17510 seqs/s.

## Fuse condition and cross-attention table prep into one kernel launch

Adds a single k_den_prep kernel that computes the condition key/value tables and the per-step cross-attention tables together, replacing separate cond_tables and ca_tables launches. The shared tile logic moves into a reusable linear_tile header so the linear kernel and the fused kernel can share it. The VAE tail QKV GEMM also gains optional bias preloading and next-GEMM weight prefetching. The aim is to cut launch count and intermediate workspace round-trips in the per-call prep. In exchange the fused kernel recomputes the folded-weight GEMM for each layer and timestep block, and it only applies when N==1 and the batch is at most 32.

```diff
diff --git a/include/seeme_hip.h b/include/seeme_hip.h
--- a/include/seeme_hip.h
+++ b/include/seeme_hip.h
@@ -120,6 +120,10 @@
 int seeme_denoiser_ca_tables(const SeemeDenoiserWeights* w, const float* ctab, const float* ttab, const int32_t* trow,
                              int trow_per_sample, int n_trow, int Bc, float* catab,
                              void* workspace, size_t ws_bytes, void* stream);
+
+#define SEEME_COND_PREP_MAX_BC 64
+int seeme_denoiser_cond_prep(const SeemeDenoiserWeights* w, const float* cond, int Bc, int N, const float* ttab,
+                             const int32_t* trow, int trow_per_sample, int n_trow, float* ctab, float* catab, void* stream);
 
 typedef struct {
     int B;
diff --git a/seeme_amd/_lib.py b/seeme_amd/_lib.py
--- a/seeme_amd/_lib.py
+++ b/seeme_amd/_lib.py
@@ -191,6 +191,7 @@
     "seeme_denoiser_time_tables": (C.c_int, [C.POINTER(DenoiserWeights), fp, C.c_int, fp, fp, C.c_size_t, fp]),
     "seeme_denoiser_cond_tables": (C.c_int, [C.POINTER(DenoiserWeights), fp, C.c_int, C.c_int, fp, fp, C.c_size_t, fp]),
     "seeme_denoiser_ca_tables": (C.c_int, [C.POINTER(DenoiserWeights), fp, fp, fp, C.c_int, C.c_int, C.c_int, fp, fp, C.c_size_t, fp]),
+    "seeme_denoiser_cond_prep": (C.c_int, [C.POINTER(DenoiserWeights), fp, C.c_int, C.c_int, fp, fp, C.c_int, C.c_int, fp, fp, fp]),
     "seeme_denoiser_sample": (C.c_int, [C.POINTER(DenoiserWeights), C.POINTER(SampleArgs), fp]),
     "seeme_denoiser_sample_cluster": (C.c_int, [C.POINTER(DenoiserWeights), C.POINTER(DenCluster), C.POINTER(SampleArgs), fp]),
     "seeme_den_cluster_xchg_bytes": (C.c_size_t, [C.c_int, C.c_int]),
diff --git a/seeme_amd/csrc/den_kernels.hip b/seeme_amd/csrc/den_kernels.hip
--- a/seeme_amd/csrc/den_kernels.hip
+++ b/seeme_amd/csrc/den_kernels.hip
@@ -1,6 +1,7 @@
 #include <atomic>
 #include "common.hpp"
 #include "api_util.hpp"
+#include "linear_tile.hpp"
 #include "den_layout.h"
 #include "lds_ring.hpp"
 #include "den_train.h"
@@ -966,6 +967,87 @@
     return seeme_launch_linear(ka, st);
 }
 
+struct DenPrepArgs {
+    LinearKArgs k0;
+    int n1, mt, R, Bc;
+    const float* cf_w; const float* cf_b;
+    const float* pn_w; const float* pn_b; const float* po_w; const float* po_b;
+    const float* ttab; const int32_t* trow; float* catab;
+};
+__global__ __launch_bounds__(256) void k_den_prep(const DenPrepArgs P) {
+    extern __shared__ __attribute__((aligned(16))) float smem[];
+    const int idx = blockIdx.x;
+    if (idx >= P.n1) {
+        const int i0 = idx - P.n1, ny = (P.k0.a.N + 63) / 64;
+        linear_tile(P.k0, i0 % P.mt, (i0 / P.mt) % ny, i0 / (P.mt * ny), smem);
+        return;
+    }
+    const int tid = threadIdx.x, wave = tid >> 6, lane = tid & 63;
+    const int m0 = (idx % P.mt) * TILE_M, r = (idx / P.mt) % P.R, l = idx / (P.mt * P.R);
+    const int lda_s = 256 + LDS_PAD, ldc = CH_N + LDS_PAD;
+    float* As = smem;
+    float* Cs = smem + TILE_M * lda_s;
+    const float* tt = P.ttab + (size_t)P.trow[r] * SEEME_TROW + 2560 + l * 1024;
+    const float4 scl = ld4(tt + 4 * lane), shf = ld4(tt + 256 + 4 * lane);
+    SeemeLinearArgs a = P.k0.a;
+    linear_stage_a(a, P.k0, m0, As, lda_s, 256);
+    {
+        f32x4 acc[2][4];
+        acc_zero(acc);
+        tile_gemm_f32<2, 4>(As, lda_s, P.cf_w, 256, l * 512 + 256 + wave * 64, 2560, 16, acc);
+        acc_store_lds<2, 4>(acc, Cs, ldc, wave * 64, P.cf_b, l * 512 + 256, 2560, SEEME_ACT_NONE);
+    }
+    __syncthreads();
+#pragma unroll
+    for (int rr = 0; rr < 8; ++rr) {
+        const int row = wave * 8 + rr;
+        const float4 hn = wave_ln(ld4(Cs + row * ldc + 4 * lane), P.pn_w + l * 256, P.pn_b + l * 256, lane);
+        const float4 h = f4_silu(f4_adaln(hn, scl, shf));
+        st4(As + row * lda_s + 4 * lane, m0 + row < P.Bc ? h : make_float4(0.f, 0.f, 0.f, 0.f));
+    }
+    __syncthreads();
+    {
+        f32x4 acc[2][4];
+        acc_zero(acc);
+        tile_gemm_f32<2, 4>(As, lda_s, P.po_w + (size_t)l * 256 * 256, 256, wave * 64, 256, 16, acc);
+        acc_store_lds<2, 4>(acc, Cs, ldc, wave * 64, P.po_b + l * 256, 0, 256, SEEME_ACT_NONE);
+    }
+    __syncthreads();
+#pragma unroll
+    for (int rr = 0; rr < 8; ++rr) {
+        const int row = wave * 8 + rr, m = m0 + row;
+        if (m < P.Bc) st4(P.catab + (((size_t)m * P.R + r) * SEEME_DEN_NL + l) * 256 + 4 * lane, ld4(Cs + row * ldc + 4 * lane));
+    }
+}
+
+extern "C" int seeme_denoiser_cond_prep(const SeemeDenoiserWeights* w, const float* cond, int Bc, int N, const float* ttab,
+                                        const int32_t* trow, int trow_per_sample, int n_trow, float* ctab, float* catab,
+                                        void* stream) {
+    hipStream_t st = (hipStream_t)stream;
+    if (N != 1) return seeme_fail("cond_prep: one condition token only (N == 1); use cond_tables + ca_tables");
+    if (trow_per_sample) return seeme_fail("cond_prep: shared table rows only (trow_per_sample == 0); use cond_tables + ca_tables");
+    if (Bc <= 0 || Bc > SEEME_COND_PREP_MAX_BC) return seeme_fail("cond_prep: Bc must be in 1..64; use cond_tables + ca_tables");
+    if (n_trow <= 0) return seeme_fail("cond_prep: empty row list");
+    if (w->ca_fold_w == nullptr) return seeme_fail("cond_prep: folded key/value weights missing");
+    if (w->ca_pn_w == nullptr || w->ca_po_w == nullptr) return seeme_fail("cond_prep: proj_out weights missing");
+    DenPrepArgs P{};
+    LinearKArgs& ka = P.k0;
+    ka.a.A = cond; ka.a.lda = 256; ka.a.K1 = 256; ka.a.K = 256; ka.a.W = w->kv_cat_w; ka.a.ldw = 256; ka.a.bias = w->kv_cat_b;
+    ka.a.Y = ctab; ka.a.ldy = SEEME_CROW; ka.a.M = Bc; ka.a.N = 2560; ka.a.eps = 1e-5f;
+    ka.a.pre_ln_w = w->ln_ones; ka.a.pre_ln_b = w->ln_zeros;
+    ka.nz = 2; ka.zs_a = 0; ka.zs_w = (long)(w->ca_fold_w - w->kv_cat_w); ka.zs_b = (long)(w->ca_fold_b - w->kv_cat_b); ka.zs_y = 2560;
+    ka.zs_ln = 0; ka.pre_ln_zmin = 1;
+    ka.narrow = 1;
+    P.mt = (Bc + TILE_M - 1) / TILE_M; P.R = n_trow; P.Bc = Bc; P.n1 = SEEME_DEN_NL * n_trow * P.mt;
+    P.cf_w = w->ca_fold_w; P.cf_b = w->ca_fold_b; P.pn_w = w->ca_pn_w; P.pn_b = w->ca_pn_b; P.po_w = w->ca_po_w; P.po_b = w->ca_po_b;
+    P.ttab = ttab; P.trow = trow; P.catab = catab;
+    const int n0 = P.mt * (2560 / 64) * 2;
+    const size_t lds = (size_t)(TILE_M * (256 + LDS_PAD) + TILE_M * (CH_N + LDS_PAD)) * sizeof(float);
+    SEEME_HIP(hipFuncSetAttribute((const void*)k_den_prep, hipFuncAttributeMaxDynamicSharedMemorySize, (int)lds));
+    hipLaunchKernelGGL(k_den_prep, dim3(P.n1 + n0), dim3(256), lds, st, P);
+    return seeme_check_launch("k_den_prep");
+}
+
 #ifdef DEN_DBG_TIMES
 extern "C" int seeme_debug_den_times(unsigned long long* host, int n) {
     SEEME_HIP(hipMemcpyFromSymbol(host, HIP_SYMBOL(den_dbg_times), sizeof(unsigned long long) * (size_t)(n < 512 ? n : 512)));
diff --git a/seeme_amd/csrc/linear_tile.hpp b/seeme_amd/csrc/linear_tile.hpp
--- /dev/null
+++ b/seeme_amd/csrc/linear_tile.hpp
@@ -0,0 +1,149 @@
+#pragma once
+#include "common.hpp"
+#include "api_util.hpp"
+
+__device__ __forceinline__ void linear_stage_a(const SeemeLinearArgs& a, const LinearKArgs& ka, int m0, float* As, int lda_s, int Kp) {
+    const int tid = threadIdx.x, wave = tid >> 6, lane = tid & 63;
+    const bool a_vec = (a.A2 == nullptr) && ((a.K & 3) == 0) && ((a.lda & 3) == 0) && ((reinterpret_cast<size_t>(a.A) & 15) == 0);
+    if (a_vec) {
+        const int K4 = a.K >> 2, Kp4 = Kp >> 2, total = TILE_M * Kp4;
+        for (int base = 0; base < total; base += 256 * 8) {
+            float4 v[8];
+#pragma unroll
+            for (int j = 0; j < 8; ++j) {
+                const int idx = base + tid + j * 256, row = idx / Kp4, c4 = idx - row * Kp4, m = m0 + row;
+                const bool valid = idx < total && m < a.M && c4 < K4;
+                int prow = valid ? m : 0;
+                if (ka.seq_in > 0) prow = (prow / ka.seq_in) * ka.in_stride + (prow % ka.seq_in) + ka.in_off;
+                v[j] = *reinterpret_cast<const float4*>(valid ? a.A + (size_t)prow * a.lda + 4 * c4 : a.A);
+                if (!valid) v[j] = make_float4(0.f, 0.f, 0.f, 0.f);
+            }
+#pragma unroll
+            for (int j = 0; j < 8; ++j) {
+                const int idx = base + tid + j * 256, row = idx / Kp4, c4 = idx - row * Kp4;
+                if (idx < total) *reinterpret_cast<float4*>(As + row * lda_s + 4 * c4) = v[j];
+            }
+        }
+    } else {
+        for (int idx = tid; idx < TILE_M * Kp; idx += 256) {
+            const int row = idx / Kp, c = idx - row * Kp;
+            const int m = m0 + row;
+            float v = 0.f;
+            if (m < a.M && c < a.K) {
+                int prow = m;
+                if (ka.seq_in > 0) prow = (m / ka.seq_in) * ka.in_stride + (m % ka.seq_in) + ka.in_off;
+                v = (c < a.K1) ? a.A[(size_t)prow * a.lda + c] : a.A2[(size_t)prow * a.lda2 + (c - a.K1)];
+            }
+            As[row * lda_s + c] = v;
+        }
+    }
+    __syncthreads();
+    if (a.pre_ln_w != nullptr) {
+        for (int rr = 0; rr < 8; ++rr) {
+            const int row = wave * 8 + rr;
+            float s = 0.f;
+            for (int c = lane; c < a.K; c += 64) s += As[row * lda_s + c];
+            const float mean = wave_sum(s) / (float)a.K;
+            float q = 0.f;
+            for (int c = lane; c < a.K; c += 64) { float d = As[row * lda_s + c] - mean; q += d * d; }
+            const float rs = 1.f / sqrtf(wave_sum(q) / (float)a.K + a.eps);
+            for (int c = lane; c < a.K; c += 64)
+                As[row * lda_s + c] = (As[row * lda_s + c] - mean) * rs * a.pre_ln_w[c] + a.pre_ln_b[c];
+        }
+        __syncthreads();
+    }
+    if (a.pre_act != SEEME_ACT_NONE) {
+        for (int idx = tid; idx < TILE_M * Kp; idx += 256) {
+            const int row = idx / Kp, c = idx - row * Kp;
+            if (c < a.K) As[row * lda_s + c] = act_apply(As[row * lda_s + c], a.pre_act);
+        }
+        __syncthreads();
+    }
+
+}
+
+__device__ __forceinline__ void linear_tile(const LinearKArgs& ka, int bx, int by, int bz, float* smem) {
+    SeemeLinearArgs a = ka.a;
+    if (ka.nz > 1) {
+        const long z = bz;
+        a.A += z * ka.zs_a; a.W += z * ka.zs_w; a.Y += z * ka.zs_y;
+        if (a.bias) a.bias += z * ka.zs_b;
+        if (a.pre_ln_w) { a.pre_ln_w += z * ka.zs_ln; a.pre_ln_b += z * ka.zs_ln; }
+        if (z < ka.pre_ln_zmin) { a.pre_ln_w = nullptr; a.pre_ln_b = nullptr; }
+    }
+    const int tid = threadIdx.x, wave = tid >> 6, lane = tid & 63;
+    const int Kp = (a.K + 15) & ~15;
+    const int lda_s = Kp + LDS_PAD;
+    float* As = smem;
+    float* Cs = smem + TILE_M * lda_s;
+    const int ldc = CH_N + LDS_PAD;
+    const int m0 = bx * TILE_M;
+    const int cn0 = by * (ka.narrow ? 64 : CH_N);
+
+
+    linear_stage_a(a, ka, m0, As, lda_s, Kp);
+
+    if (ka.narrow) {
+        f32x4 acc[2][1];
+        acc_zero(acc);
+        const int n0 = cn0 + wave * 16;
+        if (n0 < a.N) tile_gemm_f32<2, 1>(As, lda_s, a.W, a.ldw, n0, a.N, Kp >> 4, acc);
+        acc_store_lds<2, 1>(acc, Cs, ldc, wave * 16, a.bias, cn0, a.N, a.act);
+    } else {
+        f32x4 acc[2][4];
+        acc_zero(acc);
+        const int n0 = cn0 + wave * 64;
+        if (n0 < a.N) tile_gemm_f32<2, 4>(As, lda_s, a.W, a.ldw, n0, a.N, Kp >> 4, acc);
+        acc_store_lds<2, 4>(acc, Cs, ldc, wave * 64, a.bias, cn0, a.N, a.act);
+    }
+    __syncthreads();
+
+    const bool vec_ok = ((a.ldy & 3) == 0) && ((a.N & 3) == 0) && ((reinterpret_cast<size_t>(a.Y) & 15) == 0);
+    const bool res_vec = a.res != nullptr && ((a.ldr & 3) == 0) && ((a.N & 3) == 0) && ((reinterpret_cast<size_t>(a.res) & 15) == 0);
+    const LnParams lp = ln_params256(a.ln_w, a.ln_b);
+    float4 rv[8];
+#pragma unroll
+    for (int rr = 0; rr < 8; ++rr) {
+        rv[rr] = make_float4(0.f, 0.f, 0.f, 0.f);
+        if (res_vec) {
+            const int m = m0 + wave * 8 + rr, mc = m < a.M ? m : 0, g = (ka.narrow && lane >= 16) ? a.N : cn0 + lane * 4;
+            int orow = mc;
+            if (ka.seq_in > 0) orow = (mc / ka.seq_in) * ka.out_stride + (mc % ka.seq_in) + ka.out_off;
+            const size_t rrow = ka.res_mode == 1 ? (size_t)((mc % ka.seq_in) + ka.res_off)
+                              : ka.res_mode == 2 ? (size_t)(mc / ka.seq_in) : (size_t)orow;
+            rv[rr] = *reinterpret_cast<const float4*>(a.res + rrow * a.ldr + (g + 3 < a.N ? g : 0));
+            if (g + 3 >= a.N) rv[rr] = make_float4(0.f, 0.f, 0.f, 0.f);
+        }
+    }
+#pragma unroll
+    for (int rr = 0; rr < 8; ++rr) {
+        const int row = wave * 8 + rr;
+        const int m = m0 + row;
+        if (m >= a.M) continue;
+        int orow = m;
+        if (ka.seq_in > 0) orow = (m / ka.seq_in) * ka.out_stride + (m % ka.seq_in) + ka.out_off;
+        const int c = (ka.narrow && lane >= 16) ? 0 : lane * 4, g = (ka.narrow && lane >= 16) ? a.N : cn0 + c;
+        float4 v = *reinterpret_cast<const float4*>(Cs + row * ldc + c);
+        if (res_vec) {
+            v = make_float4(v.x + rv[rr].x, v.y + rv[rr].y, v.z + rv[rr].z, v.w + rv[rr].w);
+        } else if (a.res != nullptr) {
+            const size_t rrow = ka.res_mode == 1 ? (size_t)((m % ka.seq_in) + ka.res_off)
+                              : ka.res_mode == 2 ? (size_t)(m / ka.seq_in) : (size_t)orow;
+            const float* rp = a.res + rrow * a.ldr + g;
+            if (g + 0 < a.N) v.x += rp[0];
+            if (g + 1 < a.N) v.y += rp[1];
+            if (g + 2 < a.N) v.z += rp[2];
+            if (g + 3 < a.N) v.w += rp[3];
+        }
+        if (a.ln_w != nullptr) v = wave_layernorm256(v, lp, a.eps);
+        float* yp = a.Y + (size_t)orow * a.ldy + g;
+        if (vec_ok && g + 3 < a.N) {
+            *reinterpret_cast<float4*>(yp) = v;
+        } else {
+            if (g + 0 < a.N) yp[0] = v.x;
+            if (g + 1 < a.N) yp[1] = v.y;
+            if (g + 2 < a.N) yp[2] = v.z;
+            if (g + 3 < a.N) yp[3] = v.w;
+        }
+    }
+}
diff --git a/seeme_amd/csrc/vae_h16.hip b/seeme_amd/csrc/vae_h16.hip
--- a/seeme_amd/csrc/vae_h16.hip
+++ b/seeme_amd/csrc/vae_h16.hip
@@ -1,5 +1,6 @@
 #include "common.hpp"
 #include "api_util.hpp"
+#include <type_traits>
 
 typedef _Float16 h16x8 __attribute__((ext_vector_type(8)));
 #define HPAD 16
@@ -46,9 +47,10 @@
         for (int nt = 0; nt < NTL; ++nt) ring.br[u][nt] = loadb(nt, u < K32 ? u : K32 - 1);
 }
 
-template <int MTL, int NTL, int PF, typename LoadB>
+struct NoNextGemm {};
+template <int MTL, int NTL, int PF, typename LoadB, typename LoadN = NoNextGemm>
 __device__ __forceinline__ void tile_gemm_h16(const unsigned short* __restrict__ As, int lda, int K32, LoadB loadb,
-                                              f32x4 (&acc)[MTL][NTL], BRing<NTL, PF>& ring) {
+                                              f32x4 (&acc)[MTL][NTL], BRing<NTL, PF>& ring, LoadN loadn = LoadN{}) {
     const int lane = threadIdx.x & 63, r = lane & 15, kq = lane >> 4;
     const unsigned short* ap = As + r * lda + 8 * kq;
     uint4 (&br)[PF][NTL] = ring.br;
@@ -95,6 +97,10 @@
                     acc[mt][nt] = __builtin_amdgcn_mfma_f32_16x16x32_f16(__builtin_bit_cast(h16x8, ab[u % AS][mt]), __builtin_bit_cast(h16x8, br[u][nt]), acc[mt][nt], 0, 0, 0);
         }
         __builtin_amdgcn_sched_barrier(0);
+        if constexpr (!std::is_same<LoadN, NoNextGemm>::value) {
+#pragma unroll
+            for (int nt = 0; nt < NTL; ++nt) br[u][nt] = loadn(nt, u);
+        }
     }
 }
 struct PackedSrc {
@@ -787,11 +793,20 @@
         if (kb < KB) vb_out[((size_t)nt * KB + kb) * 64 + g * 16 + r] = make_uint4(w[0], w[1], w[2], w[3]);
     }
 }
-template <int WAVES, int RW, int PF>
+template <int NTL>
+struct TailBias { BiasRegs<NTL> v[3]; };
+template <int WAVES>
+__device__ __forceinline__ TailBias<16 / WAVES> tail_bias_load(const float* __restrict__ qkv_b) {
+    TailBias<16 / WAVES> t;
+#pragma unroll
+    for (int p = 0; p < 3; ++p) t.v[p] = bias_load<16 / WAVES>(qkv_b, p * 256 + (int)(threadIdx.x >> 6) * (256 / WAVES), 768);
+    return t;
+}
+template <int WAVES, int RW, int PF, bool PRE>
 __device__ __forceinline__ void tail_qkv_rows(const unsigned short* Xh, unsigned short* Oh, const uint4* __restrict__ qkv_w,
                                               const float* __restrict__ qkv_b, unsigned short* __restrict__ q_out,
                                               uint4* __restrict__ kp_out, uint4* __restrict__ vp_out, int b, int q0, int S, int spv,
-                                              BRing<16 / WAVES, PF>& ring_t) {
+                                              BRing<16 / WAVES, PF>& ring_t, const TailBias<16 / WAVES>& pre) {
     constexpr int ROWS = RW * WAVES, MTL = ROWS / 16, NTL = 16 / WAVES, CW = 256 / WAVES;
     const int tid = threadIdx.x, wave = tid >> 6;
     const int ldq = 256 + HPAD;
@@ -802,24 +817,32 @@
     {
         f32x4 acc[MTL][NTL];
         acc_zero(acc);
-        const BiasRegs<NTL> bias = bias_load<NTL>(qkv_b, 0 * 256 + wave * CW, 768);
-        gemm_packed<MTL, NTL, PF>(Xh, ldq, qkv_w, 8, 0 * 16 + wave * NTL, 48, 8, acc, ring_t);
-        prime_packed(ring_t, qkv_w, 8, 1 * 16 + wave * NTL, 48, 8);
+        const BiasRegs<NTL> bias = PRE ? pre.v[0] : bias_load<NTL>(qkv_b, 0 * 256 + wave * CW, 768);
+        if constexpr (PRE) {
+            tile_gemm_h16<MTL, NTL, PF>(Xh, ldq, 8, PackedSrc(qkv_w, 8, 0 * 16 + wave * NTL, 48), acc, ring_t, PackedSrc(qkv_w, 8, 1 * 16 + wave * NTL, 48));
+        } else {
+            gemm_packed<MTL, NTL, PF>(Xh, ldq, qkv_w, 8, 0 * 16 + wave * NTL, 48, 8, acc, ring_t);
+            prime_packed(ring_t, qkv_w, 8, 1 * 16 + wave * NTL, 48, 8);
+        }
         __syncthreads();
         acc_store_h16<MTL, NTL>(acc, Oh, ldq, wave * CW, bias, SEEME_ACT_NONE);
     }
     {
         f32x4 acc[MTL][NTL];
         acc_zero(acc);
-        const BiasRegs<NTL> bias = bias_load<NTL>(qkv_b, 1 * 256 + wave * CW, 768);
-        gemm_packed<MTL, NTL, PF>(Xh, ldq, qkv_w, 8, 1 * 16 + wave * NTL, 48, 8, acc, ring_t);
-        prime_packed(ring_t, qkv_w, 8, 2 * 16 + wave * NTL, 48, 8);
+        const BiasRegs<NTL> bias = PRE ? pre.v[1] : bias_load<NTL>(qkv_b, 1 * 256 + wave * CW, 768);
+        if constexpr (PRE) {
+            tile_gemm_h16<MTL, NTL, PF>(Xh, ldq, 8, PackedSrc(qkv_w, 8, 1 * 16 + wave * NTL, 48), acc, ring_t, PackedSrc(qkv_w, 8, 2 * 16 + wave * NTL, 48));
+        } else {
+            gemm_packed<MTL, NTL, PF>(Xh, ldq, qkv_w, 8, 1 * 16 + wave * NTL, 48, 8, acc, ring_t);
+            prime_packed(ring_t, qkv_w, 8, 2 * 16 + wave * NTL, 48, 8);
+        }
         acc_store_h16<MTL, NTL>(acc, OhK, ldk, wave * CW, bias, SEEME_ACT_NONE);
     }
     {
         f32x4 acc[MTL][NTL];
         acc_zero(acc);
-        const BiasRegs<NTL> bias = bias_load<NTL>(qkv_b, 2 * 256 + wave * CW, 768);
+        const BiasRegs<NTL> bias = PRE ? pre.v[2] : bias_load<NTL>(qkv_b, 2 * 256 + wave * CW, 768);
         gemm_packed<MTL, NTL, PF>(Xh, ldq, qkv_w, 8, 2 * 16 + wave * NTL, 48, 8, acc, ring_t);
         __syncthreads();
         tail_store_q<WAVES, RW>(Oh, ldq, q_out, base, q0, S);
@@ -829,6 +852,15 @@
         __syncthreads();
         tail_store_v<WAVES, RW>(Oh, ldq, vp_out, b, q0, S, KB);
     }
+}
+
+template <int WAVES, int RW, int PF>
+__device__ __forceinline__ void tail_qkv_rows(const unsigned short* Xh, unsigned short* Oh, const uint4* __restrict__ qkv_w,
+                                              const float* __restrict__ qkv_b, unsigned short* __restrict__ q_out,
+                                              uint4* __restrict__ kp_out, uint4* __restrict__ vp_out, int b, int q0, int S, int spv,
+                                              BRing<16 / WAVES, PF>& ring_t) {
+    TailBias<16 / WAVES> none;
+    tail_qkv_rows<WAVES, RW, PF, false>(Xh, Oh, qkv_w, qkv_b, q_out, kp_out, vp_out, b, q0, S, spv, ring_t, none);
 }
 
 #define LAYER_DBG(i) do { if (a.qkv_w != nullptr) H16_DBG(5, i); } while (0)
@@ -1129,7 +1161,10 @@
     float* x;
     const uint4* qkv_w; const float* qkv_b; unsigned short* q_out; uint4* kp_out; uint4* vp_out;
 };
-__global__ __launch_bounds__(256) void k_vae_pro_h(const ProHArgs a) {
+template <int WAVES, int RW>
+__global__ __launch_bounds__(64 * WAVES, WAVES == 4 ? 3 : 1) void k_vae_pro_h(const ProHArgs a) {
+    constexpr int ROWS = RW * WAVES, MTL = ROWS / 16, NTL = 16 / WAVES, CW = 256 / WAVES, NT = 64 * WAVES;
+    static_assert(ROWS == TILE_M, "one 32-row tile per workgroup");
     extern __shared__ __attribute__((aligned(16))) float smem[];
     const int tid = threadIdx.x, wave = tid >> 6, lane = tid & 63;
     const int ldq = 256 + HPAD, ldc = 256 + LDS_PAD;
@@ -1137,32 +1172,76 @@
     unsigned short* R1 = reinterpret_cast<unsigned short*>(Cs + TILE_M * ldc);
     const int b = blockIdx.y, q0 = blockIdx.x * TILE_M;
     const size_t base = (size_t)b * a.S;
-    BRing<4, H16_PF> ring_t;
+    const int Kp = (a.F + 31) & ~31, lda_h = Kp + HPAD;
+    constexpr bool TWO_RINGS = WAVES == 8;
+    constexpr int PFE = TWO_RINGS ? 8 : H16_PF;
+    BRing<NTL, PFE> ring_e;
+    BRing<NTL, H16_PF> ring_t;
+    if constexpr (TWO_RINGS) {
+        if (a.mode == 1) prime_packed(ring_e, a.emb_w, Kp >> 5, wave * NTL, 16, Kp >> 5);
+        prime_packed(ring_t, a.qkv_w, 8, wave * NTL, 48, 8);
+    } else {
+        if (a.mode == 1) prime_packed(ring_t, a.emb_w, Kp >> 5, wave * NTL, 16, Kp >> 5);
+        else prime_packed(ring_t, a.qkv_w, 8, wave * NTL, 48, 8);
+    }
+    float4 tk[2];
+#pragma unroll
+    for (int i = 0; i < 2; ++i) tk[i] = *reinterpret_cast<const float4*>((a.token != nullptr ? a.token + i * 256 : a.pe) + lane * 4);
+    const BiasRegs<NTL> bias = bias_load<NTL>(a.emb_b, wave * CW, 256);
+    const TailBias<NTL> bias_t = tail_bias_load<WAVES>(a.qkv_b);
+    constexpr bool PE_EARLY = WAVES == 8;
+    float4 pv[RW];
+    if constexpr (PE_EARLY) {
+#pragma unroll
+        for (int rr = 0; rr < RW; ++rr) {
+            const int s = q0 + wave * RW + rr;
+            pv[rr] = *reinterpret_cast<const float4*>(a.pe + (size_t)(s < a.S ? s : 0) * 256 + lane * 4);
+        }
+    }
+    __builtin_amdgcn_sched_barrier(0);
     if (a.mode == 1) {
-        const int Kp = (a.F + 31) & ~31, lda_h = Kp + HPAD;
-        const BiasRegs<4> bias = bias_load<4>(a.emb_b, wave * 64, 256);
-        for (int idx = tid; idx < TILE_M * Kp; idx += 256) {
-            const int row = idx / Kp, c = idx - row * Kp, s = q0 + row;
-            const bool ok = s >= 2 && s < a.S && c < a.F;
-            float v = a.features[ok ? ((size_t)b * a.T + (s - 2)) * a.F + c : 0];
-            R1[row * lda_h + c] = f2h(ok ? v : 0.f);
-        }
-        __syncthreads();
-        f32x4 acc[2][4];
+        if ((a.F & 3) == 0 && (reinterpret_cast<size_t>(a.features) & 15) == 0) {
+            const int F4 = a.F >> 2, Kp4 = Kp >> 2;
+            float4 v[RW];
+#pragma unroll
+            for (int rr = 0; rr < RW; ++rr) {
+                const int s = q0 + wave * RW + rr;
+                const bool ok = s >= 2 && s < a.S && lane < F4;
+                v[rr] = *reinterpret_cast<const float4*>(a.features + (ok ? ((size_t)b * a.T + (s - 2)) * a.F + 4 * lane : 0));
+                if (!ok) v[rr] = make_float4(0.f, 0.f, 0.f, 0.f);
+            }
+            __builtin_amdgcn_sched_barrier(0);
+            if (lane < Kp4) {
+#pragma unroll
+                for (int rr = 0; rr < RW; ++rr) {
+                    const unsigned lo = (unsigned)f2h(v[rr].x) | ((unsigned)f2h(v[rr].y) << 16), hi = (unsigned)f2h(v[rr].z) | ((unsigned)f2h(v[rr].w) << 16);
+                    *reinterpret_cast<uint2*>(R1 + (wave * RW + rr) * lda_h + 4 * lane) = make_uint2(lo, hi);
+                }
+            }
+        } else {
+            for (int idx = tid; idx < TILE_M * Kp; idx += NT) {
+                const int row = idx / Kp, c = idx - row * Kp, s = q0 + row;
+                const bool ok = s >= 2 && s < a.S && c < a.F;
+                float v = a.features[ok ? ((size_t)b * a.T + (s - 2)) * a.F + c : 0];
+                R1[row * lda_h + c] = f2h(ok ? v : 0.f);
+            }
+        }
+        __syncthreads();
+        f32x4 acc[MTL][NTL];
         acc_zero(acc);
-        gemm_packed<2, 4>(R1, lda_h, a.emb_w, Kp >> 5, wave * 4, 16, Kp >> 5, acc);
-        acc_store_lds<2, 4>(acc, Cs, ldc, wave * 64, bias, SEEME_ACT_NONE);
-    }
-    prime_packed(ring_t, a.qkv_w, 8, wave * 4, 48, 8);
+        if constexpr (TWO_RINGS) gemm_packed<MTL, NTL, PFE>(R1, lda_h, a.emb_w, Kp >> 5, wave * NTL, 16, Kp >> 5, acc, ring_e);
+        else tile_gemm_h16<MTL, NTL, H16_PF>(R1, lda_h, Kp >> 5, PackedSrc(a.emb_w, Kp >> 5, wave * NTL, 16), acc, ring_t, PackedSrc(a.qkv_w, 8, wave * NTL, 48));
+        acc_store_lds<MTL, NTL>(acc, Cs, ldc, wave * CW, bias, SEEME_ACT_NONE);
+    }
     __syncthreads();
     unsigned short* Xh = R1;
 #pragma unroll
-    for (int rr = 0; rr < 8; ++rr) {
-        const int row = wave * 8 + rr, s = q0 + row, sc = s < a.S ? s : 0;
-        float4 v = *reinterpret_cast<const float4*>(a.pe + (size_t)sc * 256 + lane * 4);
+    for (int rr = 0; rr < RW; ++rr) {
+        const int row = wave * RW + rr, s = q0 + row, sc = s < a.S ? s : 0;
+        float4 v = PE_EARLY ? pv[rr] : *reinterpret_cast<const float4*>(a.pe + (size_t)sc * 256 + lane * 4);
         if (a.mode == 1) {
-            const float4 e = s < 2 ? *reinterpret_cast<const float4*>(a.token + (size_t)sc * 256 + lane * 4)
-                                   : *reinterpret_cast<const float4*>(Cs + row * ldc + lane * 4);
+            float4 e = *reinterpret_cast<const float4*>(Cs + row * ldc + lane * 4);
+            if (rr < 2 && s < 2) e = tk[rr];
             v = make_float4(v.x + e.x, v.y + e.y, v.z + e.z, v.w + e.w);
         }
         if (s >= a.S) v = make_float4(0.f, 0.f, 0.f, 0.f);
@@ -1170,15 +1249,19 @@
         rows_to_h16(Xh, ldq, row, lane, v);
     }
     __syncthreads();
-    tail_qkv_rows<4, 8, H16_PF>(Xh, reinterpret_cast<unsigned short*>(Cs), a.qkv_w, a.qkv_b, a.q_out, a.kp_out, a.vp_out, b, q0, a.S, a.spv, ring_t);
+    tail_qkv_rows<WAVES, RW, H16_PF, true>(Xh, reinterpret_cast<unsigned short*>(Cs), a.qkv_w, a.qkv_b, a.q_out, a.kp_out, a.vp_out, b, q0, a.S, a.spv, ring_t, bias_t);
+}
+template <int WAVES, int RW>
+static int launch_pro_w(const ProHArgs& a, hipStream_t st) {
+    const size_t lds = (size_t)TILE_M * (256 + LDS_PAD) * 4 + (size_t)TILE_M * (256 + HPAD) * 2;
+    dim3 grid((a.S + TILE_M - 1) / TILE_M, a.B);
+    SEEME_HIP(hipFuncSetAttribute((const void*)k_vae_pro_h<WAVES, RW>, hipFuncAttributeMaxDynamicSharedMemorySize, (int)lds));
+    hipLaunchKernelGGL((k_vae_pro_h<WAVES, RW>), grid, dim3(64 * WAVES), lds, st, a);
+    return seeme_check_launch("k_vae_pro_h");
 }
 static int launch_pro_h(const ProHArgs& a, hipStream_t st) {
     if (a.mode == 1 && a.F > 256) return seeme_fail("vae_pro_h: nfeats > 256");
-    const size_t lds = (size_t)TILE_M * (256 + LDS_PAD) * 4 + (size_t)TILE_M * (256 + HPAD) * 2;
-    dim3 grid((a.S + TILE_M - 1) / TILE_M, a.B);
-    SEEME_HIP(hipFuncSetAttribute((const void*)k_vae_pro_h, hipFuncAttributeMaxDynamicSharedMemorySize, (int)lds));
-    hipLaunchKernelGGL(k_vae_pro_h, grid, dim3(256), lds, st, a);
-    return seeme_check_launch("k_vae_pro_h");
+    return layer_form(a.B, a.S, a.S) == 1 ? launch_pro_w<8, 4>(a, st) : launch_pro_w<4, 8>(a, st);
 }
 
 __global__ void k_enc_tokens_h(const float* __restrict__ token, const float* __restrict__ pe, float* __restrict__ x, int B, int S) {
diff --git a/seeme_amd/csrc/vae_kernels.hip b/seeme_amd/csrc/vae_kernels.hip
--- a/seeme_amd/csrc/vae_kernels.hip
+++ b/seeme_amd/csrc/vae_kernels.hip
@@ -1,146 +1,12 @@
 #include "common.hpp"
 #include "api_util.hpp"
+#include "linear_tile.hpp"
 
 
 
 __global__ __launch_bounds__(256) void k_linear(const LinearKArgs ka) {
     extern __shared__ __attribute__((aligned(16))) float smem[];
-    SeemeLinearArgs a = ka.a;
-    if (ka.nz > 1) {
-        const long z = blockIdx.z;
-        a.A += z * ka.zs_a; a.W += z * ka.zs_w; a.Y += z * ka.zs_y;
-        if (a.bias) a.bias += z * ka.zs_b;
-        if (a.pre_ln_w) { a.pre_ln_w += z * ka.zs_ln; a.pre_ln_b += z * ka.zs_ln; }
-        if (z < ka.pre_ln_zmin) { a.pre_ln_w = nullptr; a.pre_ln_b = nullptr; }
-    }
-    const int tid = threadIdx.x, wave = tid >> 6, lane = tid & 63;
-    const int Kp = (a.K + 15) & ~15;
-    const int lda_s = Kp + LDS_PAD;
-    float* As = smem;
-    float* Cs = smem + TILE_M * lda_s;
-    const int ldc = CH_N + LDS_PAD;
-    const int m0 = blockIdx.x * TILE_M;
-    const int cn0 = blockIdx.y * (ka.narrow ? 64 : CH_N);
-
-    const bool a_vec = (a.A2 == nullptr) && ((a.K & 3) == 0) && ((a.lda & 3) == 0) && ((reinterpret_cast<size_t>(a.A) & 15) == 0);
-    if (a_vec) {
-        const int K4 = a.K >> 2, Kp4 = Kp >> 2, total = TILE_M * Kp4;
-        for (int base = 0; base < total; base += 256 * 8) {
-            float4 v[8];
-#pragma unroll
-            for (int j = 0; j < 8; ++j) {
-                const int idx = base + tid + j * 256, row = idx / Kp4, c4 = idx - row * Kp4, m = m0 + row;
-                const bool valid = idx < total && m < a.M && c4 < K4;
-                int prow = valid ? m : 0;
-                if (ka.seq_in > 0) prow = (prow / ka.seq_in) * ka.in_stride + (prow % ka.seq_in) + ka.in_off;
-                v[j] = *reinterpret_cast<const float4*>(valid ? a.A + (size_t)prow * a.lda + 4 * c4 : a.A);
-                if (!valid) v[j] = make_float4(0.f, 0.f, 0.f, 0.f);
-            }
-#pragma unroll
-            for (int j = 0; j < 8; ++j) {
-                const int idx = base + tid + j * 256, row = idx / Kp4, c4 = idx - row * Kp4;
-                if (idx < total) *reinterpret_cast<float4*>(As + row * lda_s + 4 * c4) = v[j];
-            }
-        }
-    } else {
-        for (int idx = tid; idx < TILE_M * Kp; idx += 256) {
-            const int row = idx / Kp, c = idx - row * Kp;
-            const int m = m0 + row;
-            float v = 0.f;
-            if (m < a.M && c < a.K) {
-                int prow = m;
-                if (ka.seq_in > 0) prow = (m / ka.seq_in) * ka.in_stride + (m % ka.seq_in) + ka.in_off;
-                v = (c < a.K1) ? a.A[(size_t)prow * a.lda + c] : a.A2[(size_t)prow * a.lda2 + (c - a.K1)];
-            }
-            As[row * lda_s + c] = v;
-        }
-    }
-    __syncthreads();
-    if (a.pre_ln_w != nullptr) {
-        for (int rr = 0; rr < 8; ++rr) {
-            const int row = wave * 8 + rr;
-            float s = 0.f;
-            for (int c = lane; c < a.K; c += 64) s += As[row * lda_s + c];
-            const float mean = wave_sum(s) / (float)a.K;
-            float q = 0.f;
-            for (int c = lane; c < a.K; c += 64) { float d = As[row * lda_s + c] - mean; q += d * d; }
-            const float rs = 1.f / sqrtf(wave_sum(q) / (float)a.K + a.eps);
-            for (int c = lane; c < a.K; c += 64)
-                As[row * lda_s + c] = (As[row * lda_s + c] - mean) * rs * a.pre_ln_w[c] + a.pre_ln_b[c];
-        }
-        __syncthreads();
-    }
-    if (a.pre_act != SEEME_ACT_NONE) {
-        for (int idx = tid; idx < TILE_M * Kp; idx += 256) {
-            const int row = idx / Kp, c = idx - row * Kp;
-            if (c < a.K) As[row * lda_s + c] = act_apply(As[row * lda_s + c], a.pre_act);
-        }
-        __syncthreads();
-    }
-
-    if (ka.narrow) {
-        f32x4 acc[2][1];
-        acc_zero(acc);
-        const int n0 = cn0 + wave * 16;
-        if (n0 < a.N) tile_gemm_f32<2, 1>(As, lda_s, a.W, a.ldw, n0, a.N, Kp >> 4, acc);
-        acc_store_lds<2, 1>(acc, Cs, ldc, wave * 16, a.bias, cn0, a.N, a.act);
-    } else {
-        f32x4 acc[2][4];
-        acc_zero(acc);
-        const int n0 = cn0 + wave * 64;
-        if (n0 < a.N) tile_gemm_f32<2, 4>(As, lda_s, a.W, a.ldw, n0, a.N, Kp >> 4, acc);
-        acc_store_lds<2, 4>(acc, Cs, ldc, wave * 64, a.bias, cn0, a.N, a.act);
-    }
-    __syncthreads();
-
-    const bool vec_ok = ((a.ldy & 3) == 0) && ((a.N & 3) == 0) && ((reinterpret_cast<size_t>(a.Y) & 15) == 0);
-    const bool res_vec = a.res != nullptr && ((a.ldr & 3) == 0) && ((a.N & 3) == 0) && ((reinterpret_cast<size_t>(a.res) & 15) == 0);
-    const LnParams lp = ln_params256(a.ln_w, a.ln_b);
-    float4 rv[8];
-#pragma unroll
-    for (int rr = 0; rr < 8; ++rr) {
-        rv[rr] = make_float4(0.f, 0.f, 0.f, 0.f);
-        if (res_vec) {
-            const int m = m0 + wave * 8 + rr, mc = m < a.M ? m : 0, g = (ka.narrow && lane >= 16) ? a.N : cn0 + lane * 4;
-            int orow = mc;
-            if (ka.seq_in > 0) orow = (mc / ka.seq_in) * ka.out_stride + (mc % ka.seq_in) + ka.out_off;
-            const size_t rrow = ka.res_mode == 1 ? (size_t)((mc % ka.seq_in) + ka.res_off)
-                              : ka.res_mode == 2 ? (size_t)(mc / ka.seq_in) : (size_t)orow;
-            rv[rr] = *reinterpret_cast<const float4*>(a.res + rrow * a.ldr + (g + 3 < a.N ? g : 0));
-            if (g + 3 >= a.N) rv[rr] = make_float4(0.f, 0.f, 0.f, 0.f);
-        }
-    }
-#pragma unroll
-    for (int rr = 0; rr < 8; ++rr) {
-        const int row = wave * 8 + rr;
-        const int m = m0 + row;
-        if (m >= a.M) continue;
-        int orow = m;
-        if (ka.seq_in > 0) orow = (m / ka.seq_in) * ka.out_stride + (m % ka.seq_in) + ka.out_off;
-        const int c = (ka.narrow && lane >= 16) ? 0 : lane * 4, g = (ka.narrow && lane >= 16) ? a.N : cn0 + c;
-        float4 v = *reinterpret_cast<const float4*>(Cs + row * ldc + c);
-        if (res_vec) {
-            v = make_float4(v.x + rv[rr].x, v.y + rv[rr].y, v.z + rv[rr].z, v.w + rv[rr].w);
-        } else if (a.res != nullptr) {
-            const size_t rrow = ka.res_mode == 1 ? (size_t)((m % ka.seq_in) + ka.res_off)
-                              : ka.res_mode == 2 ? (size_t)(m / ka.seq_in) : (size_t)orow;
-            const float* rp = a.res + rrow * a.ldr + g;
-            if (g + 0 < a.N) v.x += rp[0];
-            if (g + 1 < a.N) v.y += rp[1];
-            if (g + 2 < a.N) v.z += rp[2];
-            if (g + 3 < a.N) v.w += rp[3];
-        }
-        if (a.ln_w != nullptr) v = wave_layernorm256(v, lp, a.eps);
-        float* yp = a.Y + (size_t)orow * a.ldy + g;
-        if (vec_ok && g + 3 < a.N) {
-            *reinterpret_cast<float4*>(yp) = v;
-        } else {
-            if (g + 0 < a.N) yp[0] = v.x;
-            if (g + 1 < a.N) yp[1] = v.y;
-            if (g + 2 < a.N) yp[2] = v.z;
-            if (g + 3 < a.N) yp[3] = v.w;
-        }
-    }
+    linear_tile(ka, blockIdx.x, blockIdx.y, blockIdx.z, smem);
 }
 
 #define SEEME_LDS_PER_WORKGROUP 163840
diff --git a/seeme_amd/mld_denoiser.py b/seeme_amd/mld_denoiser.py
--- a/seeme_amd/mld_denoiser.py
+++ b/seeme_amd/mld_denoiser.py
@@ -155,6 +155,7 @@
         self.cluster = cluster
         self.cluster_placement = 1
         self.cluster_flags = 0
+        self.fused_prep = True
         self.cluster_ms = True
         self.pack_xcds = "auto"
 
@@ -408,14 +409,29 @@
                trow.numel(), Bc, catab.data_ptr(), ws.data_ptr(), ws.numel() * 4, L.current_stream())
         return catab
 
-    def _launch(self, latents2d, ctab, ttab, trow, per_sample, steps, sched, coef, noise, cfg, guidance):
+    PREP_MAX_BC = 64
+    PREP_BC = 32
+
+    def cond_prep(self, cond_bf: torch.Tensor, ttab: torch.Tensor, trow: torch.Tensor, per_sample: bool = False):
+        L.require_cuda(cond_bf, "condition")
+        cond_bf = cond_bf.contiguous()
+        Bc, N, _ = cond_bf.shape
+        ctab = torch.empty(Bc, N, L.CROW, device=cond_bf.device, dtype=torch.float32)
+        catab = torch.empty(Bc, trow.numel(), 5, self.latent_dim, device=cond_bf.device, dtype=torch.float32)
+        w = self._weights()
+        L.call("seeme_denoiser_cond_prep", C.byref(w), cond_bf.data_ptr(), Bc, N, ttab.data_ptr(), trow.data_ptr(), int(per_sample),
+               trow.numel(), ctab.data_ptr(), catab.data_ptr(), L.current_stream())
+        return ctab, catab
+
+    def _launch(self, latents2d, ctab, ttab, trow, per_sample, steps, sched, coef, noise, cfg, guidance, catab=None):
         B, N = latents2d.shape[0], ctab.shape[1]
         out = torch.empty(B, self.latent_dim, device=latents2d.device, dtype=torch.float32)
         a = L.SampleArgs()
         a.B, a.N, a.steps, a.sched, a.cfg, a.guidance_scale = B, N, steps, sched, int(cfg), float(guidance)
         a.latents, a.ctab, a.ttab, a.trow, a.trow_per_sample = latents2d.data_ptr(), ctab.data_ptr(), ttab.data_ptr(), trow.data_ptr(), int(per_sample)
         a.coef, a.noise, a.out = L.ptr(coef), L.ptr(noise), out.data_ptr()
-        catab = self.ca_tables(ctab, ttab, trow, per_sample) if N == 1 else None
+        if catab is None and N == 1:
+            catab = self.ca_tables(ctab, ttab, trow, per_sample)
         a.catab = L.ptr(catab)
         a.xcds = L.default_xcds((B + 1) // 2 if (B > 256 and not per_sample and not cfg) else B, self.pack_xcds)
         w = self._weights()
@@ -475,7 +491,11 @@
             cached = (tfeat, coef, trow, self.time_tables(tfeat))
             self._table_cache = {key: cached}
         tfeat, coef, trow, ttab = cached
-        ctab = self.cond_tables(cond_bf)
+        catab = None
+        if self.fused_prep and cond_bf.shape[1] == 1 and cond_bf.shape[0] <= self.PREP_BC:
+            ctab, catab = self.cond_prep(cond_bf, ttab, trow)
+        else:
+            ctab = self.cond_tables(cond_bf)
         steps = len(trow)
         noise = None
         if scheduler.needs_noise(eta):
@@ -486,7 +506,7 @@
         lat2 = latents.reshape(B, -1).contiguous()
         if events is not None:
             events[0].record()
-        out = self._launch(lat2, ctab, ttab, trow, False, steps, sched, coef, noise, cfg, guidance_scale)
+        out = self._launch(lat2, ctab, ttab, trow, False, steps, sched, coef, noise, cfg, guidance_scale, catab)
         if events is not None:
             events[1].record()
         return out.reshape(1, B, self.latent_dim)
```

Measured after the change: 17560 seqs/s (median of 2 runs). Within noise of the previous version (+0.3%).
